# jeffchy/RE2NN-SEQ

Measured on AMD Instinct MI355X. Metric: tagged tokens/sec @ batch=256, seqlen=64; achieved HBM GB/s vs peak, higher is better.
Workload: dtype f32; 1 GPU; ATIS-BIO-sized onehot i-FST (--method onehot --independent 2): V=950 S=71 C=128, batch 256 x seqlen 64 per GPU, lengths U[5,64]; batches_rotated=4, parallelism=batch-sharded x1 (weights replicated)

## Files before the change

re2nn-seq_amd/csrc/chain_dest.hip.h:

```cpp
#pragma once
#include "common.hip.h"
#include "chain_regs_params.hip.h"

namespace farnn {

template <int D, int LPR>
struct DestRing {
    static constexpr int NC = 20 / LPR;
    v4f r[D][NC];
    unsigned voff[NC];
    int tkw_lo, tkw_hi;
};

template <int LPR>
__device__ __forceinline__ void dest_lane(const int lane, int &rj, int &rs, bool &has_row) {
    if constexpr (LPR == 4) { rj = lane >> 2; rs = lane & 3; has_row = true; }
    else { const int r16 = lane & 15, bq = r16 / 5; rs = r16 - 5 * bq; rj = 3 * (lane >> 4) + bq; has_row = bq < 3; }
}

#ifndef FARNN_RD_CPOL
#define FARNN_RD_CPOL ""
#endif
#define FARNN_RD_ISSUE_(ring_, d, base_)                                                       \
    do {                                                                                       \
        const char *bp_ = (base_);                                                             \
        if constexpr (NC == 5)                                                                 \
            asm volatile("s_nop 4\n\t"                                                         \
                         "global_load_dwordx4 %0, %5, %10" FARNN_RD_CPOL "\n\t"                                 \
                         "global_load_dwordx4 %1, %6, %10" FARNN_RD_CPOL "\n\t"                                 \
                         "global_load_dwordx4 %2, %7, %10" FARNN_RD_CPOL "\n\t"                                 \
                         "global_load_dwordx4 %3, %8, %10" FARNN_RD_CPOL "\n\t"                                 \
                         "global_load_dwordx4 %4, %9, %10" FARNN_RD_CPOL                                     \
                         : "=&v"(ring_.r[d][0]), "=&v"(ring_.r[d][1]), "=&v"(ring_.r[d][2]), "=&v"(ring_.r[d][3]), "=&v"(ring_.r[d][NC - 1]) \
                         : "v"(ring_.voff[0]), "v"(ring_.voff[1]), "v"(ring_.voff[2]), "v"(ring_.voff[3]), "v"(ring_.voff[NC - 1]), "s"(bp_)); \
        else                                                                                   \
            asm volatile("s_nop 4\n\t"                                                         \
                         "global_load_dwordx4 %0, %4, %8" FARNN_RD_CPOL "\n\t"                                  \
                         "global_load_dwordx4 %1, %5, %8" FARNN_RD_CPOL "\n\t"                                  \
                         "global_load_dwordx4 %2, %6, %8" FARNN_RD_CPOL "\n\t"                                  \
                         "global_load_dwordx4 %3, %7, %8" FARNN_RD_CPOL                                      \
                         : "=&v"(ring_.r[d][0]), "=&v"(ring_.r[d][1]), "=&v"(ring_.r[d][2]), "=&v"(ring_.r[d][3]) \
                         : "v"(ring_.voff[0]), "v"(ring_.voff[1]), "v"(ring_.voff[2]), "v"(ring_.voff[3]), "s"(bp_)); \
    } while (0)

template <int D, int LPR>
__device__ __forceinline__ void regs_dest_prime(const RegsParams &p, const int dir, const int w, const int lane, const int nsteps,
                                                const int len, const int b, DestRing<D, LPR> &ring) {
    constexpr int NC = DestRing<D, LPR>::NC;
    const int S = p.S, SP = p.SP, CPR = p.CPR;
    const int RW = (S + RG_NWC - 1) / RG_NWC;
    int rj, rs;
    bool has_row;
    dest_lane<LPR>(lane, rj, rs, has_row);
    const int my_row = w * RW + rj;
    const bool my_valid = has_row && rj < RW && my_row < S;
#pragma unroll
    for (int i = 0; i < NC; i++) {
        const int ci = rs + LPR * i;
        ring.voff[i] = ((unsigned)(my_valid ? my_row : 0) * (unsigned)SP + (unsigned)((my_valid && ci < CPR) ? ci : rs < CPR ? rs : 0) * 4u) * 4u;
    }
    {
        const int t = lane < nsteps ? lane : nsteps - 1;
        const int idx = (dir == 0) ? t : (t < len ? len - 1 - t : t);
        const long long o_ = (long long)clamp_tok(p.x[(long long)b * p.L + idx], p.V) * p.blk * 4;
        ring.tkw_lo = (int)(unsigned)o_; ring.tkw_hi = (int)(unsigned)(o_ >> 32);
    }
    const char *Mbase = reinterpret_cast<const char *>(dir == 0 ? p.Mb : p.Mf);
#pragma unroll
    for (int d = 0; d < D; d++) {
#pragma unroll
        for (int u = 0; u < NC; u++) ring.r[d][u] = v4f{0.f, 0.f, 0.f, 0.f};
        if (d < nsteps) {
            const unsigned lo = (unsigned)__builtin_amdgcn_readlane(ring.tkw_lo, d), hi = (unsigned)__builtin_amdgcn_readlane(ring.tkw_hi, d);
            FARNN_RD_ISSUE_(ring, d, Mbase + (((long long)hi << 32) | lo));
        }
    }
}

template <bool NLX, int D, int LPR>
__device__ __forceinline__ void regs_compute_dest(const RegsParams &p, const int dir, const int w, const int lane_in, const int nsteps,
                                                  const long long *tokoff, float *flags, const float *ol, float *hist, float *xd,
                                                  const bool probe, const int b, DestRing<D, LPR> &ring) {
    static_assert(D == 2 || D == 4, "an even ring depth that divides 64 (the exchange row's parity and the address window)");
    static_assert(LPR == 4 || LPR == 5, "four or five lanes per output row");
    constexpr int NC = 20 / LPR;
    static_assert(LPR * NC * 4 == RD_XS, "the exchange row holds every lane's chunks");
    int lane = lane_in;
    const int S = p.S, SP = p.SP, CPR = p.CPR;
    const int RW = (S + RG_NWC - 1) / RG_NWC;
    int rj, rs;
    bool has_row;
    dest_lane<LPR>(lane, rj, rs, has_row);
    const int my_row = w * RW + rj;
    const bool my_valid = has_row && rj < RW && my_row < S;
    const bool my_writer = my_valid && rs == (LPR == 4 ? 0 : 4);
    const bool is_flane = lane == 63;
    (void)CPR;
    const char *Mbase = reinterpret_cast<const char *>(dir == 0 ? p.Mb : p.Mf);
    const float my_o = my_valid ? ol[my_row] : 1.0f;
    const float c_pre = dir == 0 ? my_o : 1.0f, c_post = dir == 0 ? 1.0f : my_o;
    float *xbuf = xd;
    float *dumpa = xd + 2 * RD_XS, *dumpb = dumpa + 64;
    float *hptr = my_writer ? hist + SP + my_row : dumpa + lane;
    const int hstep = my_writer ? SP : 0;
    float *xw0 = my_writer ? xbuf + my_row : (is_flane ? flags + 4 * w : dumpb + lane);
    float *xw1 = my_writer ? xbuf + RD_XS + my_row : (is_flane ? flags + 4 * w : dumpb + lane);
    const float *xr = xbuf + 4 * rs;
    const int nl_mode = p.nl;
    const bool nl_relu = nl_mode == FARNN_NL_RELU;
    const int *pflag = reinterpret_cast<const int *>(flags) + 4 * (lane < RG_NWC ? lane : 0);

    v4f (&r)[D][NC] = ring.r;
    int &tkw_lo = ring.tkw_lo, &tkw_hi = ring.tkw_hi;
#define FARNN_RD_WINDOW(t_)                                                                    \
    do {                                                                                       \
        const int ti_ = (t_) + lane;                                                           \
        const long long o_ = tokoff[ti_ < nsteps ? ti_ : nsteps - 1];                          \
        tkw_lo = (int)(unsigned)o_; tkw_hi = (int)(unsigned)(o_ >> 32);                        \
    } while (0)
#define FARNN_RD_BASE(t_, lo_, hi_)                                                            \
    do {                                                                                       \
        const int li_ = (t_) & 63;                                                             \
        lo_ = (unsigned)__builtin_amdgcn_readlane(tkw_lo, li_);                                \
        hi_ = (unsigned)__builtin_amdgcn_readlane(tkw_hi, li_);                                \
    } while (0)
#define FARNN_RD_ISSUE(d, lo_, hi_) FARNN_RD_ISSUE_(ring, d, Mbase + (((long long)(hi_) << 32) | (lo_)))
#define FARNN_RD_WAITSTR                                                                       \
    "s_cmp_ge_i32 %[rem], %[dm1]\n\t"                                                          \
    "s_cbranch_scc1 1f\n\t"                                                                    \
    "s_waitcnt vmcnt(0)\n\t"                                                                   \
    "s_branch 2f\n"                                                                            \
    "1:\n\t"                                                                                   \
    "s_waitcnt vmcnt(%[cnt])\n"                                                                \
    "2:"
#define FARNN_RD_WAIT(d, rem_)                                                                 \
    do {                                                                                       \
        if constexpr (NC == 5)                                                                 \
            asm volatile(FARNN_RD_WAITSTR : "+v"(r[d][0]), "+v"(r[d][1]), "+v"(r[d][2]), "+v"(r[d][3]), "+v"(r[d][NC - 1]) \
                         : [rem] "s"(rem_), [dm1] "n"(D - 1), [cnt] "n"((D - 1) * NC) : "scc"); \
        else                                                                                   \
            asm volatile(FARNN_RD_WAITSTR : "+v"(r[d][0]), "+v"(r[d][1]), "+v"(r[d][2]), "+v"(r[d][3]) \
                         : [rem] "s"(rem_), [dm1] "n"(D - 1), [cnt] "n"((D - 1) * NC) : "scc"); \
    } while (0)

    unsigned nlo = 0, nhi = 0;
#if defined(FARNN_PROBES)
    long long ph[4] = {0, 0, 0, 0}, pt = 0;
#define FARNN_RD_PHASE(i) do { if (probe && w == 0 && (p.dbg & 256)) { const long long n_ = (long long)__builtin_amdgcn_s_memtime(); ph[i] += n_ - pt; pt = n_; } } while (0)
    if (probe && w == 0) pt = (long long)__builtin_amdgcn_s_memtime();
#else
#define FARNN_RD_PHASE(i) do { } while (0)
    (void)probe; (void)b;
#endif
    if (D < nsteps) FARNN_RD_BASE(D, nlo, nhi);
    for (int t0 = 0; t0 < nsteps; t0 += D) {
#pragma unroll
        for (int d = 0; d < D; d++) {
            const int t = t0 + d;
            if (t >= nsteps) break;
            constexpr int dummy = 0; (void)dummy;
            const int roff = (d & 1) * RD_XS;
            v4f st[NC];
            {
                int fl = lds_flag_get(pflag);
#pragma unroll
                for (int i = 0; i < NC; i++) st[i] = *reinterpret_cast<const v4f *>(xr + roff + 4 * LPR * i);
                asm volatile("" ::: "memory");
                if (__ballot(fl < t + 1) != 0ull) {
                    do { fl = lds_flag_get(pflag); } while (__ballot(fl < t + 1) != 0ull);
#pragma unroll
                    for (int i = 0; i < NC; i++) st[i] = *reinterpret_cast<const v4f *>(xr + roff + 4 * LPR * i);
                    asm volatile("" ::: "memory");
                }
            }
            FARNN_RD_PHASE(0);
            FARNN_RD_WAIT(d, nsteps - 1 - t);
            FARNN_RD_PHASE(1);
            v2f a01 = v2f{0.f, 0.f}, a23 = v2f{0.f, 0.f};
#pragma unroll
            for (int i = 0; i < NC; i++) {
                a01 = __builtin_elementwise_fma(st[i].xy, r[d][i].xy, a01);
                a23 = __builtin_elementwise_fma(st[i].zw, r[d][i].zw, a23);
            }
            float sa = a01.x + a01.y, sb = a23.x + a23.y;
            asm volatile("" : "+v"(sa), "+v"(sb));
            float s = sa + sb;
            if constexpr (LPR == 4) s = quad_sum(s);
            else {
                const float s1 = s + __int_as_float(__builtin_amdgcn_update_dpp(0, __float_as_int(s), 0x111, 0xf, 0xf, true));
                const float s2 = s1 + __int_as_float(__builtin_amdgcn_update_dpp(0, __float_as_int(s1), 0x112, 0xf, 0xf, true));
                s = s2 + __int_as_float(__builtin_amdgcn_update_dpp(0, __float_as_int(s), 0x114, 0xf, 0xf, true));
            }
            const float pre = s * c_pre;
            float hn;
            if (NLX) hn = apply_nl(pre, nl_mode);
            else     hn = nl_relu ? fmaxf(pre, 0.0f) : pre;
            const float hx = is_flane ? __int_as_float(t + 2) : hn * c_post;
            asm volatile("" ::: "memory");
            *hptr = hn;
            hptr += hstep;
            if (d & 1) *xw0 = hx; else *xw1 = hx;
            asm volatile("" ::: "memory");
            if (t + D < nsteps) FARNN_RD_ISSUE(d, nlo, nhi);
            if (d == D - 1 && ((t + 1 + D) & 63) == 0 && t + 1 + D < nsteps) FARNN_RD_WINDOW(t + 1 + D);
            FARNN_RD_BASE(t + 1 + D, nlo, nhi);
            asm volatile("" : "+s"(nlo), "+s"(nhi));
            FARNN_RD_PHASE(2);
        }
    }
#if defined(FARNN_PROBES)
    if (probe && w == 0 && lane == 0 && (p.dbg & 256))
        printf("seq %d dir %d chain phases (destination split), cycles per step: partner wait + state reads %lld, block wait %lld, fma + reduce + stores + issue %lld\n",
               b, dir, ph[0] / nsteps, ph[1] / nsteps, ph[2] / nsteps);
#endif
#undef FARNN_RD_PHASE
#undef FARNN_RD_WAIT
#undef FARNN_RD_WAITSTR
#undef FARNN_RD_ISSUE
#undef FARNN_RD_BASE
#undef FARNN_RD_WINDOW
}

}
```

re2nn-seq_amd/csrc/chain_regs.hip:

```cpp
#include <hip/hip_runtime.h>
#include <hip/hip_ext.h>

#include "common.hip.h"
#include "host_util.hip.h"
#include "chain_regs.hip.h"

namespace farnn {

int launch_chain_regs(const RegsParams &p, bool maxsr, bool score, hipStream_t s, hipEvent_t e0, hipEvent_t e1) {
    const int NP = RG_NWC * p.G;
    const bool dest = p.dest && !maxsr;
    const size_t lds = (size_t)regs_lds(p.L, p.SP, NP, p.sp.c16, p.sp.Kc, score, RG_RQ, score && bs_label_map_path(p.sp), dest).total * sizeof(float);
    const dim3 grid(2 * p.B), block(RG_WAVES * 64);
    int rc;
    const bool nlx = p.nl != FARNN_NL_NONE && p.nl != FARNN_NL_RELU;
    const bool lmo = score && bs_label_map_path(p.sp);
#define FARNN_LAUNCH_REGS5(MX, SC, NX, LM, DS)                                                 \
    do {                                                                                       \
        if ((rc = raise_lds_limit(chain_regs_kernel<MX, SC, NX, LM, DS>, lds))) return rc;     \
        if (e0 && e1)                                                                          \
            hipExtLaunchKernelGGL((chain_regs_kernel<MX, SC, NX, LM, DS>), grid, block, (uint32_t)lds, s, e0, e1, 0, p); \
        else                                                                                   \
            chain_regs_kernel<MX, SC, NX, LM, DS><<<grid, block, lds, s>>>(p);                \
    } while (0)
#if defined(FARNN_AB)
#define FARNN_LAUNCH_REGS4(MX, SC, NX, LM) do { if (!MX && dest) FARNN_LAUNCH_REGS5(MX, SC, NX, LM, !MX); else FARNN_LAUNCH_REGS5(MX, SC, NX, LM, false); } while (0)
#else
#define FARNN_LAUNCH_REGS4(MX, SC, NX, LM)                                                     \
    do {                                                                                       \
        if (!MX && dest) FARNN_LAUNCH_REGS5(MX, SC, NX, LM, !MX);                              \
        else if constexpr (MX) FARNN_LAUNCH_REGS5(MX, SC, NX, LM, false);                      \
        else return fail(FARNN_EINVAL, "FARNN_NODEST=1: the source-split compute wavefronts of the sum semiring are compiled into the A/B " \
                                       "build only (FARNN_LIB=.../libfarnn_hip_probes.so, csrc/build.py --probes)%s%s"); \
    } while (0)
#endif
#define FARNN_LAUNCH_REGS3(MX, SC, NX) do { if (SC && lmo) FARNN_LAUNCH_REGS4(MX, SC, NX, SC); else FARNN_LAUNCH_REGS4(MX, SC, NX, false); } while (0)
#define FARNN_LAUNCH_REGS(MX, SC) do { if (nlx) FARNN_LAUNCH_REGS3(MX, SC, true); else FARNN_LAUNCH_REGS3(MX, SC, false); } while (0)
    if (maxsr) { if (score) FARNN_LAUNCH_REGS(true, true); else FARNN_LAUNCH_REGS(true, false); }
    else       { if (score) FARNN_LAUNCH_REGS(false, true); else FARNN_LAUNCH_REGS(false, false); }
#undef FARNN_LAUNCH_REGS
#undef FARNN_LAUNCH_REGS3
#undef FARNN_LAUNCH_REGS4
#undef FARNN_LAUNCH_REGS5
    FARNN_HIP_TRY(hipGetLastError());
    return FARNN_OK;
}

}

#if defined(FARNN_PROBES)
extern "C" int farnn_debug_wg_stamps(long long *out, int n_workgroups) {
    if (!out || n_workgroups < 0 || n_workgroups > farnn::WG_STAMP_MAX) return FARNN_EINVAL;
    if (hipDeviceSynchronize() != hipSuccess) return FARNN_EIO;
    return hipMemcpyFromSymbol(out, HIP_SYMBOL(farnn::g_wg_stamps), sizeof(long long) * 16 * (size_t)n_workgroups) == hipSuccess ? FARNN_OK : FARNN_EIO;
}
#endif
```

re2nn-seq_amd/csrc/chain_regs.hip.h:

```cpp
#pragma once
#include "common.hip.h"
#include "score_params.hip.h"
#include "launch_order.hip.h"
#include "chain_regs_params.hip.h"
#include "beside.hip.h"

#ifndef FARNN_ABLATE
#define FARNN_ABLATE 0
#endif

namespace farnn {

__device__ __forceinline__ void lds_flag_set(int *f, int v) {
    asm volatile("" ::: "memory");
    __hip_atomic_store(f, v, __ATOMIC_RELAXED, __HIP_MEMORY_SCOPE_WORKGROUP);
}
__device__ __forceinline__ int lds_flag_get(const int *f) {
    const int v = __hip_atomic_load(f, __ATOMIC_RELAXED, __HIP_MEMORY_SCOPE_WORKGROUP);
    asm volatile("" ::: "memory");
    return v;
}
template <int PSTR = RG_PART_STRIDE>
__device__ __forceinline__ int regs_flag_newest(const float *fbase, int lane) {
    const int *f = reinterpret_cast<const int *>(fbase) + 4 * (lane < RG_NWC ? lane : 0);
    const int v0 = lds_flag_get(f), v1 = lds_flag_get(f + PSTR);
    return max(v0, v1);
}
template <int PSTR = RG_PART_STRIDE>
__device__ __forceinline__ bool regs_rows_reached(const float *fbase, int lane, int rows) {
    return __ballot(regs_flag_newest<PSTR>(fbase, lane) < rows + 1) == 0ull;
}
template <int PSTR = RG_PART_STRIDE>
__device__ __forceinline__ int regs_rows_done(const float *fbase, int lane) {
    int v = regs_flag_newest<PSTR>(fbase, lane);
#pragma unroll
    for (int off = 1; off < 8; off <<= 1) v = min(v, __shfl_xor(v, off, WAVE));
    return __builtin_amdgcn_readfirstlane(v) - 1;
}

__device__ __forceinline__ float quad_sum(float x) {
    x += __int_as_float(__builtin_amdgcn_update_dpp(0, __float_as_int(x), 0xB1, 0xf, 0xf, true));
    x += __int_as_float(__builtin_amdgcn_update_dpp(0, __float_as_int(x), 0x4E, 0xf, 0xf, true));
    return x;
}
__device__ __forceinline__ float quad_max(float x) {
    x = fmaxf(x, __int_as_float(__builtin_amdgcn_update_dpp(0, __float_as_int(x), 0xB1, 0xf, 0xf, true)));
    x = fmaxf(x, __int_as_float(__builtin_amdgcn_update_dpp(0, __float_as_int(x), 0x4E, 0xf, 0xf, true)));
    return x;
}

}
#include "chain_wide.hip.h"
#include "chain_dest.hip.h"
namespace farnn {

#if defined(FARNN_PROBES)
constexpr int WG_STAMP_MAX = 4096;
__device__ long long g_wg_stamps[16 * WG_STAMP_MAX];
#define FARNN_RG_STAMP(i) do { if (probe && lane == 0) stamps[i] = (long long)__builtin_amdgcn_s_memtime(); } while (0)
#else
#define FARNN_RG_STAMP(i) do { } while (0)
#endif

template <bool MAXSR, bool SCORE, bool NLX, int RQ = RG_RQ, int D = RG_D, bool LMO = false, bool DEST = false>
__device__ __forceinline__ void chain_regs_body(const RegsParams &p, float *smem, const int tid, const int item, int *b_out) {
    constexpr bool WIDE = RQ != RG_RQ;
    static_assert(!DEST || (!WIDE && !MAXSR), "the destination-split form exists for the narrow kernel and the sum semiring");
    constexpr int PSTR = WIDE ? rgw_part_stride(RQ) : RG_PART_STRIDE;
    constexpr int NG = WIDE ? RGW_NG : RG_NG;
    const int lane = tid & 63;
    const int w = __builtin_amdgcn_readfirstlane(tid >> 6);
    constexpr int nthreads = RG_WAVES * 64;
    const int dir = item & 1, slot = item >> 1;
    const int S = p.S, SP = p.SP, G = p.G, RPG = p.RPG, NP = RG_NWC * G;
    const int PS = WIDE ? p.PS : SP;
    const bool lm_path = SCORE && (LMO || bs_label_map_path(p.sp));
    const RegsLds lds = regs_lds(p.L, SP, NP, p.sp.c16, p.sp.Kc, SCORE, RQ, lm_path, DEST);
    long long *tokoff = reinterpret_cast<long long *>(smem + lds.tok);
    float *part = smem + lds.part, *ol = smem + lds.ol, *hist = smem + lds.hist;
    float *ab = smem + lds.ab, *scl = smem + lds.scl, *obuf = smem + lds.obuf;
    int *misc = reinterpret_cast<int *>(smem + lds.misc);

    int b = p.order ? p.order[slot] : slot;
    int len_sel = -1;
    if (p.sort) b = select_by_length_rank(p.len, p.B, p.L, p.pair ? folded_rank(slot, p.B) : slot, reinterpret_cast<int *>(hist), tid, nthreads, &len_sel);
    if (b_out) *b_out = b;
    const int len = len_sel >= 0 ? len_sel : clamp_len(p.len[b], p.L);
    const int nsteps = p.full ? p.L : len;
    const float *hinit = dir == 0 ? p.h0 : p.hT;
#if defined(FARNN_PROBES)
    __shared__ long long stamps[8];
    const bool quiet = (p.dbg & 2048) != 0;
    const bool probe = ((p.dbg & 32768) && nsteps == p.L && p.L >= 32) || quiet;
    if (w == 0) FARNN_RG_STAMP(0);
#endif

    constexpr bool PRIME_EARLY = DEST && (!SCORE || LMO);
    DestRing<RD_D, RD_LPR> dring;
    if constexpr (PRIME_EARLY)
        if (w < RG_NWC && nsteps > 0) regs_dest_prime<RD_D, RD_LPR>(p, dir, w, lane, nsteps, len, b, dring);
    for (int k = tid; k < nsteps; k += nthreads) {
        const int idx = (dir == 0) ? k : (k < len ? len - 1 - k : k);
        tokoff[k] = (long long)clamp_tok(p.x[(long long)b * p.L + idx], p.V) * p.blk * 4;
    }
    for (int j = tid; j < SP; j += nthreads) ol[j] = (p.o && j < S) ? p.o[j] : 1.0f;
    for (int j = tid; j < (nsteps + 1) * SP; j += nthreads) hist[j] = (j < S) ? hinit[j] : 0.0f;
    if (tid < 32) misc[tid] = tid == RGM_ACQ ? -1 : 0;
    if (tid < 2) part[tid * PSTR + PSTR - 1] = MAXSR ? -INFINITY : 0.0f;
    if (tid < 2 * 4 * RG_NWC) {
        const int fb = tid / (4 * RG_NWC), fk = tid % (4 * RG_NWC);
        part[fb * PSTR + NP * PS + fk] = (DEST && fb == 0 && (fk & 3) == 0) ? __int_as_float(1) : 0.0f;
    }
    if constexpr (DEST) {
        for (int j = tid; j < 2 * RD_XS; j += nthreads)
            smem[lds.xd + j] = j < S ? hinit[j] * ((dir == 1 && p.o) ? p.o[j] : 1.0f) : 0.0f;
    }
    if (WIDE && tid < RG_NWC * RGW_XCH) smem[lds.xch + tid] = 0.0f;
    __syncthreads();
    if (w == 0) FARNN_RG_STAMP(1);
#if FARNN_ABLATE & 256
    return;
#endif

    const float *sflag = part + NP * PS;
    float *stash = (dir == 0 ? p.A : p.Bk) + (long long)b * (p.L + 1) * SP;
    const int ntl = (nsteps + RG_TT - 1) / RG_TT;
    int kmid = 0, pubmax = 0;
    if (SCORE) bs_halves(dir, len, nsteps, kmid, pubmax);
    BesideParams bs;
    bs.A = p.A; bs.Bk = p.Bk; bs.B = p.B; bs.L = p.L; bs.SP = p.SP; bs.CPR = p.CPR; bs.prog = p.prog; bs.arr = p.arr;
    bs.done = p.done; bs.spin = p.spin; bs.dbg = p.dbg; bs.sp = p.sp;
    bs.epoch = (SCORE && w >= RG_NWC) ? (p.done ? bs_launch_epoch(p.done, lane) : p.epoch_host) : 0u;
    int wr_next = 0;
    unsigned lm_pk0 = 0u, lm_pk1 = 0u;
    if (lm_path) lm_load_packed(bs.sp.lm, lane, lm_pk0, lm_pk1);
    if (w < RG_NWC) {
        if constexpr (WIDE) {
            if (nsteps > 0) {
                __builtin_amdgcn_s_setprio(2);
                regs_compute_wide<MAXSR, NLX, RQ, D>(p, dir, w, lane, nsteps, tokoff, part, ol, hist, smem + lds.xch);
                __builtin_amdgcn_s_setprio(0);
                if (w == 0) FARNN_RG_STAMP(2);
#if defined(FARNN_PROBES)
                if (!SCORE && probe && !quiet && w == 0 && lane == 0)
                    printf("seq %d dir %d (wide): setup %lld, chain %lld (%lld per step)\n", b, dir, stamps[1] - stamps[0], stamps[2] - stamps[1],
                           (stamps[2] - stamps[1]) / nsteps);
#endif
            }
        } else if constexpr (DEST) {
            if (nsteps > 0) {
                __builtin_amdgcn_s_setprio(2);
#if defined(FARNN_PROBES)
                const bool probe_ = probe;
#else
                const bool probe_ = false;
#endif
                if constexpr (!PRIME_EARLY) regs_dest_prime<RD_D, RD_LPR>(p, dir, w, lane, nsteps, len, b, dring);
                regs_compute_dest<NLX, RD_D, RD_LPR>(p, dir, w, lane, nsteps, tokoff, part + NP * PS, ol, hist, smem + lds.xd, probe_, b, dring);
                __builtin_amdgcn_s_setprio(0);
                if (w == 0) FARNN_RG_STAMP(2);
#if defined(FARNN_PROBES)
                if (!SCORE && probe && !quiet && w == 0 && lane == 0)
                    printf("seq %d dir %d (destination split): setup %lld, chain %lld (%lld per step)\n", b, dir, stamps[1] - stamps[0], stamps[2] - stamps[1],
                           (stamps[2] - stamps[1]) / nsteps);
#endif
            }
        } else if (nsteps > 0) {
            __builtin_amdgcn_s_setprio(2);
            int g = lane / p.CPR;
            const int c = lane - g * p.CPR;
            const bool active = g < G;
            if (!active) g = 0;
            const int gid = w * G + g, row0 = gid * RPG;
            unsigned voff[RG_RQ];
#pragma unroll
            for (int u = 0; u < RG_RQ; u++) voff[u] = ((unsigned)(row0 + u) * (unsigned)SP + (unsigned)c * 4u) * 4u;
            const char *Mbase = reinterpret_cast<const char *>(dir == 0 ? p.Mf : p.Mb);
            const int rows_w = G * RPG;
            const int rj = lane >> 2, rs = lane & 3;
            const int my_row = w * rows_w + rj;
            const bool my_valid = rj < rows_w && my_row < S;
            const bool my_writer = my_valid && rs == 0;
            const float my_o = my_valid ? ol[my_row] : 1.0f;
            const float c_pre = dir == 0 ? my_o : 1.0f, c_post = dir == 0 ? 1.0f : my_o;
            const float ninf = -INFINITY;
            bool okrow[RG_RQ];
#pragma unroll
            for (int u = 0; u < RG_RQ; u++) okrow[u] = u < RPG && row0 + u < S;
            constexpr int NQI = (RG_NWC * RG_MAXG + 3) / 4;
            const float *ident = part + RG_PART_STRIDE - 1;
            float *dump = part + 2 * RG_PART_STRIDE;
            const float *qptr[NQI];
#pragma unroll
            for (int i = 0; i < NQI; i++)
                qptr[i] = (my_valid && rs + 4 * i < NP) ? part + (rs + 4 * i) * SP + my_row : ident;
            const int nact = G * p.CPR;
            const bool has_flane = nact < 64;
            const bool is_flane = lane == nact;
            float *fslot = part + NP * SP + 4 * w;
            float *wptr = active ? part + gid * SP + c * 4 : (is_flane ? fslot : part + NP * SP + 4 * RG_NWC + (lane - nact) * 4);
            float *hptr = my_writer ? hist + SP + my_row : dump + lane;
            const int hstep = my_writer ? SP : 0;
            int bsrc[RG_RQ];
            float hs[RG_RQ];
#pragma unroll
            for (int u = 0; u < RG_RQ; u++) {
                bsrc[u] = u < RPG ? 16 * (g * RPG + u) : 4 * 63;
                hs[u] = okrow[u] ? hist[row0 + u] * (dir == 1 ? ol[row0 + u] : 1.0f) : 0.0f;
            }
            const int nl_mode = p.nl;
            const bool nl_relu = nl_mode == FARNN_NL_RELU;
            const int *pflag = reinterpret_cast<const int *>(part + NP * SP) + 4 * (lane < RG_NWC ? lane : 0);

            v4f r[RG_D][RG_RQ];
#define FARNN_RG_WINDOW(t_)                                                                    \
            do {                                                                               \
                const int ti_ = (t_) + lane;                                                   \
                const long long o_ = tokoff[ti_ < nsteps ? ti_ : nsteps - 1];                  \
                tkw_lo = (int)(unsigned)o_; tkw_hi = (int)(unsigned)(o_ >> 32);                \
            } while (0)
#define FARNN_RG_BASE(t_, lo_, hi_)                                                            \
            do {                                                                               \
                const int li_ = (t_) & 63;                                                     \
                lo_ = (unsigned)__builtin_amdgcn_readlane(tkw_lo, li_);                        \
                hi_ = (unsigned)__builtin_amdgcn_readlane(tkw_hi, li_);                        \
            } while (0)
#define FARNN_RG_ISSUE(d, lo_, hi_)                                                            \
            do {                                                                               \
                const char *bp_ = Mbase + (((long long)(hi_) << 32) | (lo_));                  \
                asm volatile("s_nop 4\n\t"                                                     \
                             "global_load_dwordx4 %0, %4, %8\n\t"                              \
                             "global_load_dwordx4 %1, %5, %8\n\t"                              \
                             "global_load_dwordx4 %2, %6, %8\n\t"                              \
                             "global_load_dwordx4 %3, %7, %8"                                  \
                             : "=&v"(r[d][0]), "=&v"(r[d][1]), "=&v"(r[d][2]), "=&v"(r[d][3]) \
                             : "v"(voff[0]), "v"(voff[1]), "v"(voff[2]), "v"(voff[3]), "s"(bp_)); \
            } while (0)
#define FARNN_RG_WAIT(d, rem_)                                                                 \
            asm volatile("s_cmp_ge_i32 %4, 3\n\t"                                              \
                         "s_cbranch_scc1 1f\n\t"                                               \
                         "s_waitcnt vmcnt(0)\n\t"                                              \
                         "s_branch 2f\n"                                                       \
                         "1:\n\t"                                                              \
                         "s_waitcnt vmcnt(12)\n"                                               \
                         "2:"                                                                  \
                         : "+v"(r[d][0]), "+v"(r[d][1]), "+v"(r[d][2]), "+v"(r[d][3]) : "s"(rem_) : "scc")
            unsigned nlo = 0, nhi = 0;
            int tkw_lo, tkw_hi;
            FARNN_RG_WINDOW(0);
#pragma unroll
            for (int d = 0; d < RG_D; d++) {
#pragma unroll
                for (int u = 0; u < RG_RQ; u++) r[d][u] = v4f{0.f, 0.f, 0.f, 0.f};
                if (d < nsteps) {
                    FARNN_RG_BASE(d, nlo, nhi);
                    FARNN_RG_ISSUE(d, nlo, nhi);
                }
            }
#if defined(FARNN_PROBES)
            long long ph[5] = {0, 0, 0, 0, 0}, pt = 0;
#define FARNN_RG_PHASE(i) do { if (probe && w == 0 && (p.dbg & 256)) { const long long n_ = (long long)__builtin_amdgcn_s_memtime(); ph[i] += n_ - pt; pt = n_; } } while (0)
            if (probe && w == 0) pt = (long long)__builtin_amdgcn_s_memtime();
#else
#define FARNN_RG_PHASE(i) do { } while (0)
#endif
            if (RG_D < nsteps) FARNN_RG_BASE(RG_D, nlo, nhi);
#if FARNN_ABLATE & 512
            for (int t0 = 0; t0 < 0; t0 += RG_D) {
#else
            for (int t0 = 0; t0 < nsteps; t0 += RG_D) {
#endif
#pragma unroll
                for (int d = 0; d < RG_D; d++) {
                    const int t = t0 + d;
                    if (t >= nsteps) break;
                    static_assert(RG_D == 4 && RG_RQ == 4, "FARNN_RG_WAIT is written out for a 4 x 4 ring");
                    FARNN_RG_WAIT(d, nsteps - 1 - t);
                    FARNN_RG_PHASE(0);
                    v4f acc = MAXSR ? v4f{ninf, ninf, ninf, ninf} : v4f{0.f, 0.f, 0.f, 0.f};
#if FARNN_ABLATE & 8
                    acc = r[d][0] + r[d][1] * hs[0] + r[d][2] + r[d][3];
#else
#pragma unroll
                    for (int u = 0; u < RG_RQ; u++) {
                        if (MAXSR) {
                            acc.x = fmaxf(acc.x, okrow[u] ? hs[u] * r[d][u].x : ninf);
                            acc.y = fmaxf(acc.y, okrow[u] ? hs[u] * r[d][u].y : ninf);
                            acc.z = fmaxf(acc.z, okrow[u] ? hs[u] * r[d][u].z : ninf);
                            acc.w = fmaxf(acc.w, okrow[u] ? hs[u] * r[d][u].w : ninf);
                        } else {
                            acc.x = fmaf(hs[u], r[d][u].x, acc.x);
                            acc.y = fmaf(hs[u], r[d][u].y, acc.y);
                            acc.z = fmaf(hs[u], r[d][u].z, acc.z);
                            acc.w = fmaf(hs[u], r[d][u].w, acc.w);
                        }
                    }
#endif
                    const int boff = (d & 1) * RG_PART_STRIDE;
#if !(FARNN_ABLATE & 32)
                    if (has_flane) acc.x = is_flane ? __int_as_float(t + 1) : acc.x;
                    asm volatile("" ::: "memory");
                    *reinterpret_cast<v4f *>(wptr + boff) = acc;
                    if (!has_flane && lane == 0) lds_flag_set(reinterpret_cast<int *>(fslot + boff), t + 1);
#endif
                    asm volatile("" : "+v"(acc));
#if !(FARNN_ABLATE & 1)
                    if (t + RG_D < nsteps) FARNN_RG_ISSUE(d, nlo, nhi);
#endif
                    FARNN_RG_PHASE(1);
                    float pv[NQI];
#if FARNN_ABLATE & 16
#pragma unroll
                    for (int i = 0; i < NQI; i++) pv[i] = acc.x;
#else
                    for (;;) {
                        const int fl = lds_flag_get(pflag + boff);
#pragma unroll
                        for (int i = 0; i < NQI - 1; i++) pv[i] = qptr[i][boff];
                        pv[NQI - 1] = MAXSR ? ninf : 0.0f;
                        if (NP > 4 * (NQI - 1)) pv[NQI - 1] = qptr[NQI - 1][boff];
                        asm volatile("" ::: "memory");
                        if (__ballot(fl < t + 1) == 0ull) break;
#if FARNN_ABLATE & 2
                        break;
#endif
                    }
#endif
                    FARNN_RG_PHASE(2);
                    static_assert(NQI == 6, "the reduction tree below is written out for six partial sums per lane");
                    float s;
                    if (MAXSR) s = fmaxf(fmaxf(fmaxf(pv[0], pv[1]), fmaxf(pv[2], pv[3])), fmaxf(pv[4], pv[5]));
                    else       s = ((pv[0] + pv[1]) + (pv[2] + pv[3])) + (pv[4] + pv[5]);
                    s = MAXSR ? quad_max(s) : quad_sum(s);
                    const float pre = s * c_pre;
                    float hn;
                    if (NLX) hn = apply_nl(pre, nl_mode);
                    else     hn = nl_relu ? fmaxf(pre, 0.0f) : pre;
                    const float hx = my_valid ? hn * c_post : 0.0f;
#if !(FARNN_ABLATE & 64)
                    *hptr = hn;
                    hptr += hstep;
#endif
#if !(FARNN_ABLATE & 4)
                    int bp[RG_RQ];
#pragma unroll
                    for (int u = 0; u < RG_RQ; u++) bp[u] = __builtin_amdgcn_ds_bpermute(bsrc[u], __float_as_int(hx));
                    if (d == RG_D - 1 && ((t + 1 + RG_D) & 63) == 0 && t + 1 + RG_D < nsteps) FARNN_RG_WINDOW(t + 1 + RG_D);
                    FARNN_RG_BASE(t + 1 + RG_D, nlo, nhi);
                    asm volatile("" : "+s"(nlo), "+s"(nhi));
#pragma unroll
                    for (int u = 0; u < RG_RQ; u++) hs[u] = __int_as_float(bp[u]);
#else
                    if (t + 1 + RG_D < nsteps) {
                        if (((t + 1 + RG_D) & 63) == 0) FARNN_RG_WINDOW(t + 1 + RG_D);
                        FARNN_RG_BASE(t + 1 + RG_D, nlo, nhi);
                    }
#endif
                    FARNN_RG_PHASE(3);
                }
            }
            if (lane == 0) lds_flag_set(reinterpret_cast<int *>(fslot), nsteps + 1);
#if defined(FARNN_PROBES)
            if (probe && w == 0 && lane == 0 && (p.dbg & 256))
                printf("seq %d dir %d chain phases, cycles per step: block wait %lld, fma + store + issue %lld, partner wait + partial reads %lld, reduce + exchange %lld\n",
                       b, dir, ph[0] / nsteps, ph[1] / nsteps, ph[2] / nsteps, ph[3] / nsteps);
#endif
#undef FARNN_RG_PHASE
#undef FARNN_RG_ISSUE
#undef FARNN_RG_BASE
#undef FARNN_RG_WINDOW
#undef FARNN_RG_WAIT
            __builtin_amdgcn_s_setprio(0);
            if (w == 0) FARNN_RG_STAMP(2);
#if defined(FARNN_PROBES)
            if (!SCORE && probe && !quiet && w == 0 && lane == 0)
                printf("seq %d dir %d: setup %lld, chain %lld (%lld per step)\n", b, dir, stamps[1] - stamps[0], stamps[2] - stamps[1],
                       (stamps[2] - stamps[1]) / nsteps);
#endif
        }
    } else if (w == RG_NWC) {
        if (SCORE && dir == 0) {
            for (int i = nsteps + lane; i < p.L; i += WAVE)
                if (p.sp.tags) p.sp.tags[(long long)b * p.L + i] = -1;
            if (p.sp.scores)
                for (long long e = (long long)nsteps * p.sp.K + lane; e < (long long)p.L * p.sp.K; e += WAVE)
                    p.sp.scores[(long long)b * p.L * p.sp.K + e] = 0.0f;
        }
        int published = -1;
        auto copy_rows = [&](int r0, int r1) {
            const float *src = hist + r0 * SP;
            float *dst = stash + (long long)r0 * SP;
            const int nfl = (r1 - r0 + 1) * SP;
            if (SCORE) {
                for (int j = 2 * lane; j < nfl; j += 2 * WAVE) st2_agent(dst + j, src[j], src[j + 1]);
            } else {
                for (int j = lane; j < nfl; j += WAVE) dst[j] = src[j];
            }
        };
        if (!SCORE && !p.A) wr_next = nsteps + 1;
        while (wr_next <= nsteps) {
            const int done = nsteps > 0 ? regs_rows_done<PSTR>(sflag, lane) : 0;
            if (done < wr_next) { __builtin_amdgcn_s_sleep(1); continue; }
            if (SCORE && nsteps > 0 && wr_next > pubmax && done >= nsteps) break;
            const int hi = min(done, (SCORE && wr_next <= pubmax) ? pubmax : nsteps);
            copy_rows(wr_next, hi);
            wr_next = hi + 1;
            if (SCORE && hi < nsteps && published < pubmax) {
                published = hi;
                asm volatile("s_waitcnt vmcnt(0)" ::: "memory");
                if (lane == 0)
                    __hip_atomic_store(p.prog + (long long)dir * p.B + b, ((unsigned long long)bs.epoch << 32) | (unsigned)published,
                                       __ATOMIC_RELAXED, __HIP_MEMORY_SCOPE_AGENT);
            }
        }
    } else if (SCORE) {
        const int fo = bs_flat_offset(bs, b, lane);
        if (lane == 0) misc[RGM_FOFF] = fo;
        const long long foff = fo;
        unsigned mine = 0u;
        int acq = -1;
        const unsigned long long *oprog = p.prog + (long long)(dir ^ 1) * p.B + b;
        const int kfirst = dir == 0 ? kmid : kmid - 1, kstep = dir == 0 ? 1 : -1, klast = dir == 0 ? ntl : -1;
        if constexpr (!LMO)
        for (int k = kfirst; k != klast && !lm_path; k += kstep) {
            int na, nb;
            bs_tile_need(k, len, nsteps, na, nb);
            const int need_own = dir == 0 ? na : nb, need_oth = dir == 0 ? nb : na;
            if (nsteps - need_own < p.solo_margin) break;
            while (!regs_rows_reached<PSTR>(sflag, lane, need_own)) __builtin_amdgcn_s_sleep(4);
            if (need_oth > acq) {
                int pr = -1;
                for (;;) {
                    pr = lane == 0 ? bs_read_prog(oprog, bs.epoch) : 0;
                    pr = __builtin_amdgcn_readfirstlane(pr);
                    if (pr >= need_oth) break;
                    if (regs_rows_reached<PSTR>(sflag, lane, nsteps)) break;
                    __builtin_amdgcn_s_sleep(8);
                }
                if (pr < need_oth) break;
                __builtin_amdgcn_fence(__ATOMIC_ACQUIRE, "agent");
                acq = pr;
            }
            {
                const rg_f32x4 none[NG] = {};
                bs_score_tiles<false, RG_WAVES, NG, RG_NWC>(bs, b, dir, len, nsteps, k, -1, hist, nullptr, nullptr, ab, scl, foff, 0, lane, none);
            }
            mine |= 1u << k;
        }
        {
            int slot = 0;
            for (int k = kfirst; k != klast && slot < RG_NOB; k += kstep) {
                if ((mine >> k) & 1u) continue;
                int na, nb;
                bs_tile_need(k, len, nsteps, na, nb);
                const int need_oth = dir == 0 ? nb : na;
                if (need_oth > acq) {
                    int pr = -1;
                    for (;;) {
                        pr = lane == 0 ? bs_read_prog(oprog, bs.epoch) : 0;
                        pr = __builtin_amdgcn_readfirstlane(pr);
                        if (pr >= need_oth) break;
                        if (regs_rows_reached<PSTR>(sflag, lane, nsteps)) break;
                        __builtin_amdgcn_s_sleep(16);
                    }
                    if (pr < need_oth) break;
                    __builtin_amdgcn_fence(__ATOMIC_ACQUIRE, "agent");
                    acq = pr;
                }
                bs_park_rows<NG, (LMO && WIDE) ? NG / 2 : NG>(bs, b, dir, len, nsteps, k, obuf + slot * RG_TT * SP, lane);
                if (lane == 0) misc[RGM_PARK + slot] = k + 1;
                slot++;
            }
        }
        if (lane == 0) { misc[RGM_MINE] = (int)mine; misc[RGM_ACQ] = acq; }
        FARNN_RG_STAMP(3);
    }
    if constexpr (!SCORE) {
        if (b_out && dir == 0 && w == RG_WAVES - 1) {
            int partsum = 0;
            if (p.sp.flat && !p.sp.offs)
                for (int j = lane; j < b; j += WAVE) partsum += clamp_len(p.len[j], p.L);
#pragma unroll
            for (int off = 32; off >= 1; off >>= 1) partsum += __shfl_xor(partsum, off, WAVE);
            if (lane == 0) { misc[RGM_FOFF] = partsum; misc[RGM_FOFF + 1] = len; }
        }
        return;
    }

    if (w == 0) FARNN_RG_STAMP(4);
    bs_finish<RG_WAVES, NG, RG_WAVES - 1, RG_NWC, true, LMO>(bs, b, dir, len, nsteps, kmid, hist, ab, scl, obuf, misc, w, lane, lm_pk0, lm_pk1, bs.epoch,
        [&]() {
            if (w == RG_NWC)
                for (; wr_next <= nsteps; wr_next++)
                    for (int j = 2 * lane; j < SP; j += 2 * WAVE)
                        st2_agent(stash + (long long)wr_next * SP + j, hist[wr_next * SP + j], hist[wr_next * SP + j + 1]);
        },
        [&]() {
            if (w == RG_NWC) {
                asm volatile("s_waitcnt vmcnt(0)" ::: "memory");
                if (lane == 0)
                    __hip_atomic_store(p.prog + (long long)dir * p.B + b, ((unsigned long long)bs.epoch << 32) | (unsigned)nsteps,
                                       __ATOMIC_RELAXED, __HIP_MEMORY_SCOPE_AGENT);
            }
        });
#if defined(FARNN_PROBES)
    if (quiet && tid == 0 && item < WG_STAMP_MAX) {
        long long *o = g_wg_stamps + 16 * (long long)item + 8;
        o[0] = stamps[1] - stamps[0]; o[1] = stamps[2] - stamps[1]; o[2] = stamps[3] - stamps[2]; o[3] = stamps[4] - stamps[2];
        o[4] = (long long)__builtin_amdgcn_s_memtime() - stamps[4];
    }
    if (probe && !quiet && tid == 0) {
        const long long e = (long long)__builtin_amdgcn_s_memtime();
        printf("seq %d dir %d: setup %lld, chain %lld (%lld per step), scorer alone until +%lld, all waves at the meeting point +%lld, "
               "tiles + arrival %lld; tiles alone %d of %d\n", b, dir, stamps[1] - stamps[0], stamps[2] - stamps[1],
               (stamps[2] - stamps[1]) / nsteps, stamps[3] - stamps[2], stamps[4] - stamps[2], e - stamps[4],
               __popc((unsigned)misc[RGM_MINE]), ntl);
    }
#endif
}

template <bool MAXSR, bool SCORE, bool NLX, bool LMO = false, bool DEST = false>
__global__ void __launch_bounds__(RG_WAVES * 64, 4)
chain_regs_kernel(const RegsParams p) {
    extern __shared__ __align__(16) float smem[];
#if defined(FARNN_PROBES)
    long long w0r = 0, w0c = 0;
    if ((p.dbg & 2048) && threadIdx.x == 0) { w0r = (long long)__builtin_amdgcn_s_memrealtime(); w0c = (long long)__builtin_amdgcn_s_memtime(); }
    int b_probe = -1;
    chain_regs_body<MAXSR, SCORE, NLX, RG_RQ, RG_D, LMO, DEST>(p, smem, (int)threadIdx.x, (int)blockIdx.x, &b_probe);
    if ((p.dbg & 2048) && threadIdx.x == 0 && blockIdx.x < WG_STAMP_MAX) {
        const long long w1r = (long long)__builtin_amdgcn_s_memrealtime(), w1c = (long long)__builtin_amdgcn_s_memtime();
        unsigned hwid, xcc;
        asm volatile("s_getreg_b32 %0, hwreg(HW_REG_HW_ID)" : "=s"(hwid));
        asm volatile("s_getreg_b32 %0, hwreg(HW_REG_XCC_ID)" : "=s"(xcc));
        long long *o = g_wg_stamps + 16 * (long long)blockIdx.x;
        o[0] = b_probe; o[1] = b_probe >= 0 ? (long long)p.len[b_probe] : -1; o[2] = w0r; o[3] = w1r; o[4] = w1c - w0c;
        o[5] = xcc & 15u; o[6] = (hwid >> 13) & 7u; o[7] = (hwid >> 8) & 15u;
    }
#else
    chain_regs_body<MAXSR, SCORE, NLX, RG_RQ, RG_D, LMO, DEST>(p, smem, (int)threadIdx.x, (int)blockIdx.x, nullptr);
#endif
}

template <bool MAXSR, bool SCORE, bool NLX, int RQ, int D>
__global__ void __launch_bounds__(RG_WAVES * 64, 2)
chain_wide_kernel(const RegsParams p) {
    extern __shared__ __align__(16) float smem[];
    chain_regs_body<MAXSR, SCORE, NLX, RQ, D>(p, smem, (int)threadIdx.x, (int)blockIdx.x, nullptr);
}

template <bool MAXSR, bool NLX, int RQ>
__global__ void __launch_bounds__(RG_WAVES * 64, 4)
chain_wide_paired_kernel(const RegsParams p) {
    extern __shared__ __align__(16) float smem[];
    chain_regs_body<MAXSR, true, NLX, RQ, 2, true>(p, smem, (int)threadIdx.x, (int)blockIdx.x, nullptr);
}

}
```

re2nn-seq_amd/csrc/chain_regs_params.hip.h:

```cpp
#pragma once
#include <hip/hip_runtime.h>
#include "common.hip.h"
#include "score_params.hip.h"

namespace farnn {

constexpr int RG_NWC = 6;
constexpr int RG_WAVES = 8;
constexpr int RG_D = 4;
constexpr int RG_RQ = 4;
constexpr int RG_MAXG = 4;
constexpr int RG_MAXSP = 72;
constexpr int RG_PART_STRIDE = RG_NWC * RG_MAXG * RG_MAXSP;
constexpr int RGW_G = 2;
constexpr int RGW_NP = RG_NWC * RGW_G;
constexpr int RGW_MAXSP = 128;
constexpr int RGW_MAXRQ = 11;
__host__ __device__ constexpr int rgw_part_stride(int rq) { return rq <= 9 ? 1536 : 2048; }
constexpr int RGW_XCH = 32;
constexpr int RD_LPR = 5;
constexpr int RD_XS = 80;
constexpr int RD_D = 4;
constexpr int RD_XD_FLOATS = 2 * RD_XS + 128;

struct RegsParams {
    const float *Mf, *Mb;
    long long blk;
    const float *o, *h0, *hT;
    const int64_t *x, *len;
    const int *order;
    int sort;
    float *A, *Bk;
    int B, L, S, SP, CPR, V;
    int G, RPG;
    int RQ, D;
    int pair;
    int PS;
    int nl, full;
    unsigned long long *prog;
    unsigned long long *arr;
    unsigned long long *done;
    unsigned epoch_host;
    int spin;
    int dbg;
    int solo_margin;
    int dest;
    ScoreParams sp;
};
constexpr int RG_NG = 5;
constexpr int RGW_NG = 8;

struct RegsGeom {
    int G, RPG, NP, CPR, SP, rows;
    bool ok;
    bool wide;
    int RQ, D, PS;
};

inline RegsGeom regs_geometry(int S) {
    RegsGeom g;
    g.wide = false; g.RQ = RG_RQ; g.D = RG_D; g.PS = 0;
    g.SP = round_up(S, 4);
    g.CPR = g.SP / 4;
    g.ok = g.CPR <= 64 && S >= 1;
    g.G = g.ok ? 64 / g.CPR : 1;
    if (g.G > RG_MAXG) g.G = RG_MAXG;
    g.NP = RG_NWC * g.G;
    g.RPG = (S + g.NP - 1) / g.NP;
    if (g.RPG > RG_RQ) g.ok = false;
    g.rows = (g.NP - 1) * g.RPG + RG_RQ;
    if (g.NP * g.SP + 4 * RG_NWC + 4 * (64 - g.G * g.CPR) >= RG_PART_STRIDE) g.ok = false;
    if (!g.ok && S > 4 * RG_RQ && g.SP <= RGW_MAXSP) {
        g.wide = true;
        g.G = RGW_G; g.NP = RGW_NP;
        g.RPG = (S + g.NP - 1) / g.NP;
        g.RQ = g.RPG <= 8 ? 8 : (g.RPG <= 9 ? 9 : RGW_MAXRQ);
        g.D = 4;
        g.rows = g.NP * g.RPG;
        g.PS = ((g.SP + 15) & ~31) + 16;
        g.ok = g.RPG <= RGW_MAXRQ && g.NP * g.PS + 4 * RG_NWC + 4 * (64 - g.G * g.CPR) < rgw_part_stride(g.RQ);
    }
    return g;
}

struct RegsLds {
    int tok, hp, part, ol, hist, ab, scl, obuf, misc, xch, xd, total;
};
__host__ __device__ inline RegsLds regs_lds(int L, int SP, int NP, int c16, int Kc, bool score, int rq = RG_RQ, bool lm = false, bool dest = false) {
    const bool wide = rq != RG_RQ;
    RegsLds l;
    int at = 0;
    l.tok = at;  at += 2 * ((L + 1) & ~1);
    l.hp = at;
    l.part = at; at += 2 * (wide ? rgw_part_stride(rq) : RG_PART_STRIDE) + 64 * 4;
    l.ol = at;   at += SP;
    l.hist = at; at += (L + 1) * SP + 16;
    l.ab = at;   at += (score && !lm) ? 2 * RG_TT * (16 * c16 + 4) : 0;
    l.scl = at;  at += (score && !lm) ? 2 * RG_TT * Kc : 0;
    l.obuf = at; at += score ? 2 * RG_TT * SP : 0;
    l.misc = at; at += 32;
    l.xch = at;  at += wide ? RG_NWC * RGW_XCH : 0;
    l.xd = at;   at += dest ? RD_XD_FLOATS : 0;
    l.total = at;
    return l;
}

int launch_chain_regs(const RegsParams &p, bool maxsr, bool score, hipStream_t s, hipEvent_t e0, hipEvent_t e1);
int launch_chain_wide(const RegsParams &p, bool maxsr, bool score, hipStream_t s, hipEvent_t e0, hipEvent_t e1);
int launch_chain_wide_paired(const RegsParams &p, bool maxsr, hipStream_t s, hipEvent_t e0, hipEvent_t e1);

bool chain_viterbi_fits(int L, int SP, int NP, int K, int Kp, bool label_map, int rq = RG_RQ);
int launch_chain_viterbi(const RegsParams &p, const ScoreParams &sp, bool maxsr, hipStream_t s, hipEvent_t e0, hipEvent_t e1);

}
```

re2nn-seq_amd/csrc/farnn_hip.hip:

```cpp
#include <hip/hip_runtime.h>
#include <hip/hip_ext.h>
#include <stdlib.h>
#include <algorithm>
#include <utility>
#include <vector>

#include "common.hip.h"
#include "host_util.hip.h"
#include "chain.hip.h"
#include "score_decode.hip.h"
#include "layout.hip.h"
#include "fst4_score.hip.h"
#include "decomp_chain.hip.h"
#include "decomp1_score.hip.h"
#include "decomp_rows.hip.h"
#include "compact_tag.hip.h"
#include "decomp_regs.hip.h"
#include "compact.hip.h"
#include "chain_regs_params.hip.h"
#include "tag_host.hip.h"
#include "tag_create.hip.h"

namespace farnn {
thread_local char g_err[512] = "";
thread_local const Tunables *g_tun = nullptr;
}

extern "C" int farnn_has_compact(const farnn_model *m) { return (m && m->bmNS > 0 && m->bmF) ? 1 : 0; }

extern "C" int farnn_set_compact(farnn_model *m, int32_t enable) {
    if (!m) return fail(FARNN_EINVAL, "set_compact: null model%s%s");
    if (enable && !farnn_has_compact(m))
        return fail(FARNN_EINVAL, "set_compact: this model has no compact form (i-FST with 0/1 weights, sum semiring, at most 512 states)%s%s");
    if (!enable && !m->Mf) return fail(FARNN_EINVAL, "set_compact: this handle was created compact-only (no dense blocks)%s%s");
    m->compact_on = enable != 0;
    return FARNN_OK;
}

extern "C" int farnn_reserve(farnn_model *m, int32_t B, int32_t L) {
    if (!m || B <= 0 || L <= 0) return fail(FARNN_EINVAL, "reserve: bad arguments%s%s");
    Workspace &w = m->ws;
    if (B <= w.B && L <= w.L) return FARNN_OK;
    TunScope tun_scope(&m->tun);
    FARNN_HIP_TRY(hipSetDevice(m->device));
    const int nB = B > w.B ? B : w.B, nL = L > w.L ? L : w.L;
    if (w.A) FARNN_HIP_TRY(hipDeviceSynchronize());
    w.release();
    size_t stash = (size_t)nB * (nL + 1) * m->SP * sizeof(float);
    FARNN_HIP_TRY(hipMalloc((void **)&w.A, stash));
    FARNN_HIP_TRY(hipMalloc((void **)&w.Bk, stash));
    FARNN_HIP_TRY(hipMalloc((void **)&w.offs, (size_t)(nB + 1) * sizeof(int64_t)));
    FARNN_HIP_TRY(hipMalloc((void **)&w.order, (size_t)nB * sizeof(int)));
    w.hs_bytes = round_up_sz((size_t)(3 * nB + 48) * sizeof(unsigned long long), 16);
    FARNN_HIP_TRY(hipMalloc((void **)&w.hs, w.hs_bytes));
    FARNN_HIP_TRY(hipMemset(w.hs, 0, w.hs_bytes));
    if (m->use_crf)
        FARNN_HIP_TRY(hipMalloc((void **)&w.crf_scores, (size_t)nB * nL * m->Kp * sizeof(float) + 1024));
    if (m->d1_BSSp)
        FARNN_HIP_TRY(hipMalloc((void **)&w.d1_br, (size_t)nB * nL * ((m->S + 15) / 16) * ((m->RO + 15) / 16 * 16) * sizeof(float)));
    FARNN_HIP_TRY(hipMemset(w.A, 0, stash));
    FARNN_HIP_TRY(hipMemset(w.Bk, 0, stash));
    FARNN_HIP_TRY(hipDeviceSynchronize());
    w.B = nB; w.L = nL;
    return FARNN_OK;
}

struct KernelTimer {
    farnn_model *m; int which; hipStream_t s; hipEvent_t e0 = nullptr, e1 = nullptr;
    bool ext;
    KernelTimer(farnn_model *m_, int w, hipStream_t s_, bool ext_ = false) : m(m_), which(w), s(s_), ext(ext_) {
        if (m->prof_this_call) {
            e0 = m->prof.get(); e1 = m->prof.get();
            if (e0 && e1 && !ext) (void)hipEventRecord(e0, s);
        }
    }
    ~KernelTimer() {
        if (e0 && e1) {
            if (!ext) (void)hipEventRecord(e1, s);
            m->prof.ev[which].push_back(e0);
            m->prof.ev[which].push_back(e1);
        }
    }
};

static void prof_fold(farnn_model *m) {
    for (int k = 0; k < KERN_COUNT; k++) {
        auto &v = m->prof.ev[k];
        for (size_t i = 0; i + 1 < v.size(); i += 2) {
            float ms = 0.f;
            if (hipEventSynchronize(v[i + 1]) == hipSuccess &&
                hipEventElapsedTime(&ms, v[i], v[i + 1]) == hipSuccess) {
                m->prof.ms[k] += ms; m->prof.n[k] += 1;
            }
            m->prof.pool.push_back(v[i]); m->prof.pool.push_back(v[i + 1]);
        }
        v.clear();
    }
}

extern "C" int farnn_set_profiling(farnn_model *m, int32_t enable) {
    if (!m) return fail(FARNN_EINVAL, "null model%s%s");
    prof_fold(m);
    if (enable) {
        for (int k = 0; k < KERN_COUNT; k++) { m->prof.ms[k] = 0; m->prof.n[k] = 0; }
        while (m->prof.pool.size() < 256) {
            hipEvent_t e = nullptr;
            if (hipEventCreate(&e) != hipSuccess) break;
            m->prof.pool.push_back(e);
        }
    }
    m->profiling = enable > 0 ? enable : 0;
    m->calls = 0;
    return FARNN_OK;
}

extern "C" int farnn_kernel_time(farnn_model *m, int32_t which, double *total_ms, int64_t *launches) {
    if (!m || which < 0 || which >= KERN_COUNT) return fail(FARNN_EINVAL, "kernel_time: bad arguments%s%s");
    prof_fold(m);
    if (total_ms) *total_ms = m->prof.ms[which];
    if (launches) *launches = m->prof.n[which];
    return FARNN_OK;
}

extern "C" const char *farnn_kernel_name(const farnn_model *m, int32_t which) {
    if (!m) return "";
    TunScope tun_scope(&m->tun);
    switch (which) {
        case KERN_CHAIN:
            if (m->compact_on) return m->last_fused ? "compact_tag_kernel<fused: both chains + label-map scores + decode>" : "compact_chain_kernel";
            if (m->last_regs && m->last_fused && m->use_crf) return "chain_viterbi_kernel<fused: recurrence + scores + CRF decode>";
            if (m->last_regs && m->rgeom.wide) return m->last_fused ? "chain_wide_kernel<fused: scores + decode beside the recurrence>" : "chain_wide_kernel";
            if (m->last_regs) return m->last_fused ? "chain_regs_kernel<fused: scores + decode beside the recurrence>" : "chain_regs_kernel";
            if (m->dense_decomp) return "chain_kernel";
            if (m->kind == KIND_DECOMP && m->last_fused && m->last_wave) return "decomp_regs_kernel<fused: scores + decode beside the recurrence>";
            if (m->kind == KIND_DECOMP || m->kind == KIND_DECOMP1 || m->kind == KIND_DECOMP0)
                return m->rows.ok ? ((m->last_wave || (m->calls == 0 && m->dw.farnn == 0 && m->dw.R <= DG_ROWS && !tun(TUN_DECOMP_NOREGS))) ? "decomp_regs_kernel" : "decomp_rows_kernel") : "decomp_chain_kernel";
            return "chain_kernel";
        case KERN_SCORE: return m->kind == KIND_FST4 ? "fst4_score_kernel"
                              : (m->kind == KIND_IND1 ? "ind1_score_kernel"
                              : (m->kind == KIND_DECOMP1 ? (m->d1_BSSp ? "decomp1_br_mfma_kernel+decomp1_label_kernel" : "decomp1_score_kernel")
                              : (m->kind == KIND_DECOMP0 ? "decomp0_score_kernel"
                              : (m->use_crf ? "score_tile_kernel+viterbi_kernel" : (m->last_lm_score ? "label_map_score_kernel" : "score_tile_kernel")))));
        case KERN_PREP:  return "batch_prep_kernel";
        default: return "";
    }
}


static RegsParams make_regs_params(farnn_model *m, const int64_t *x, const int64_t *len, int B, int full) {
    const RegsGeom &rg = m->rgeom;
    RegsParams rp;
    memset(&rp, 0, sizeof(rp));
    rp.Mf = m->Mf; rp.Mb = m->Mb; rp.blk = (long long)m->geom.SR * m->SP;
    rp.o = m->o; rp.h0 = m->h0; rp.hT = m->hT; rp.x = x; rp.len = len;
    rp.order = m->order_valid ? m->ws.order : nullptr; rp.sort = m->sort_in_kernel ? 1 : 0;
    rp.A = m->ws.A; rp.Bk = m->ws.Bk; rp.B = B; rp.L = m->curL; rp.S = m->S; rp.SP = m->SP; rp.CPR = rg.CPR; rp.V = m->V;
    rp.G = rg.G; rp.RPG = rg.RPG; rp.RQ = rg.RQ; rp.D = rg.D; rp.PS = rg.PS; rp.pair = rg.wide ? 0 : 1;
    rp.nl = m->nl; rp.full = full; rp.dbg = tun(TUN_DBG);
    rp.dest = (!rg.wide && m->semiring != FARNN_SEMIRING_MAX && !tun(TUN_NODEST)) ? 1 : 0;
    return rp;
}

static int handoff_words(farnn_model *m, unsigned long long **prog, unsigned long long **arr, unsigned long long **done) {
    *prog = m->ws.hs; *arr = m->ws.hs + (size_t)2 * m->ws.B; *done = m->ws.hs + (size_t)3 * m->ws.B + 16;
    return FARNN_OK;
}

static int launch_chain(farnn_model *m, const int64_t *x, const int64_t *len, int B, int L, int full,
                        hipStream_t s, const ScoreParams *fuse_sp = nullptr, bool *fused = nullptr) {
    const ChainGeom &g = m->geom;
    if (fused) *fused = false;
    m->last_regs = false;
    if (m->rgeom.ok && !tun(TUN_NOREGS)) {
        const RegsGeom &rg = m->rgeom;
        const size_t lds_cap = rg.wide ? 158 * 1024 : 80 * 1024;
        bool score = fuse_sp && m->ws.hs && m->OTm && m->c16 >= 1 && m->c16 <= (rg.wide ? RGW_NG : RG_NG) && m->Kc <= 256 && m->curL <= 31 * RG_TT &&
                     (B <= 1024 || !fuse_sp->flat || fuse_sp->offs) && !tun(TUN_NOFUSE);
        if (score && !rg.wide && bs_label_map_path(*fuse_sp) && !tun(TUN_FUSE)) score = false;
        const bool lm_path = score && bs_label_map_path(*fuse_sp);
        const bool dest = !rg.wide && m->semiring != FARNN_SEMIRING_MAX && !tun(TUN_NODEST);
        size_t lds = (size_t)regs_lds(m->curL, m->SP, rg.NP, score ? m->c16 : 0, score ? m->Kc : 0, score, rg.RQ, lm_path, dest).total * sizeof(float);
        const bool paired = rg.wide && lm_path && rg.RQ <= 9 && lds <= 80 * 1024 && !tun(TUN_WIDE_UNPAIRED);
        if (score && lds > lds_cap) {
            score = false;
            lds = (size_t)regs_lds(m->curL, m->SP, rg.NP, 0, 0, false, rg.RQ, false, dest).total * sizeof(float);
        }
        if (lds <= lds_cap) {
            RegsParams rp = make_regs_params(m, x, len, B, full);
            if (score) {
                int hrc = handoff_words(m, &rp.prog, &rp.arr, &rp.done);
                if (hrc) return hrc;
                if (tun(TUN_HOST_EPOCH)) {
                    if (++m->epoch_u == 0) { FARNN_HIP_TRY(hipMemsetAsync(m->ws.hs, 0, m->ws.hs_bytes, s)); m->epoch_u = 1; }
                    rp.done = nullptr; rp.epoch_host = m->epoch_u + 0x40000000u;
                }
                rp.spin = tun(TUN_FUSE_SPIN);
                rp.solo_margin = tun(TUN_SOLO_MARGIN);
                rp.sp = *fuse_sp;
                if (fused) *fused = true;
            }
            KernelTimer kt(m, KERN_CHAIN, s, true);
            if (paired && score) { rp.D = 2; rp.pair = 1; }
            const int rc = (paired && score) ? launch_chain_wide_paired(rp, m->semiring == FARNN_SEMIRING_MAX, s, kt.e0, kt.e1)
                           : rg.wide ? launch_chain_wide(rp, m->semiring == FARNN_SEMIRING_MAX, score, s, kt.e0, kt.e1)
                                     : launch_chain_regs(rp, m->semiring == FARNN_SEMIRING_MAX, score, s, kt.e0, kt.e1);
            if (rc) return rc;
            m->last_regs = true;
            return FARNN_OK;
        }
    }
    (void)fuse_sp;
    ChainParams p;
    p.Mf = m->Mf; p.Mb = m->Mb; p.blk = (long long)m->geom.SR * m->SP;
    p.o = m->o; p.h0 = m->h0; p.hT = m->hT; p.x = x; p.len = len; p.A = m->ws.A; p.Bk = m->ws.Bk;
    p.order = m->order_valid ? m->ws.order : nullptr;
    p.sort = m->sort_in_kernel ? 1 : 0;
    p.B = B; p.L = m->curL; p.S = m->S; p.SP = m->SP; p.CPR = g.CPR; p.V = m->V;
    p.NW = g.NW; p.NLD = g.NLD; p.G = g.G; p.LPR = g.LPR; p.RPG = g.RPG; p.RPGp = g.RPGp; p.NQ = g.NQ;
    p.nl = m->nl; p.full = full; p.dbg = tun(TUN_DBG);
    int ks = 2, nqp = g.NQ;
    if (!g.pick_ring(m->curL, m->chain_ks, ks, nqp))
        return fail(FARNN_ERANGE, "chain kernel: LDS ring does not fit (sequence too long for this S)%s%s");
    p.KS = ks; p.NQP = nqp; p.PPS = (g.NQ + nqp - 1) / nqp;
    const size_t lds = g.lds_bytes(m->curL, ks, nqp);
    dim3 grid(2 * B), block((g.NW + g.NLD + 1) * 64);
    const bool mx = m->semiring == FARNN_SEMIRING_MAX;
    int rc = FARNN_OK;
    if (tun(TUN_CHAIN_HELPER) && block.x < 512) block = dim3(block.x + 64);
    KernelTimer kt(m, KERN_CHAIN, s, true);
    const int fq_max = block.x <= 384 ? 6 : 3;
    const int fq = (g.NCH == 1 && p.PPS == 1 && g.NQ <= fq_max && !tun(TUN_NOFAST)) ? g.NQ : 0;
    auto go = [&](auto NCH, auto FQ) {
        return mx ? launch_timed(chain_kernel<NCH(), true, FQ()>, grid, block, lds, s, kt.e0, kt.e1, p)
                  : launch_timed(chain_kernel<NCH(), false, FQ()>, grid, block, lds, s, kt.e0, kt.e1, p);
    };
    if (g.NCH == 1) {
        if (fq == 1) rc = go(int_c<1>(), int_c<1>());
        else if (fq == 2) rc = go(int_c<1>(), int_c<2>());
        else if (fq == 3) rc = go(int_c<1>(), int_c<3>());
        else if (fq == 4) rc = go(int_c<1>(), int_c<4>());
        else if (fq == 5) rc = go(int_c<1>(), int_c<5>());
        else if (fq == 6) rc = go(int_c<1>(), int_c<6>());
        else rc = go(int_c<1>(), int_c<0>());
    } else if (g.NCH == 2) rc = go(int_c<2>(), int_c<0>());
    else if (g.NCH <= 4) rc = go(int_c<4>(), int_c<0>());
    else return fail(FARNN_ERANGE, "unsupported state count%s%s");
    if (rc) return rc;
    FARNN_HIP_TRY(hipGetLastError());
    return FARNN_OK;
}

static int launch_decomp_recurrence(farnn_model *m, const int64_t *x, const int64_t *lengths, int B, int full,
                                    hipStream_t s, const ScoreParams *fuse_sp = nullptr, bool *fused = nullptr) {
    if (fused) *fused = false;
    const int *order = m->order_valid ? m->ws.order : nullptr;
    if (m->n_cu <= 0) m->n_cu = device_cus(m->device);
    RegsPlan rp;
    m->last_wave = m->rows.ok && regs_plan(m->rows, m->dw, m->curL, rp);
    if (m->last_wave) {
        BesideParams bs;
        const BesideParams *use = nullptr;
        bool score = fuse_sp && m->ws.hs && m->OTm && m->c16 >= 1 && m->c16 <= DG_NG && m->Kc <= 256 && m->curL <= 31 * RG_TT &&
                     (B <= 1024 || !fuse_sp->flat || fuse_sp->offs) && !tun(TUN_NOFUSE);
        if (score) {
            rp.lds_score = regs_score_lds(rp, m->curL, m->SP, m->c16, m->Kc);
            if (rp.lds_score > 80 * 1024) score = false;
        }
        if (score) {
            memset(&bs, 0, sizeof(bs));
            bs.A = m->ws.A; bs.Bk = m->ws.Bk; bs.B = B; bs.L = m->curL; bs.SP = m->SP; bs.CPR = m->SP / 4;
            int hrc = handoff_words(m, &bs.prog, &bs.arr, &bs.done);
            if (hrc) return hrc;
            bs.spin = tun(TUN_FUSE_SPIN); bs.dbg = tun(TUN_DBG); bs.sp = *fuse_sp;
            use = &bs;
            if (fused) *fused = true;
        }
        return launch_decomp_regs(m->rows, m->dw, rp, x, lengths, order, m->sort_in_kernel ? 1 : 0, m->ws.A, m->ws.Bk, B, m->curL,
                                  full, s, use);
    }
    RowsPlan pl;
    if (m->rows.ok && rows_plan(m->rows, m->dw, B, m->curL, pl))
        return launch_decomp_rows(m->rows, m->dw, pl, x, lengths, order, m->sort_in_kernel ? 1 : 0, m->ws.A, m->ws.Bk, B,
                                  m->curL, full, m->n_cu, s);
    return launch_decomp_chain(m->dw, x, lengths, order, m->ws.A, m->ws.Bk, B, m->curL, full, s);
}

static bool viterbi_can_fuse(const farnn_model *m, const ScoreParams &p) {
    return m->use_crf && !p.scores && !p.P && p.A && p.OT && m->K <= 256 &&
           viterbi_hist_lds_bytes(m->K, m->Kp, p.SP, p.L, true) <= 158 * 1024 && viterbi_hist_ib4(m->K) <= 6 &&
           !tun(TUN_VITERBI_BP) && !tun(TUN_VITERBI_UNFUSED);
}

static int launch_viterbi(farnn_model *m, const ScoreParams &p, int B, hipStream_t s, bool fused = false) {
    int rc;
    if (m->K > 256) return fail(FARNN_ERANGE, "Viterbi: more than 256 tags%s%s");
    const size_t hlds = viterbi_hist_lds_bytes(m->K, m->Kp, p.SP, p.L, fused);
    if (hlds <= 158 * 1024 && viterbi_hist_ib4(m->K) <= 6 && !tun(TUN_VITERBI_BP)) {
        const int threads = viterbi_hist_score_threads(m->K, fused);
        auto go = [&](auto N) {
            return fused ? launch(viterbi_hist_kernel<N(), true>, dim3(B), dim3(threads), hlds, s, p)
                         : launch(viterbi_hist_kernel<N(), false>, dim3(B), dim3(threads), hlds, s, p);
        };
        rc = FARNN_OK;
        switch (viterbi_hist_ib4(m->K)) {
            case 0: rc = go(int_c<0>()); break;
            case 1: rc = go(int_c<1>()); break;
            case 2: rc = go(int_c<2>()); break;
            case 3: rc = go(int_c<3>()); break;
            case 4: rc = go(int_c<4>()); break;
            case 5: rc = go(int_c<5>()); break;
            case 6: rc = go(int_c<6>()); break;
        }
        if (rc) return rc;
        FARNN_HIP_TRY(hipGetLastError());
        return FARNN_OK;
    }
    if (fused) return fail(FARNN_EINVAL, "Viterbi: the fused form needs the history in LDS%s%s");
    const size_t vlds = viterbi_lds_bytes(m->K, m->Kp, p.L);
    const int threads = round_up(4 * m->K, 64);
    auto go = [&](auto N) { return launch(viterbi_kernel<N()>, dim3(B), dim3(threads), vlds, s, p); };
    const int ib4 = viterbi_ib4(m->K);
    if (ib4 == 2) rc = go(int_c<2>());
    else if (ib4 == 4) rc = go(int_c<4>());
    else if (ib4 == 9) rc = go(int_c<9>());
    else if (ib4 == 13) rc = go(int_c<13>());
    else rc = go(int_c<16>());
    if (rc) return rc;
    FARNN_HIP_TRY(hipGetLastError());
    return FARNN_OK;
}

static int launch_decomp1_score(farnn_model *m, const int64_t *x, const int64_t *len, int B, int full,
                                int32_t *tags, int64_t *flat, float *scores, hipStream_t s) {
    Decomp1ScoreParams p;
    p.A = m->ws.A; p.Bk = m->ws.Bk; p.Vgen = m->dw.Vgen; p.S1 = m->dw.S1; p.S2 = m->dw.S2; p.W = m->dw.W;
    p.S1o = m->d1_S1o; p.S2o = m->d1_S2o; p.CoutT = m->d1_CoutT; p.P = m->P;
    p.x = x; p.len = len; p.offs = flat ? m->ws.offs : nullptr;
    p.tags = tags; p.flat = flat; p.scores = scores; p.crf_scores = m->ws.crf_scores;
    p.B = B; p.L = m->curL; p.S = m->S; p.SP = m->SP; p.R = m->R; p.Rp = m->Rp; p.RO = m->RO; p.ROp = m->ROp;
    p.V = m->V;
    p.K = m->K; p.Kp = m->Kp; p.Kc = m->Kc;
    p.full = full; p.use_crf = m->use_crf; p.o_idx = m->o_idx; p.threshold = m->threshold;
    int rc;
    KernelTimer kt(m, KERN_SCORE, s);
    Decomp1MfmaParams qm;
    qm.base = p; qm.BSSp = m->d1_BSSp; qm.S1oP = m->d1_S1oP; qm.S2oP = m->d1_S2oP; qm.br = m->ws.d1_br;
    if (!full) qm.base.offs = m->ws.offs;
    qm.MT = (m->S + 15) / 16; qm.NT = (m->RO + 15) / 16; qm.KQ4 = (m->S + 15) / 16;
    const size_t mlds = decomp1_mfma_lds_bytes(qm.MT, qm.NT);
    if (m->d1_BSSp && m->ws.d1_br && mlds <= 80 * 1024) {
        if (m->n_cu <= 0) m->n_cu = device_cus(m->device);
        const int nwg = std::min(2 * m->n_cu, (B * p.L + 3) / 4);
        auto go = [&](auto N) { return launch(decomp1_br_mfma_kernel<N()>, dim3(nwg), dim3(256), mlds, s, qm); };
        switch (qm.NT) {
            case 1: rc = go(int_c<1>()); break;
            case 2: rc = go(int_c<2>()); break;
            case 3: rc = go(int_c<3>()); break;
            case 4: rc = go(int_c<4>()); break;
            case 5: rc = go(int_c<5>()); break;
            default: return fail(FARNN_ERANGE, "decomp_ind1: output rank above 80 on the MFMA path%s%s");
        }
        if (rc) return rc;
        FARNN_HIP_TRY(hipGetLastError());
        const int NC = qm.NT * 16;
        const bool staged = decomp1_label_lds_bytes(NC, m->RO, m->K, m->Kc, true, 16) <= 150 * 1024;
        const int lthreads = staged ? 1024 : 256;
        const size_t llds = decomp1_label_lds_bytes(NC, m->RO, m->K, m->Kc, staged, lthreads / 64);
        const int lgrid = std::min((staged ? 1 : 4) * m->n_cu, (B * p.L + lthreads / 64 - 1) / (lthreads / 64));
        if (staged) {
            if ((rc = raise_lds_limit(decomp1_label_kernel<true>, llds))) return rc;
            decomp1_label_kernel<true><<<dim3(lgrid), dim3(lthreads), llds, s>>>(p, m->ws.d1_br, NC, qm.MT, full ? nullptr : m->ws.offs);
        } else {
            decomp1_label_kernel<false><<<dim3(lgrid), dim3(lthreads), llds, s>>>(p, m->ws.d1_br, NC, qm.MT, full ? nullptr : m->ws.offs);
        }
    } else {
        const size_t lds = decomp1_score_lds_bytes(m->S, m->SP, m->Rp, m->ROp, m->Kc);
        if ((rc = raise_lds_limit(decomp1_score_kernel, lds))) return rc;
        decomp1_score_kernel<<<dim3(p.L, B), dim3(256), lds, s>>>(p);
    }
    FARNN_HIP_TRY(hipGetLastError());
    if (m->use_crf) {
        ScoreParams v;
        memset(&v, 0, sizeof(v));
        v.trT = m->tr; v.len = len; v.offs = flat ? m->ws.offs : nullptr; v.tags = tags; v.flat = flat;
        v.crf_scores = m->ws.crf_scores; v.B = B; v.L = m->curL; v.K = m->K; v.Kp = m->Kp;
        v.full = full; v.use_crf = 1; v.o_idx = m->o_idx; v.threshold = m->threshold;
        if ((rc = launch_viterbi(m, v, B, s))) return rc;
    }
    return FARNN_OK;
}

static int launch_decomp0_score(farnn_model *m, const int64_t *x, const int64_t *len, int B, int full,
                                int32_t *tags, int64_t *flat, float *scores, hipStream_t s) {
    Decomp0ScoreParams p;
    p.A = m->ws.A; p.Bk = m->ws.Bk; p.Vgen = m->d0_Vgen; p.S1 = m->dw.S1; p.S2 = m->dw.S2; p.CT = m->d0_CT;
    p.S1w = m->d0_S1w; p.S2w = m->d0_S2w; p.CwT = m->d0_CwT; p.P = m->P;
    p.x = x; p.len = len; p.offs = flat ? m->ws.offs : nullptr;
    p.tags = tags; p.flat = flat; p.scores = scores; p.crf_scores = m->ws.crf_scores;
    p.B = B; p.L = m->curL; p.S = m->S; p.SP = m->SP; p.R = m->R; p.Rp = m->Rp; p.RW = m->RW; p.RWp = m->RWp;
    p.V = m->V;
    p.K = m->K; p.Kp = m->Kp; p.Kc = m->Kc;
    p.full = full; p.use_crf = m->use_crf; p.o_idx = m->o_idx; p.threshold = m->threshold;
    const size_t lds = decomp0_score_lds_bytes(m->SP, m->Rp, m->RWp, m->Kc);
    int rc;
    if ((rc = raise_lds_limit(decomp0_score_kernel, lds))) return rc;
    KernelTimer kt(m, KERN_SCORE, s);
    decomp0_score_kernel<<<dim3((p.L + D0_TOK - 1) / D0_TOK, B), dim3(256), lds, s>>>(p);
    FARNN_HIP_TRY(hipGetLastError());
    if (m->use_crf) {
        ScoreParams v;
        memset(&v, 0, sizeof(v));
        v.trT = m->tr; v.len = len; v.offs = flat ? m->ws.offs : nullptr; v.tags = tags; v.flat = flat;
        v.crf_scores = m->ws.crf_scores; v.B = B; v.L = m->curL; v.K = m->K; v.Kp = m->Kp;
        v.full = full; v.use_crf = 1; v.o_idx = m->o_idx; v.threshold = m->threshold;
        if ((rc = launch_viterbi(m, v, B, s))) return rc;
    }
    return FARNN_OK;
}

static ScoreParams make_score_params(farnn_model *m, const int64_t *len, int B, int full, int32_t *tags,
                                     int64_t *flat, float *scores) {
    ScoreParams p;
    memset(&p, 0, sizeof(p));
    p.A = m->ws.A; p.Bk = m->ws.Bk; p.OT = m->OT; p.OTm = m->OTm; p.c16 = m->c16; p.P = m->P; p.trT = m->tr; p.len = len;
    p.offs = (flat && !m->prep_in_kernel) ? m->ws.offs : nullptr; p.tags = tags; p.flat = flat; p.scores = scores;
    p.crf_scores = m->ws.crf_scores;
    p.B = B; p.L = m->curL; p.S = m->S; p.SP = m->SP; p.K = m->K; p.Kp = m->Kp; p.Kc = m->Kc;
    p.kch = m->Kc / 64;
    p.full = full; p.use_crf = m->use_crf; p.o_idx = m->o_idx; p.threshold = m->threshold;
    p.dbg = tun(TUN_DBG);
    p.kz = (m->kind == KIND_IFST && m->use_crf && !tun(TUN_NOKZ)) ? m->C : 0;
    p.lm = m->lm;
    return p;
}

static int launch_score_decode(farnn_model *m, const int64_t *len, int B, int full, int32_t *tags,
                               int64_t *flat, float *scores, hipStream_t s) {
    ScoreParams p = make_score_params(m, len, B, full, tags, flat, scores);
    if (viterbi_can_fuse(m, p)) {
        KernelTimer kt(m, KERN_SCORE, s);
        return launch_viterbi(m, p, B, s, true);
    }
    int rc;
    if (p.lm.on && !p.P && !scores && !m->use_crf && m->S <= LM_MAXS * 2 && (B <= 1024 || !flat || p.offs)) {
        KernelTimer kt(m, KERN_SCORE, s);
        label_map_score_kernel<LMS_WAVES><<<B, LMS_WAVES * 64, 0, s>>>(p);
        FARNN_HIP_TRY(hipGetLastError());
        m->last_lm_score = true;
        return FARNN_OK;
    }
    m->last_lm_score = false;
    const size_t lds = score_lds_bytes(m->S, m->Kc);
    const dim3 grid((p.L + SCORE_TT - 1) / SCORE_TT, B), block(SCORE_WAVES * 64);
    KernelTimer kt(m, KERN_SCORE, s);
    auto go = [&](auto KCH) { return launch(score_tile_kernel<KCH()>, grid, block, lds, s, p); };
    switch (p.kch) {
        case 1: rc = go(int_c<1>()); break;
        case 2: rc = go(int_c<2>()); break;
        case 3: rc = go(int_c<3>()); break;
        default: rc = go(int_c<4>()); break;
    }
    if (rc) return rc;
    FARNN_HIP_TRY(hipGetLastError());
    if (m->use_crf && (rc = launch_viterbi(m, p, B, s))) return rc;
    return FARNN_OK;
}

static int launch_chain_and_decode(farnn_model *m, const int64_t *x, const int64_t *len, int B, int L, int full,
                                   int32_t *tags, int64_t *flat, float *scores, hipStream_t s) {
    int rc;
    if (!m->use_crf) {
        const ScoreParams sp = make_score_params(m, len, B, full, tags, flat, scores);
        bool fused = false;
        if ((rc = launch_chain(m, x, len, B, L, full, s, &sp, &fused))) return rc;
        m->last_fused = fused;
        if (fused) return FARNN_OK;
    } else {
        m->last_fused = false;
        const ScoreParams sp = make_score_params(m, len, B, full, tags, flat, scores);
#if defined(FARNN_AB)
        if (tun(TUN_CV_ONE) && m->rgeom.ok && !tun(TUN_NOREGS) && !tun(TUN_NOFUSE) && viterbi_can_fuse(m, sp) &&
            (B <= 1024 || !flat || sp.offs) && chain_viterbi_fits(m->curL, m->SP, m->rgeom.NP, m->K, m->Kp, m->lm.on != 0, m->rgeom.RQ)) {
            const RegsParams rp = make_regs_params(m, x, len, B, full);
            KernelTimer kt(m, KERN_CHAIN, s, true);
            if ((rc = launch_chain_viterbi(rp, sp, m->semiring == FARNN_SEMIRING_MAX, s, kt.e0, kt.e1))) return rc;
            m->last_regs = true; m->last_fused = true;
            return FARNN_OK;
        }
#endif
        if ((rc = launch_chain(m, x, len, B, L, full, s))) return rc;
    }
    return launch_score_decode(m, len, B, full, tags, flat, scores, s);
}

__global__ void clamp_oo_column_kernel(float *scores, long long rows, int K, int col, float threshold) {
    const long long r = (long long)blockIdx.x * blockDim.x + threadIdx.x;
    if (r < rows) {
        const float x = scores[r * K + col];
        scores[r * K + col] = (x < threshold || x != x) ? x : threshold;
    }
}

static int tag_impl(farnn_model *m, const int64_t *x, const int64_t *lengths, int32_t B, int32_t L,
                    int32_t mode, int32_t *tags, int64_t *flat_tags, float *scores, void *stream) {
    TunScope tun_scope(&m->tun);
    FARNN_HIP_TRY(hipSetDevice(m->device));
    hipStream_t s = reinterpret_cast<hipStream_t>(stream);
    int rc;
    hipStreamCaptureStatus cap_ = hipStreamCaptureStatusNone;
    const bool capturing = hipStreamIsCapturing(s, &cap_) != hipSuccess || cap_ != hipStreamCaptureStatusNone;
    if (m->have_last && m->last_stream != s && !capturing) {
        if (!m->ev_order) FARNN_HIP_TRY(hipEventCreateWithFlags(&m->ev_order, hipEventDisableTiming));
        if (!m->multi_stream) FARNN_HIP_TRY(hipEventRecord(m->ev_order, m->last_stream));
        FARNN_HIP_TRY(hipStreamWaitEvent(s, m->ev_order, 0));
        m->multi_stream = true;
    }
    m->last_stream = s; m->have_last = true;
    struct LeaveEvent {
        farnn_model *m; hipStream_t s; bool on;
        ~LeaveEvent() { if (on && m->ev_order) (void)hipEventRecord(m->ev_order, s); }
    } leave_event{m, s, m->multi_stream && !capturing};
    if (B > m->ws.B || L > m->ws.L)
        if ((rc = farnn_reserve(m, B, L))) return rc;
    m->curL = L;
    const int full = mode == FARNN_MODE_FULL;
    m->prof_this_call = m->profiling > 0 && (m->calls++ % m->profiling) == 0;
    const bool want_order = !full && B > 2 && !tun(TUN_NOSORT);
    m->prep_in_kernel = (m->kind == KIND_IFST || (m->kind == KIND_DECOMP && m->rows.ok)) && B <= 1024 && L <= 1023 &&
                        !tun(TUN_PREP);
    m->order_valid = want_order && !m->prep_in_kernel;
    m->sort_in_kernel = want_order && m->prep_in_kernel;
    const bool want_offs = flat_tags || (m->kind == KIND_DECOMP1 && m->d1_BSSp && !full);
    if ((want_offs || want_order) && !m->prep_in_kernel) {
        KernelTimer kt(m, KERN_PREP, s);
        if (B <= 1024) {
            int G = 1;
            while (G < 16 && B * G * 2 <= 1024) G *= 2;
            batch_prep_small_kernel<<<1, round_up(B * G, 64), 0, s>>>(
                lengths, want_offs ? m->ws.offs : nullptr, want_order ? m->ws.order : nullptr, B, L, G);
        }
        else
            batch_prep_kernel<<<1, 1024, (size_t)(L + 2) * sizeof(int), s>>>(
                lengths, want_offs ? m->ws.offs : nullptr, want_order ? m->ws.order : nullptr, B, L);
        FARNN_HIP_TRY(hipGetLastError());
    }
    switch (m->kind) {
        case KIND_IFST:
            if (m->compact_on) {
                if (L > 1024) return fail(FARNN_ERANGE, "compact recurrence: more than 1024 positions%s%s");
                CompactParams cp;
                cp.bitsF = m->bmF; cp.bitsB = m->bmB; cp.wF = m->bmWF; cp.wB = m->bmWB; cp.o = m->o; cp.h0 = m->h0; cp.hT = m->hT;
                cp.mF = m->bmMF; cp.mB = m->bmMB; cp.xF = m->bmXF; cp.xB = m->bmXB; cp.tokoff = m->bmTok;
                cp.x = x; cp.len = lengths; cp.order = m->order_valid ? m->ws.order : nullptr; cp.A = m->ws.A; cp.Bk = m->ws.Bk;
                cp.B = B; cp.L = L; cp.S = m->S; cp.SP = m->SP; cp.V = m->V; cp.nl = m->nl; cp.full = full; cp.dbg = tun(TUN_DBG);
                m->last_fused = false;
                {
                    const ScoreParams sp = make_score_params(m, lengths, B, full, tags, flat_tags, scores);
                    if (m->bmTok && sp.lm.on && !sp.P && !scores && !m->use_crf && !tun(TUN_NOFUSE) &&
                        compact_tag_fits(m->V, m->S, L) && (B <= 1024 || !flat_tags || sp.offs)) {
                        const size_t lds = (size_t)compact_tag_lds(L, m->bmNS).total * 4;
                        const int nlk = m->nl == FARNN_NL_NONE ? 0 : m->nl == FARNN_NL_RELU ? 1 : 2;
                        const int nw = (m->S + 31) / 32;
                        KernelTimer kt(m, KERN_CHAIN, s);
                        auto go = [&](auto NW) {
                            const dim3 grid(B), block(CT_WAVES * 64);
                            if (nlk == 0) return launch(compact_tag_kernel<NW(), 0>, grid, block, lds, s, cp, sp);
                            if (nlk == 1) return launch(compact_tag_kernel<NW(), 1>, grid, block, lds, s, cp, sp);
                            return launch(compact_tag_kernel<NW(), 2>, grid, block, lds, s, cp, sp);
                        };
                        if (nw <= 1) rc = go(int_c<1>()); else if (nw == 2) rc = go(int_c<2>());
                        else if (nw == 3) rc = go(int_c<3>()); else rc = go(int_c<4>());
                        if (rc) return rc;
                        FARNN_HIP_TRY(hipGetLastError());
                        m->last_fused = true;
                        return FARNN_OK;
                    }
                }
                {
                    KernelTimer kt(m, KERN_CHAIN, s);
                    if ((rc = launch_compact_chain(cp, m->bmNS, s))) return rc;
                }
                return launch_score_decode(m, lengths, B, full, tags, flat_tags, scores, s);
            }
            return launch_chain_and_decode(m, x, lengths, B, L, full, tags, flat_tags, scores, s);
        case KIND_FST4:
            if ((rc = launch_chain(m, x, lengths, B, L, full, s))) return rc;
            {
                KernelTimer kt(m, KERN_SCORE, s);
                return launch_fst4_score(m->A4, m->ws.A, m->ws.Bk, m->P, x, lengths, flat_tags ? m->ws.offs : nullptr,
                                         tags, flat_tags, scores, B, m->curL, m->S, m->SP, m->C, m->Kc, full,
                                         m->o_idx, m->threshold,  nullptr, m->V, s);
            }
        case KIND_IND1:
            if ((rc = launch_chain(m, x, lengths, B, L, full, s))) return rc;
            {
                KernelTimer kt(m, KERN_SCORE, s);
                return launch_fst4_score(m->Ms, m->ws.A, m->ws.Bk, m->P, x, lengths, flat_tags ? m->ws.offs : nullptr,
                                         tags, flat_tags, scores, B, m->curL, m->S, m->SP, m->C, m->Kc, full,
                                         m->o_idx, m->threshold, m->Oten, m->V, s);
            }
        case KIND_DECOMP: {
            if (m->dense_decomp) return launch_chain_and_decode(m, x, lengths, B, L, full, tags, flat_tags, scores, s);
            bool fused = false;
            {
                KernelTimer kt(m, KERN_CHAIN, s);
                if (!m->use_crf) {
                    const ScoreParams sp = make_score_params(m, lengths, B, full, tags, flat_tags, scores);
                    if ((rc = launch_decomp_recurrence(m, x, lengths, B, full, s, &sp, &fused))) return rc;
                } else if ((rc = launch_decomp_recurrence(m, x, lengths, B, full, s))) return rc;
            }
            m->last_fused = fused;
            if (fused) return FARNN_OK;
            return launch_score_decode(m, lengths, B, full, tags, flat_tags, scores, s);
        }
        case KIND_DECOMP0: {
            {
                KernelTimer kt(m, KERN_CHAIN, s);
                if ((rc = launch_decomp_recurrence(m, x, lengths, B, full, s))) return rc;
            }
            return launch_decomp0_score(m, x, lengths, B, full, tags, flat_tags, scores, s);
        }
        case KIND_DECOMP1: {
            if (m->dense_decomp) {
                if ((rc = launch_chain(m, x, lengths, B, L, full, s))) return rc;
            } else {
                KernelTimer kt(m, KERN_CHAIN, s);
                if ((rc = launch_decomp_chain(m->dw, x, lengths, nullptr, m->ws.A, m->ws.Bk, B, m->curL, full, s))) return rc;
            }
            return launch_decomp1_score(m, x, lengths, B, full, tags, flat_tags, scores, s);
        }
        default:
            return fail(FARNN_EINVAL, "tag: unknown model kind%s%s");
    }
}

extern "C" int farnn_tag(farnn_model *m, const int64_t *x, const int64_t *lengths, int32_t B, int32_t L,
                         int32_t mode, int32_t *tags, int64_t *flat_tags, float *scores, void *stream) {
    if (!m || !x || !lengths) return fail(FARNN_EINVAL, "tag: null model / x / lengths%s%s");
    if (B <= 0 || L <= 0) return fail(FARNN_EINVAL, "tag: B and L must be positive%s%s");
    if (mode != FARNN_MODE_LOCAL && mode != FARNN_MODE_FULL && mode != FARNN_MODE_RE)
        return fail(FARNN_EINVAL, "tag: bad mode%s%s");
    if (mode != FARNN_MODE_RE) return tag_impl(m, x, lengths, B, L, mode, tags, flat_tags, scores, stream);
    if (m->kind != KIND_IFST && m->kind != KIND_FST4 && m->kind != KIND_IND1)
        return fail(FARNN_EINVAL, "tag: FARNN_MODE_RE exists on the onehot models only (model_onehot.py:148)%s%s");
    int rc = tag_impl(m, x, lengths, B, L, FARNN_MODE_FULL, tags, flat_tags, scores, stream);
    if (rc || !scores) return rc;
    const long long rows = (long long)B * L;
    clamp_oo_column_kernel<<<(unsigned)((rows + 255) / 256), 256, 0, reinterpret_cast<hipStream_t>(stream)>>>(
        scores, rows, m->K, m->C - 1, m->threshold);
    FARNN_HIP_TRY(hipGetLastError());
    return FARNN_OK;
}

static void host_slot_free(farnn_model::HostSlot &h) {
    if (h.x_pin) (void)hipHostFree(h.x_pin);
    if (h.flat_pin) (void)hipHostFree(h.flat_pin);
    if (h.x_dev) (void)hipFree(h.x_dev);
    h.x_pin = h.flat_pin = h.x_dev = h.flat_dev = h.x_map = nullptr;
    h.capN = h.capB = 0;
}

extern "C" int farnn_tag_host_submit(farnn_model *m, const int64_t *x_host, const int64_t *len_host, int32_t B, int32_t L,
                                     int32_t *ticket, int64_t *n_flat) {
    if (!m || !x_host || !len_host || !ticket) return fail(FARNN_EINVAL, "tag_host_submit: null argument%s%s");
    if (B <= 0 || L <= 0) return fail(FARNN_EINVAL, "tag_host_submit: B and L must be positive%s%s");
    FARNN_HIP_TRY(hipSetDevice(m->device));
    if (!m->hs_run) FARNN_HIP_TRY(hipStreamCreateWithFlags(&m->hs_run, hipStreamNonBlocking));
    const int slot = m->hnext;
    farnn_model::HostSlot &h = m->hslot[slot];
    if (h.busy && h.ev_out && hipEventQuery(h.ev_out) == hipSuccess) h.busy = false;
    if (h.busy) return fail(FARNN_EINVAL, "tag_host_submit: FARNN_HOST_SLOTS batches already in flight (wait for the oldest ticket first)%s%s");
    const size_t N = (size_t)B * L;
    if (N > h.capN || (size_t)B > h.capB) {
        FARNN_HIP_TRY(hipStreamSynchronize(m->hs_run));
        host_slot_free(h);
        FARNN_HIP_TRY(hipHostMalloc((void **)&h.x_pin, (N + B) * 8 + 16, hipHostMallocMapped));
        FARNN_HIP_TRY(hipHostMalloc((void **)&h.flat_pin, N * 8, hipHostMallocMapped));
        FARNN_HIP_TRY(hipMalloc((void **)&h.x_dev, (N + B) * 8 + 16));
        FARNN_HIP_TRY(hipHostGetDevicePointer((void **)&h.x_map, h.x_pin, 0));
        FARNN_HIP_TRY(hipHostGetDevicePointer((void **)&h.flat_dev, h.flat_pin, 0));
        h.capN = N; h.capB = (size_t)B;
    }
    if (!h.ev_out) FARNN_HIP_TRY(hipEventCreateWithFlags(&h.ev_out, hipEventDisableTiming));
    if (B > m->ws.B || L > m->ws.L) {
        FARNN_HIP_TRY(hipStreamSynchronize(m->hs_run));
        int rc = farnn_reserve(m, B, L);
        if (rc) return rc;
    }
    memcpy(h.x_pin, x_host, N * 8);
    memcpy(h.x_pin + N, len_host, (size_t)B * 8);
    long long total = 0;
    for (int b = 0; b < B; b++) { const long long v = len_host[b]; total += v < 0 ? 0 : (v > L ? L : v); }
    h.total = total;
    {
        const long long n = (long long)(N + B);
        stage_in_kernel<<<(unsigned)((n / 2 + 256) / 256), 256, 0, m->hs_run>>>(h.x_map, h.x_dev, n);
        FARNN_HIP_TRY(hipGetLastError());
    }
    int rc = farnn_tag(m, h.x_dev, h.x_dev + N, B, L, FARNN_MODE_LOCAL, nullptr, h.flat_dev, nullptr, m->hs_run);
    if (rc) return rc;
    FARNN_HIP_TRY(hipEventRecord(h.ev_out, m->hs_run));
    h.busy = true;
    h.gen = (h.gen + 1) & 0x7fffffu;
    m->hnext = (slot + 1) % FARNN_HOST_SLOTS;
    *ticket = (int32_t)((unsigned)slot | (h.gen << 8));
    if (n_flat) *n_flat = total;
    return FARNN_OK;
}

extern "C" int farnn_tag_host_wait(farnn_model *m, int32_t ticket, int64_t *flat_out, int64_t *n_out) {
    if (!m || ticket < 0 || (ticket & 0xff) >= FARNN_HOST_SLOTS) return fail(FARNN_EINVAL, "tag_host_wait: bad ticket%s%s");
    farnn_model::HostSlot &h = m->hslot[ticket & 0xff];
    if (!h.busy || h.gen != ((unsigned)ticket >> 8))
        return fail(FARNN_EINVAL, "tag_host_wait: no batch in flight under this ticket (stale or already waited for)%s%s");
    FARNN_HIP_TRY(hipSetDevice(m->device));
    FARNN_HIP_TRY(hipEventSynchronize(h.ev_out));
    if (flat_out && h.total > 0) memcpy(flat_out, h.flat_pin, (size_t)h.total * 8);
    if (n_out) *n_out = h.total;
    h.busy = false;
    return FARNN_OK;
}

extern "C" int64_t farnn_flatten_host(const int64_t *a, const int64_t *len_host, int32_t B, int32_t L, int64_t *out) {
    int64_t n = 0;
    if (!a || !len_host || !out) return -1;
    for (int b = 0; b < B; b++) {
        long long v = len_host[b];
        v = v < 0 ? 0 : (v > L ? L : v);
        memcpy(out + n, a + (size_t)b * L, (size_t)v * 8);
        n += v;
    }
    return n;
}

extern "C" void farnn_destroy(farnn_model *m) {
    if (!m) return;
    (void)hipSetDevice(m->device);
    (void)hipDeviceSynchronize();
    for (auto &h : m->hslot) {
        host_slot_free(h);
        if (h.ev_out) (void)hipEventDestroy(h.ev_out);
    }
    if (m->hs_run) (void)hipStreamDestroy(m->hs_run);
    prof_fold(m);
    for (hipEvent_t e : m->prof.pool) (void)hipEventDestroy(e);
    for (void *p : m->owned) (void)hipFree(p);
    m->ws.release();
    if (m->ev_order) (void)hipEventDestroy(m->ev_order);
    delete m;
}

extern "C" int farnn_abi_version(void) { return FARNN_ABI_VERSION; }
extern "C" int farnn_ab_build(void) {
#if defined(FARNN_AB)
    return 1;
#else
    return 0;
#endif
}

extern "C" int farnn_device_count(void) {
    int n = 0;
    if (hipGetDeviceCount(&n) != hipSuccess) return 0;
    return n;
}

extern "C" const char *farnn_last_error(void) { return g_err; }

extern "C" int farnn_num_columns(const farnn_model *m) { return m ? m->K : 0; }

extern "C" double farnn_algorithmic_bytes(const farnn_model *m, int64_t valid_tokens) {
    if (!m) return 0.0;
    const double S = m->S, C = m->C, R = m->R, K = m->K;
    double per_tok = 0.0, once = 0.0;
    switch (m->kind) {
        case KIND_IFST: per_tok = 2.0 * S * S * 4 + 12; break;
        case KIND_IND1: per_tok = 3.0 * S * S * 4 + 12; once = C * S * S * 4; break;
        case KIND_FST4: per_tok = (C + 2.0) * S * S * 4 + 12; break;
        case KIND_DECOMP0:
        case KIND_DECOMP1:
        case KIND_DECOMP:
            per_tok = R * 4 + 12;
            once = (2.0 * S * R + S * S + K * S) * 4;
            break;
    }
    return per_tok * (double)valid_tokens + once;
}

extern "C" double farnn_kernel_algorithmic_bytes(const farnn_model *m, int32_t which, int64_t valid_tokens) {
    if (!m) return 0.0;
    const double S = m->S, C = m->C, R = m->R, K = m->K, n = (double)valid_tokens;
    if (which == KERN_CHAIN) {
        if (m->compact_on) return (2.0 * S * m->bmNS * 8 + 8) * n;
        if (!m->dense_decomp && (m->kind == KIND_DECOMP || m->kind == KIND_DECOMP1 || m->kind == KIND_DECOMP0))
            return (R * 4 + 8) * n + (2.0 * S * R + S * S) * 4;
        return (2.0 * S * S * 4 + 8 + (m->last_fused ? 4 : 0)) * n + (m->last_fused ? K * S * 4 : 0);
    }
    if (which == KERN_SCORE) {
        switch (m->kind) {
            case KIND_FST4: return (C * S * S * 4 + 4) * n;
            case KIND_IND1: return (S * S * 4 + 4) * n + C * S * S * 4;
            default: return 4 * n + K * S * 4;
        }
    }
    return 0.0;
}


#if defined(FARNN_PROBES)
extern "C" int farnn_debug_ct_stamps(long long *out, int n_workgroups) {
    if (!out || n_workgroups < 0 || n_workgroups > farnn::CT_STAMP_MAX) return FARNN_EINVAL;
    if (hipDeviceSynchronize() != hipSuccess) return FARNN_EIO;
    return hipMemcpyFromSymbol(out, HIP_SYMBOL(farnn::g_ct_stamps), sizeof(long long) * 16 * (size_t)n_workgroups) == hipSuccess ? FARNN_OK : FARNN_EIO;
}
#endif
```

re2nn-seq_amd/csrc/host_util.hip.h:

```cpp
#pragma once
#include <hip/hip_runtime.h>
#include <hip/hip_ext.h>
#include <stdlib.h>
#include <map>
#include <mutex>
#include <type_traits>
#include <utility>
#include "common.hip.h"

namespace farnn {

inline int env_int(const char *name, int dflt) {
    const char *v = getenv(name);
    return (v && *v) ? atoi(v) : dflt;
}

inline int check_env_switches() {
#if !defined(FARNN_AB)
    for (const char *name : {"FARNN_CV_ONE", "FARNN_CV_STASH", "FARNN_NODEST"})
        if (env_int(name, 0))
            return fail(FARNN_EINVAL, "%s is set: that form is compiled into the A/B build only (csrc/build.py --probes; load it with "
                                      "FARNN_LIB=.../libfarnn_hip_probes.so)%s", name);
#endif
    for (const char *name : {"FARNN_CV_WIDE", "FARNN_DECOMP_OLD"})
        if (env_int(name, 0))
            return fail(FARNN_EINVAL, "%s is set: that switch was removed (round 5; include/farnn.h lists the supported ones)%s", name);
    return FARNN_OK;
}

inline int select_device(int device) {
    if (int rc = check_env_switches()) return rc;
    int n = 0;
    if (hipGetDeviceCount(&n) != hipSuccess || n <= 0)
        return fail(FARNN_ENODEV, "no HIP device visible%s%s");
    if (device < 0 || device >= n) return fail(FARNN_EINVAL, "device index out of range%s%s");
    FARNN_HIP_TRY(hipSetDevice(device));
    return FARNN_OK;
}

#define FARNN_TUNABLES(X)                                                                                      \
                                                                                                \
    X(NOFUSE, 0, true) X(FUSE, 0, true) X(NOREGS, 0, true) X(NOLABELMAP, 0, true) X(PREP, 0, true) X(NOSORT, 0, true)           \
    X(VITERBI_BP, 0, true) X(VITERBI_UNFUSED, 0, true) X(DECOMP_NOREGS, 0, true)                               \
    X(ROWS_NOREGS, 0, true) X(TRAIN_NOLDS, 0, true) X(TRAIN_NSEQ, 0, true)              \
    X(WIDE_UNPAIRED, 0, true) X(ROWS_LPR4, 0, true) X(ROWS_NOROUNDS, 0, true)                                  \
                       \
    X(CV_ONE, 0, false) X(CV_STASH, 0, false) X(NODEST, 0, false)                                              \
                                                                         \
    X(DBG, 0, false) X(KS, 3, false) X(RPG, 12, false) X(NLD, 4, false) X(NOFAST, 0, false)                    \
    X(CHAIN_HELPER, 0, false) X(HOST_EPOCH, 0, false) X(CV_NOSORT, 0, false) X(NOKZ, 0, false)                 \
    X(FUSE_SPIN, 4, false) X(SOLO_MARGIN, 24, false) X(DECOMP_FOUR, 0, false) X(ROWS_NSEQ, 0, false)
enum TunId {
#define FARNN_TUN_ENUM(name, dflt, prod) TUN_##name,
    FARNN_TUNABLES(FARNN_TUN_ENUM)
#undef FARNN_TUN_ENUM
    TUN_COUNT
};
struct Tunables {
    int v[TUN_COUNT];
    Tunables() {
#if defined(FARNN_PROBES)
        constexpr bool diag = true;
#else
        constexpr bool diag = false;
#endif
#define FARNN_TUN_READ(name, dflt, prod) v[TUN_##name] = ((prod) || diag) ? env_int("FARNN_" #name, dflt) : (dflt);
        FARNN_TUNABLES(FARNN_TUN_READ)
#undef FARNN_TUN_READ
    }
};
extern thread_local const Tunables *g_tun;
struct TunScope {
    const Tunables *prev;
    explicit TunScope(const Tunables *t) : prev(g_tun) { g_tun = t; }
    ~TunScope() { g_tun = prev; }
};
inline int tun(TunId id) {
    static const Tunables defaults_at_load;
    return (g_tun ? g_tun : &defaults_at_load)->v[id];
}

inline int lds_fits(size_t bytes) {
    return bytes > 160 * 1024 ? fail(FARNN_ERANGE, "kernel needs more than 160 KiB of LDS%s%s") : FARNN_OK;
}

template <typename KernelT>
inline int raise_lds_limit(KernelT kern, size_t bytes) {
    static std::map<std::pair<int, const void *>, size_t> granted;
    static std::mutex granted_mu;
    if (int rc = lds_fits(bytes)) return rc;
    if (bytes <= 48 * 1024) return FARNN_OK;
    int dev = 0;
    (void)hipGetDevice(&dev);
    const void *fn = reinterpret_cast<const void *>(kern);
    std::lock_guard<std::mutex> lock(granted_mu);
    size_t &g = granted[{dev, fn}];
    if (bytes > g) {
        FARNN_HIP_TRY(hipFuncSetAttribute(fn, hipFuncAttributeMaxDynamicSharedMemorySize, (int)bytes));
        g = bytes;
    }
    return FARNN_OK;
}

template <typename... Params, typename... Args>
inline int launch(void (*kern)(Params...), dim3 grid, dim3 block, size_t lds, hipStream_t s, Args &&...args) {
    if (int rc = raise_lds_limit(kern, lds)) return rc;
    kern<<<grid, block, lds, s>>>(std::forward<Args>(args)...);
    return FARNN_OK;
}
template <typename... Params, typename... Args>
inline int launch_timed(void (*kern)(Params...), dim3 grid, dim3 block, size_t lds, hipStream_t s, hipEvent_t e0, hipEvent_t e1,
                        Args &&...args) {
    if (int rc = raise_lds_limit(kern, lds)) return rc;
    if (e0 && e1) hipExtLaunchKernelGGL(kern, grid, block, (uint32_t)lds, s, e0, e1, 0, std::forward<Args>(args)...);
    else kern<<<grid, block, lds, s>>>(std::forward<Args>(args)...);
    return FARNN_OK;
}
template <int N>
using int_c = std::integral_constant<int, N>;
inline int device_cus(int device) {
    int ncu = 0;
    return hipDeviceGetAttribute(&ncu, hipDeviceAttributeMultiprocessorCount, device) == hipSuccess && ncu > 0 ? ncu : 256;
}

template <typename T>
struct DevBuf {
    T *p = nullptr;
    size_t n = 0;
    ~DevBuf() { release(); }
    int ensure(size_t need, const char *what) {
        if (need <= n) return FARNN_OK;
        if (p) { FARNN_HIP_TRY(hipDeviceSynchronize()); release(); }
        if (hipMalloc((void **)&p, need * sizeof(T)) != hipSuccess) { p = nullptr; return fail(FARNN_ENOMEM, what); }
        n = need;
        return FARNN_OK;
    }
    void release() { if (p) (void)hipFree(p); p = nullptr; n = 0; }
};

}
```

re2nn-seq_amd/csrc/layout.hip.h:

```cpp
#pragma once
#include "common.hip.h"

namespace farnn {

__global__ void transpose_pad_kernel(const float *src, float *dst, int rows, int cols, int rows_p) {
    int i = blockIdx.x * blockDim.x + threadIdx.x;
    if (i >= rows * cols) return;
    int r = i / cols, c = i - r * cols;
    dst[(long long)c * rows_p + r] = src[i];
}

__global__ void colsum_kernel(const float *src, float *dst, int rows, int cols) {
    int c = blockIdx.x * blockDim.x + threadIdx.x;
    if (c >= cols) return;
    float s = 0.0f;
    for (int r = 0; r < rows; r++) s += src[(long long)r * cols + c];
    dst[c] = s;
}

__global__ void premix_kernel(const float *T, const float *W, const float *mask, float *Mf, float *Mb,
                              int S, int SP, int SR) {
    const long long v = blockIdx.y;
    int idx = blockIdx.x * blockDim.x + threadIdx.x;
    if (idx >= SR * SP) return;
    int r = idx / SP, cpad = idx - r * SP;
    const float *Tv = T + v * S * S;
    float f = 0.0f, bwd = 0.0f;
    if (cpad < S && r < S) {
        f = Tv[r * S + cpad] + W[r * S + cpad];
        if (mask) f *= mask[r * S + cpad];
        bwd = Tv[cpad * S + r] + W[cpad * S + r];
        if (mask) bwd *= mask[cpad * S + r];
    }
    Mf[v * SR * SP + idx] = f;
    if (Mb) Mb[v * SR * SP + idx] = bwd;
}

inline int launch_premix(const float *T, const float *W, const float *mask, float *Mf, float *Mb,
                         int V, int S, int SP, int SR) {
    dim3 grid((SR * SP + 255) / 256, V);
    premix_kernel<<<grid, 256>>>(T, W, mask, Mf, Mb, S, SP, SR);
    FARNN_HIP_TRY(hipGetLastError());
    FARNN_HIP_TRY(hipDeviceSynchronize());
    return FARNN_OK;
}

__global__ void premix_fst4_kernel(const float *T4, const float *W4, float *Mf, float *Mb, float *A4,
                                   int C, int S, int SP, int SR) {
    const long long v = blockIdx.y;
    int idx = blockIdx.x * blockDim.x + threadIdx.x;
    if (idx >= SR * SP) return;
    int r = idx / SP, cpad = idx - r * SP;
    if (r >= S) {
        Mf[v * SR * SP + idx] = 0.0f;
        Mb[v * SR * SP + idx] = 0.0f;
        return;
    }
    const long long SS = (long long)S * S;
    float tsum = 0.0f, wsum = 0.0f, tsum_b = 0.0f, wsum_b = 0.0f;
    for (int c = 0; c < C; c++) {
        float a = 0.0f;
        if (cpad < S) {
            float t = T4[(v * C + c) * SS + r * S + cpad];
            float w = W4[c * SS + r * S + cpad];
            tsum += t; wsum += w; a = t + w;
            tsum_b += T4[(v * C + c) * SS + cpad * S + r];
            wsum_b += W4[c * SS + cpad * S + r];
        }
        A4[((v * C + c) * S) * SP + idx] = a;
    }
    Mf[v * SR * SP + idx] = tsum + wsum;
    Mb[v * SR * SP + idx] = tsum_b + wsum_b;
}

inline int launch_premix_fst4(const float *T4, const float *W4, float *Mf, float *Mb, float *A4,
                              int V, int C, int S, int SP, int SR) {
    dim3 grid((SR * SP + 255) / 256, V);
    premix_fst4_kernel<<<grid, 256>>>(T4, W4, Mf, Mb, A4, C, S, SP, SR);
    FARNN_HIP_TRY(hipGetLastError());
    FARNN_HIP_TRY(hipDeviceSynchronize());
    return FARNN_OK;
}

__global__ void scatter_edges_kernel(const int32_t *word, const int32_t *from, const int32_t *to,
                                     const int32_t *label, const float *val, long long n,
                                     float *T, float *W, float *O, int V, int S, int C, int mode, int *bad) {
    const long long e = (long long)blockIdx.x * blockDim.x + threadIdx.x;
    if (e >= n) return;
    const int w = word[e], f = from[e], t = to[e], l = label ? label[e] : -1;
    if (w >= V || f < 0 || f >= S || t < 0 || t >= S || l >= C || (mode == 1 && w >= -1 && l < 0)) {
        atomicExch(bad, 1);
        return;
    }
    const float v = val ? val[e] : 1.0f;
    if (mode == 1) {
        if (w >= 0) T[(((long long)w * C + l) * S + f) * S + t] = v;
        else if (w == -1) W[((long long)l * S + f) * S + t] = v;
        return;
    }
    if (w >= 0) { if (T) T[((long long)w * S + f) * S + t] = v; }
    else if (w == -1) { if (W) W[(long long)f * S + t] = v; }
    if (l >= 0) {
        if (mode == 0) O[(long long)l * S + t] = 1.0f;
        else O[((long long)l * S + f) * S + t] = 1.0f;
    }
}

__global__ void materialise_blocks_kernel(const float *Vgen, const float *S1, const float *S2, const float *W,
                                          const float *mask, float *Mf, float *Mb, int S, int SP, int SR,
                                          int R, int Rp) {
    const long long v = blockIdx.y;
    const int idx = blockIdx.x * blockDim.x + threadIdx.x;
    if (idx >= SR * SP) return;
    const int i = idx / SP, j = idx - i * SP;
    float tr = 0.0f;
    if (i < S && j < S) {
        const float *vg = Vgen + v * Rp, *s1 = S1 + (long long)i * Rp, *s2 = S2 + (long long)j * Rp;
        for (int r = 0; r < R; r++) tr = fmaf(vg[r] * s1[r], s2[r], tr);
        tr += W[(long long)i * SP + j];
        if (mask) tr *= mask[(long long)i * SP + j];
    }
    Mf[v * SR * SP + idx] = tr;
    if (Mb && i < SP && j < SR) Mb[v * SR * SP + (long long)j * SP + i] = (i < S && j < S) ? tr : 0.0f;
}

}

__global__ void col_avg_norm_kernel(const float *M, int rows, int cols, int ld, int ord, float *avg) {
    const int c = blockIdx.x;
    __shared__ float red[256];
    float acc = 0.0f;
    for (int r = threadIdx.x; r < rows; r += blockDim.x) {
        const float v = M[(long long)r * ld + c];
        acc += ord == 1 ? fabsf(v) : v * v;
    }
    red[threadIdx.x] = acc;
    __syncthreads();
    for (int o = 128; o > 0; o >>= 1) { if ((int)threadIdx.x < o) red[threadIdx.x] += red[threadIdx.x + o]; __syncthreads(); }
    if (threadIdx.x == 0) avg[c] = (ord == 1 ? red[0] : sqrtf(red[0])) / (float)rows;
}

__global__ void norm_scales_kernel(const float *avg , float *scale , int R) {
    const int c = blockIdx.x * blockDim.x + threadIdx.x;
    if (c >= R) return;
    const float f = cbrtf(avg[c] * avg[R + c] * avg[2 * R + c]);
    scale[c] = f / avg[c]; scale[R + c] = f / avg[R + c]; scale[2 * R + c] = f / avg[2 * R + c];
}

__global__ void gram_kernel(const float *M, int rows, int cols, double *G) {
    const int i = blockIdx.x, j = blockIdx.y;
    if (j > i) return;
    __shared__ double red[256];
    double acc = 0.0;
    for (int r = threadIdx.x; r < rows; r += blockDim.x) acc += (double)M[(long long)r * cols + i] * (double)M[(long long)r * cols + j];
    red[threadIdx.x] = acc;
    __syncthreads();
    for (int o = 128; o > 0; o >>= 1) { if ((int)threadIdx.x < o) red[threadIdx.x] += red[threadIdx.x + o]; __syncthreads(); }
    if (threadIdx.x == 0) { G[(long long)i * cols + j] = red[0]; G[(long long)j * cols + i] = red[0]; }
}

__global__ void scale_cols_kernel(float *M, long long n, int cols, const float *scale) {
    const long long i = (long long)blockIdx.x * blockDim.x + threadIdx.x;
    if (i < n) M[i] *= scale[i % cols];
}

__global__ void fold_vgen_kernel(const float *Vemb, const float *E, const float *G, const float *beta, const float *cv,
                                 float *Vgen, int V, int R, int D, int add_nl) {
    const long long idx = (long long)blockIdx.x * blockDim.x + threadIdx.x;
    if (idx >= (long long)V * R) return;
    const int w = (int)(idx / R), r = (int)(idx % R);
    float g = 0.0f;
    for (int d = 0; d < D; d++) g = fmaf(E[(long long)w * D + d], G[(long long)d * R + r], g);
    const float c = cv ? cv[r] : 1.0f;
    const float b = beta[r];
    Vgen[idx] = Vemb[idx] * c * b + farnn::apply_nl(g * c, add_nl) * (1.0f - b);
}

__global__ void stage_in_kernel(const int64_t *__restrict__ src, int64_t *__restrict__ dst, long long n) {
    const long long i = ((long long)blockIdx.x * blockDim.x + threadIdx.x) * 2;
    if (i + 1 < n) *reinterpret_cast<int4 *>(dst + i) = *reinterpret_cast<const int4 *>(src + i);
    else if (i < n) dst[i] = src[i];
}
```

re2nn-seq_amd/csrc/tag_create.hip.h:

```cpp
#pragma once
#include <algorithm>
#include <utility>
#include <vector>

#include "tag_host.hip.h"
#include "score_decode.hip.h"
#include "decomp1_score.hip.h"
#include "compact.hip.h"

static int begin_create(bool args_ok, farnn_model **out) {
    if (!args_ok || !out) return fail(FARNN_EINVAL, "null argument%s%s");
    *out = nullptr;
    return FARNN_OK;
}

static int begin_model(ModelOwner &own, int kind, int device) {
    int rc = select_device(device);
    if (rc) return rc;
    own.reset(new (std::nothrow) farnn_model());
    if (!own) return fail(FARNN_ENOMEM, "host allocation failed%s%s");
    own->kind = kind; own->device = device;
    return FARNN_OK;
}

static void set_labels(farnn_model *m, int K) {
    m->K = K; m->Kp = round_up(K, 4); m->Kc = round_up(K, 64);
}

static void pick_chain_geometry(farnn_model *m) {
    m->geom = chain_geometry(m->S, tun(TUN_RPG), tun(TUN_NLD));
    m->rgeom = regs_geometry(m->S);
    if (m->rgeom.SP != m->geom.SP) m->rgeom.ok = false;
    if (m->rgeom.ok && m->rgeom.rows > m->geom.SR) m->geom.SR = m->rgeom.rows;
    m->chain_ks = tun(TUN_KS);
}

static int onehot_geometry(farnn_model *m) {
    pick_chain_geometry(m);
    m->SP = m->geom.SP;
    return m->geom.NCH > 4 ? fail(FARNN_ERANGE, "more than 1024 states%s%s") : FARNN_OK;
}

static int alloc_chain_blocks(farnn_model *m) {
    const size_t nM = (size_t)m->V * m->geom.SR * m->SP;
    if (int rc = dev_alloc(m, (void **)&m->Mf, nM * 4)) return rc;
    return dev_alloc(m, (void **)&m->Mb, nM * 4);
}

static int premix_chain_blocks(farnn_model *m, const float *T, const float *W, const float *mask) {
    if (int rc = alloc_chain_blocks(m)) return rc;
    return launch_premix(T, W, mask, m->Mf, m->Mb, m->V, m->S, m->SP, m->geom.SR);
}

static int upload_start_final(farnn_model *m, const float *h0, const float *hT, int on_device) {
    int rc;
    if ((rc = dev_upload(m, &m->h0, h0, m->S, m->SP, on_device))) return rc;
    if ((rc = dev_upload(m, &m->hT, hT, m->S, m->SP, on_device))) return rc;
    m->dw.h0 = m->h0; m->dw.hT = m->hT;
    return FARNN_OK;
}

static int default_crf_transitions(std::vector<float> &tr, int K) {
    tr.assign((size_t)K * K, 0.0f);
    for (int i = 0; i < K; i++) tr[(size_t)i * K + (K - 2)] = -10000.0f;
    for (int j = 0; j < K; j++) tr[(size_t)(K - 1) * K + j] = -10000.0f;
    return FARNN_OK;
}

static int setup_priority(farnn_model *m, const float *P, int on_device) {
    if (!P) return FARNN_OK;
    return upload_padded(m, &m->P, P, m->K, m->K, m->K, m->Kc, on_device);
}

static int setup_crf(farnn_model *m, const float *crf_trans, int on_device) {
    if (!m->use_crf) return FARNN_OK;
    std::vector<float> dflt;
    if (!crf_trans) { default_crf_transitions(dflt, m->K); crf_trans = dflt.data(); on_device = 0; }
    return upload_transposed(m, &m->tr, crf_trans, m->K, m->K, m->Kp, on_device);
}
static int upload_decode_tables(farnn_model *m, const float *P, const float *crf_trans, int on_device) {
    if (int rc = setup_priority(m, P, on_device)) return rc;
    return setup_crf(m, crf_trans, on_device);
}

static int build_ot_image(farnn_model *m) {
    int rc;
    m->c16 = (m->S + 15) / 16;
    const long long n = (long long)(m->Kc / 16) * m->c16 * 256;
    if ((rc = dev_alloc(m, (void **)&m->OTm, (size_t)n * 4))) return rc;
    ot_to_mfma_kernel<<<(unsigned)((n + 255) / 256), 256>>>(m->OT, m->OTm, m->S, m->Kc, m->c16);
    FARNN_HIP_TRY(hipGetLastError());
    return FARNN_OK;
}

static int build_label_map(farnn_model *m) {
    m->lm.on = 0;
    if (!m->OT || m->S > 1024 || tun(TUN_NOLABELMAP)) return FARNN_OK;
    std::vector<float> ot((size_t)m->S * m->Kc);
    FARNN_HIP_TRY(hipMemcpy(ot.data(), m->OT, ot.size() * 4, hipMemcpyDeviceToHost));
    std::vector<std::pair<int, int>> pos;
    for (int s = 0; s < m->S; s++) {
        int lab = -1;
        for (int c = 0; c < m->K; c++) {
            const float v = ot[(size_t)s * m->Kc + c];
            if (v == 0.0f) continue;
            if (v != 1.0f || lab >= 0) return FARNN_OK;
            lab = c;
        }
        if (lab >= 0) pos.push_back({lab, s});
    }
    const int n = (int)pos.size();
    if (n > LM_MAXS || m->S > 256 || m->K > 510) return FARNN_OK;
    std::sort(pos.begin(), pos.end());
    const int clampcol = m->use_crf ? m->K - 3 : m->K - 1;
    std::vector<unsigned> tab(128, 0u);
    int lb[128];
    for (int j = 0; j < 128; j++) lb[j] = j < n ? pos[j].first : m->K + j;
    for (int j = 0; j < 128; j++) {
        unsigned wd = j < n ? ((unsigned)pos[j].second | ((unsigned)lb[j] << LM_LB_SHIFT)) : (0x1ffu << LM_LB_SHIFT);
        const int base = j & ~63, r = (j & 63) >> 4;
        const int dd[4] = {1, 2, 4, 8};
        for (int d = 0; d < 4; d++)
            if ((j & 15) >= dd[d] && lb[j - dd[d]] == lb[j]) wd |= 1u << (LM_CF_SHIFT + d);
        if ((r == 1 || r == 3) && lb[base + 16 * r - 1] == lb[j]) wd |= 1u << (LM_CF_SHIFT + 4);
        if ((r == 2 || r == 3) && lb[base + 31] == lb[j]) wd |= 1u << (LM_CF_SHIFT + 5);
        if (j >= 64 && lb[j] == lb[63]) wd |= 1u << LM_CC_BIT;
        if (j < n && (j == n - 1 || lb[j + 1] != lb[j])) wd |= 1u << LM_TL_BIT;
        tab[j] = wd;
    }
    std::vector<char> has((size_t)m->K, 0);
    for (int j = 0; j < n; j++) has[pos[j].first] = 1;
    m->lm.e0 = -1;
    for (int c = 0; c < m->K; c++)
        if (!has[c]) { m->lm.e0 = c; break; }
    m->lm.z0 = (m->lm.e0 == clampcol) ? std::min(0.0f, m->threshold) : 0.0f;
    m->lm.nq = n > 64 ? 2 : 1;
    m->lm.clampcol = clampcol; m->lm.threshold = m->threshold;
    m->lm.clamp_empty = (clampcol >= 0 && clampcol < m->K && !has[clampcol]) ? 1 : 0;
    unsigned *dv = nullptr;
    int rc = dev_alloc(m, (void **)&dv, tab.size() * 4);
    if (rc) return rc;
    FARNN_HIP_TRY(hipMemcpy(dv, tab.data(), tab.size() * 4, hipMemcpyHostToDevice));
    m->lm.tab = dv;
    m->lm.on = 1;
    return FARNN_OK;
}
static int build_output_matrix(farnn_model *m, const float *src, int rows, int on_device) {
    DevTmp tmp;
    const float *O = nullptr;
    int rc;
    if ((rc = tmp.view(&O, src, (size_t)rows * m->S, on_device))) return rc;
    if ((rc = dev_alloc(m, (void **)&m->o, (size_t)m->SP * 4))) return rc;
    if ((rc = dev_alloc(m, (void **)&m->OT, round_up_sz((size_t)m->S * m->Kc * 4, 1024)))) return rc;
    FARNN_HIP_TRY(hipMemset(m->o, 0, (size_t)m->SP * 4));
    FARNN_HIP_TRY(hipMemset(m->OT, 0, round_up_sz((size_t)m->S * m->Kc * 4, 1024)));
    colsum_kernel<<<(m->S + 255) / 256, 256>>>(O, m->o, rows, m->S);
    int n = rows * m->S;
    transpose_pad_kernel<<<(n + 255) / 256, 256>>>(O, m->OT, rows, m->S, m->Kc);
    FARNN_HIP_TRY(hipGetLastError());
    if ((rc = build_ot_image(m))) return rc;
    FARNN_HIP_TRY(hipDeviceSynchronize());
    if ((rc = build_label_map(m))) return rc;
    m->dw.o = m->o;
    return FARNN_OK;
}

static int alloc_bitmaps(farnn_model *m) {
    m->bmNS = (m->semiring == FARNN_SEMIRING_SUM) ? compact_ns(m->S) : 0;
    if (!m->bmNS) return FARNN_OK;
    const size_t nb = (size_t)m->V * m->S * m->bmNS * sizeof(u64), nw = (size_t)m->S * m->bmNS * sizeof(u64);
    int rc;
    if ((rc = dev_alloc(m, (void **)&m->bmF, nb)) || (rc = dev_alloc(m, (void **)&m->bmB, nb)) ||
        (rc = dev_alloc(m, (void **)&m->bmWF, nw)) || (rc = dev_alloc(m, (void **)&m->bmWB, nw))) return rc;
    FARNN_HIP_TRY(hipMemset(m->bmF, 0, nb)); FARNN_HIP_TRY(hipMemset(m->bmB, 0, nb));
    FARNN_HIP_TRY(hipMemset(m->bmWF, 0, nw)); FARNN_HIP_TRY(hipMemset(m->bmWB, 0, nw));
    return FARNN_OK;
}

static int finish_bitmaps(farnn_model *m, int *bad_dev) {
    int bad = 0;
    FARNN_HIP_TRY(hipGetLastError());
    FARNN_HIP_TRY(hipMemcpy(&bad, bad_dev, sizeof(int), hipMemcpyDeviceToHost));
    if (bad) m->bmNS = 0;
    if (m->bmNS >= 1 && m->bmNS <= 2 && (unsigned long long)m->V * m->S * m->bmNS * 8ull < (1ull << 32) - 4096) {
        const size_t nb = (size_t)m->V * m->S * m->bmNS * sizeof(u64);
        int rc;
        if ((rc = dev_alloc(m, (void **)&m->bmMF, nb + 4096)) || (rc = dev_alloc(m, (void **)&m->bmMB, nb + 4096)) ||
            (rc = dev_alloc(m, (void **)&m->bmXF, nb + 4096)) || (rc = dev_alloc(m, (void **)&m->bmXB, nb + 4096)) ||
            (rc = dev_alloc(m, (void **)&m->bmTok, (size_t)m->V * sizeof(unsigned)))) return rc;
        FARNN_HIP_TRY(hipMemset(m->bmMF + nb / 8, 0, 4096)); FARNN_HIP_TRY(hipMemset(m->bmMB + nb / 8, 0, 4096));
        FARNN_HIP_TRY(hipMemset(m->bmXF + nb / 8, 0, 4096)); FARNN_HIP_TRY(hipMemset(m->bmXB + nb / 8, 0, 4096));
        std::vector<unsigned> off((size_t)m->V);
        for (int v = 0; v < m->V; v++) off[(size_t)v] = (unsigned)((size_t)v * m->S * m->bmNS * 8);
        FARNN_HIP_TRY(hipMemcpy(m->bmTok, off.data(), off.size() * sizeof(unsigned), hipMemcpyHostToDevice));
        const long long n = (long long)m->V * m->S * m->bmNS;
        merge_planes_kernel<<<(unsigned)((n + 255) / 256), 256>>>(m->bmF, m->bmB, m->bmWF, m->bmWB, m->bmMF, m->bmMB, m->bmXF, m->bmXB,
                                                                  m->bmTok, m->V, m->S, m->bmNS);
        FARNN_HIP_TRY(hipGetLastError());
        FARNN_HIP_TRY(hipDeviceSynchronize());
    }
    return FARNN_OK;
}

struct DevEdges { const int32_t *word, *from, *to; const float *val; long long n; };

static int build_bitmaps(farnn_model *m, const float *T, const float *W, const DevEdges *e) {
    DevTmp tmp;
    int *bad = nullptr;
    if (int rc = tmp.zeros(&bad, 1)) return rc;
    if (!e)
        dense_to_bits_kernel<<<dim3(m->V + 1, (m->S * m->S + 255) / 256), 256>>>(T, W, m->bmF, m->bmB, m->bmWF, m->bmWB, m->V, m->S,
                                                                              m->bmNS, bad);
    else if (e->n > 0)
        edges_to_bits_kernel<<<(unsigned)((e->n + 255) / 256), 256>>>(e->word, e->from, e->to, e->val, e->n, m->bmF, m->bmB, m->bmWF,
                                                                      m->bmWB, m->V, m->S, m->bmNS, bad);
    return finish_bitmaps(m, bad);
}

static int ifst_create_impl(const farnn_onehot_ifst_desc *d, int device, farnn_model **out, const DevEdges *compact_edges) {
    int rc = begin_create(d != nullptr, out);
    if (rc) return rc;
    if (d->V <= 0 || d->S <= 0 || d->C <= 0 || ((!d->T || !d->W) && !compact_edges) || !d->O || !d->h0 || !d->hT)
        return fail(FARNN_EINVAL, "onehot_ifst: sizes must be positive and T/W/O/h0/hT non-null%s%s");
    if (d->nl < 0 || d->nl > FARNN_NL_RELUTANH) return fail(FARNN_EINVAL, "onehot_ifst: bad nl%s%s");
    if (d->semiring != FARNN_SEMIRING_SUM && d->semiring != FARNN_SEMIRING_MAX)
        return fail(FARNN_EINVAL, "onehot_ifst: bad semiring%s%s");
    ModelOwner own;
    if ((rc = begin_model(own, KIND_IFST, device))) return rc;
    farnn_model *m = own.get();
    TunScope tun_scope(&m->tun);
    m->V = d->V; m->S = d->S; m->C = d->C;
    m->use_crf = d->use_crf ? 1 : 0;
    set_labels(m, d->C + (m->use_crf ? 2 : 0));
    m->nl = d->nl; m->semiring = d->semiring; m->threshold = d->threshold; m->o_idx = d->o_idx;
    if (m->K > 64 * SCORE_KCH) return fail(FARNN_ERANGE, "more than 256 label columns%s%s");
    if ((rc = onehot_geometry(m))) return rc;
    const int od = d->weights_on_device;

    if (compact_edges) {
        if ((rc = alloc_bitmaps(m))) return rc;
        if (!m->bmNS) return fail(FARNN_ERANGE, "onehot_ifst compact form: needs the sum semiring and at most 512 states%s%s");
        if ((rc = build_bitmaps(m, nullptr, nullptr, compact_edges))) return rc;
        if (!m->bmNS) return fail(FARNN_EINVAL, "onehot_ifst compact form: an edge is out of range or has a weight other than 1%s%s");
        m->compact_on = true;
    } else {
        DevTmp tmp;
        const float *T = nullptr, *W = nullptr;
        if ((rc = tmp.view(&T, d->T, (size_t)m->V * m->S * m->S, od))) return rc;
        if ((rc = tmp.view(&W, d->W, (size_t)m->S * m->S, od))) return rc;
        if ((rc = premix_chain_blocks(m, T, W, nullptr))) return rc;
        if ((rc = alloc_bitmaps(m))) return rc;
        if (m->bmNS && (rc = build_bitmaps(m, T, W, nullptr))) return rc;
    }
    if ((rc = build_output_matrix(m, d->O, m->C, od))) return rc;
    if ((rc = upload_start_final(m, d->h0, d->hT, od))) return rc;
    if (d->P && m->use_crf) {
        std::vector<float> Pc((size_t)m->C * m->C), Pk((size_t)m->K * m->K, 0.0f);
        FARNN_HIP_TRY(hipMemcpy(Pc.data(), d->P, Pc.size() * 4,
                                od ? hipMemcpyDeviceToHost : hipMemcpyHostToHost));
        for (int i = 0; i < m->C; i++)
            for (int j = 0; j < m->C; j++) Pk[(size_t)i * m->K + j] = Pc[(size_t)i * m->C + j];
        Pk[(size_t)(m->K - 2) * m->K + m->K - 2] = 1.0f;
        Pk[(size_t)(m->K - 1) * m->K + m->K - 1] = 1.0f;
        if ((rc = setup_priority(m, Pk.data(), 0))) return rc;
    } else if ((rc = setup_priority(m, d->P, od))) return rc;
    if ((rc = setup_crf(m, d->crf_trans, od))) return rc;
    *out = own.release();
    return FARNN_OK;
}

extern "C" int farnn_onehot_ifst_create(const farnn_onehot_ifst_desc *d, int device, farnn_model **out) {
    return ifst_create_impl(d, device, out, nullptr);
}

extern "C" int farnn_onehot_fst4_create(const farnn_onehot_fst4_desc *d, int device, farnn_model **out) {
    int rc = begin_create(d != nullptr, out);
    if (rc) return rc;
    if (d->V <= 0 || d->S <= 0 || d->C <= 0 || !d->T4 || !d->W4 || !d->h0 || !d->hT)
        return fail(FARNN_EINVAL, "onehot_fst4: sizes must be positive and T4/W4/h0/hT non-null%s%s");
    ModelOwner own;
    if ((rc = begin_model(own, KIND_FST4, device))) return rc;
    farnn_model *m = own.get();
    TunScope tun_scope(&m->tun);
    m->V = d->V; m->S = d->S; m->C = d->C;
    set_labels(m, d->C);
    m->nl = FARNN_NL_RELU;
    m->semiring = d->semiring; m->threshold = d->threshold; m->o_idx = d->o_idx;
    if (m->K > 1024) return fail(FARNN_ERANGE, "more than 1024 label columns%s%s");
    if ((rc = onehot_geometry(m))) return rc;
    const int od = d->weights_on_device;
    {
        DevTmp tmp;
        const float *T4 = nullptr, *W4 = nullptr;
        if ((rc = tmp.view(&T4, d->T4, (size_t)m->V * m->C * m->S * m->S, od))) return rc;
        if ((rc = tmp.view(&W4, d->W4, (size_t)m->C * m->S * m->S, od))) return rc;
        if ((rc = alloc_chain_blocks(m))) return rc;
        if ((rc = dev_alloc(m, (void **)&m->A4, (size_t)m->V * m->C * m->S * m->SP * 4))) return rc;
        if ((rc = launch_premix_fst4(T4, W4, m->Mf, m->Mb, m->A4, m->V, m->C, m->S, m->SP, m->geom.SR))) return rc;
    }
    if ((rc = upload_start_final(m, d->h0, d->hT, od))) return rc;
    if ((rc = upload_decode_tables(m, d->P, nullptr, od))) return rc;
    *out = own.release();
    return FARNN_OK;
}

extern "C" int farnn_onehot_ind1_create(const farnn_onehot_ind1_desc *d, int device, farnn_model **out) {
    int rc = begin_create(d != nullptr, out);
    if (rc) return rc;
    if (d->V <= 0 || d->S <= 0 || d->C <= 0 || !d->T || !d->W || !d->Oten || !d->h0 || !d->hT)
        return fail(FARNN_EINVAL, "onehot_ind1: sizes must be positive and T/W/Oten/h0/hT non-null%s%s");
    ModelOwner own;
    if ((rc = begin_model(own, KIND_IND1, device))) return rc;
    farnn_model *m = own.get();
    TunScope tun_scope(&m->tun);
    m->V = d->V; m->S = d->S; m->C = d->C;
    set_labels(m, d->C);
    m->nl = FARNN_NL_RELU;
    m->semiring = d->semiring; m->threshold = d->threshold; m->o_idx = d->o_idx;
    m->mask_by_output = d->mask_by_output;
    if (m->K > 1024) return fail(FARNN_ERANGE, "more than 1024 label columns%s%s");
    if ((rc = onehot_geometry(m))) return rc;
    const int od = d->weights_on_device;
    {
        DevTmp tmp;
        const float *T = nullptr, *W = nullptr, *Ot = nullptr;
        if ((rc = tmp.view(&T, d->T, (size_t)m->V * m->S * m->S, od))) return rc;
        if ((rc = tmp.view(&W, d->W, (size_t)m->S * m->S, od))) return rc;
        if ((rc = tmp.view(&Ot, d->Oten, (size_t)m->C * m->S * m->S, od))) return rc;
        if ((rc = dev_alloc(m, (void **)&m->Ms, (size_t)m->V * m->S * m->SP * 4))) return rc;
        if ((rc = upload_padded(m, &m->Oten, Ot, m->C * m->S, m->S, m->C * m->S, m->SP, 1))) return rc;
        float *osum = nullptr;
        if (m->mask_by_output) {
            if ((rc = dev_alloc(m, (void **)&osum, (size_t)m->S * m->S * 4))) return rc;
            colsum_kernel<<<(m->S * m->S + 255) / 256, 256>>>(Ot, osum, m->C, m->S * m->S);
            FARNN_HIP_TRY(hipGetLastError());
        }
        if ((rc = premix_chain_blocks(m, T, W, osum))) return rc;
        if ((rc = launch_premix(T, W, nullptr, m->Ms, nullptr, m->V, m->S, m->SP, m->S))) return rc;
    }
    if ((rc = upload_start_final(m, d->h0, d->hT, od))) return rc;
    if ((rc = upload_decode_tables(m, d->P, nullptr, od))) return rc;
    *out = own.release();
    return FARNN_OK;
}

template <typename Desc>
static int begin_edge_create(const Desc *b, farnn_model **out, const char *who, bool args_ok = true) {
    if (int rc = begin_create(b && args_ok, out)) return rc;
    if (b->V <= 0 || b->S <= 0 || b->C <= 0) return fail(FARNN_EINVAL, "%s: V, S, C must be positive%s", who, "");
    return FARNN_OK;
}

static int stage_small_params(DevTmp &tmp, int on_device, int S, int C, int use_crf, const float **h0, const float **hT,
                              const float **P, const float **crf_trans) {
    if (on_device) return FARNN_OK;
    int rc;
    const size_t K = (size_t)C + (use_crf ? 2 : 0);
    if ((rc = tmp.view(h0, *h0, S, 0)) || (rc = tmp.view(hT, *hT, S, 0)) || (rc = tmp.view(P, *P, (size_t)C * C, 0))) return rc;
    return crf_trans ? tmp.view(crf_trans, *crf_trans, K * K, 0) : FARNN_OK;
}

static int scatter_edges(DevTmp &tmp, const farnn_edge_list *e, float *T, float *W, float *O, int V, int S, int C,
                         int mode) {
    if (!e || e->n_edges < 0 || (e->n_edges > 0 && (!e->word || !e->from || !e->to)))
        return fail(FARNN_EINVAL, "from_edges: edge arrays missing%s%s");
    const size_t ne = (size_t)e->n_edges;
    if (!ne) return FARNN_OK;
    int32_t *word = nullptr;
    float *val = nullptr;
    int *bad = nullptr;
    int rc;
    if ((rc = tmp.raw(&word, ne * 4))) return rc;
    int32_t *from = word + ne, *to = from + ne, *label = to + ne;
    if ((rc = tmp.raw(&val, ne))) return rc;
    if ((rc = tmp.zeros(&bad, 1))) return rc;
    FARNN_HIP_TRY(hipMemcpy(word, e->word, ne * 4, hipMemcpyHostToDevice));
    FARNN_HIP_TRY(hipMemcpy(from, e->from, ne * 4, hipMemcpyHostToDevice));
    FARNN_HIP_TRY(hipMemcpy(to, e->to, ne * 4, hipMemcpyHostToDevice));
    if (e->label) FARNN_HIP_TRY(hipMemcpy(label, e->label, ne * 4, hipMemcpyHostToDevice));
    if (e->val) FARNN_HIP_TRY(hipMemcpy(val, e->val, ne * 4, hipMemcpyHostToDevice));
    scatter_edges_kernel<<<(unsigned)((ne + 255) / 256), 256>>>(word, from, to, e->label ? label : nullptr,
                                                                 e->val ? val : nullptr, (long long)ne, T, W, O,
                                                                 V, S, C, mode, bad);
    FARNN_HIP_TRY(hipGetLastError());
    int hbad = 0;
    FARNN_HIP_TRY(hipMemcpy(&hbad, bad, 4, hipMemcpyDeviceToHost));
    if (hbad) return fail(FARNN_EINVAL, "from_edges: an edge has a word, state or label index out of range%s%s");
    return FARNN_OK;
}

extern "C" int farnn_onehot_ifst_create_from_edges(const farnn_onehot_ifst_desc *b, const farnn_edge_list *e,
                                                   int device, farnn_model **out) {
    int rc = begin_edge_create(b, out, "ifst_from_edges");
    if (rc || (rc = select_device(device))) return rc;
    DevTmp tmp;
    float *T = nullptr, *W = nullptr, *O = nullptr;
    if ((rc = tmp.zeros(&T, (size_t)b->V * b->S * b->S)) || (rc = tmp.zeros(&W, (size_t)b->S * b->S)) ||
        (rc = tmp.zeros(&O, (size_t)b->C * b->S))) return rc;
    if ((rc = scatter_edges(tmp, e, T, W, O, b->V, b->S, b->C, 0))) return rc;
    farnn_onehot_ifst_desc full = *b;
    if ((rc = stage_small_params(tmp, b->weights_on_device, b->S, b->C, b->use_crf, &full.h0, &full.hT, &full.P, &full.crf_trans))) return rc;
    full.T = T; full.W = W; full.O = O; full.weights_on_device = 1;
    return farnn_onehot_ifst_create(&full, device, out);
}

extern "C" int farnn_onehot_ifst_create_compact(const farnn_onehot_ifst_desc *b, const farnn_edge_list *e, int device,
                                                farnn_model **out) {
    int rc = begin_edge_create(b, out, "ifst_create_compact", e != nullptr);
    if (rc) return rc;
    if (e->n_edges < 0 || (e->n_edges > 0 && (!e->word || !e->from || !e->to)))
        return fail(FARNN_EINVAL, "ifst_create_compact: edge arrays missing%s%s");
    if ((rc = select_device(device))) return rc;
    DevTmp tmp;
    float *O = nullptr;
    if ((rc = tmp.zeros(&O, (size_t)b->C * b->S))) return rc;
    if ((rc = scatter_edges(tmp, e, nullptr, nullptr, O, b->V, b->S, b->C, 0))) return rc;
    const size_t ne = (size_t)e->n_edges;
    int32_t *dw = nullptr;
    float *dv = nullptr;
    if ((rc = tmp.raw(&dw, (ne ? ne : 1) * 3))) return rc;
    if (ne) {
        FARNN_HIP_TRY(hipMemcpy(dw, e->word, ne * 4, hipMemcpyHostToDevice));
        FARNN_HIP_TRY(hipMemcpy(dw + ne, e->from, ne * 4, hipMemcpyHostToDevice));
        FARNN_HIP_TRY(hipMemcpy(dw + 2 * ne, e->to, ne * 4, hipMemcpyHostToDevice));
        if (e->val && (rc = tmp.copy(&dv, e->val, ne, 0))) return rc;
    }
    DevEdges de{dw, dw + ne, dw + 2 * ne, dv, (long long)ne};
    farnn_onehot_ifst_desc full = *b;
    if ((rc = stage_small_params(tmp, b->weights_on_device, b->S, b->C, b->use_crf, &full.h0, &full.hT, &full.P, &full.crf_trans))) return rc;
    full.T = nullptr; full.W = nullptr; full.O = O; full.weights_on_device = 1;
    return ifst_create_impl(&full, device, out, &de);
}

extern "C" int farnn_onehot_fst4_create_from_edges(const farnn_onehot_fst4_desc *b, const farnn_edge_list *e,
                                                   int device, farnn_model **out) {
    int rc = begin_edge_create(b, out, "fst4_from_edges");
    if (rc || (rc = select_device(device))) return rc;
    DevTmp tmp;
    float *T4 = nullptr, *W4 = nullptr;
    if ((rc = tmp.zeros(&T4, (size_t)b->V * b->C * b->S * b->S)) || (rc = tmp.zeros(&W4, (size_t)b->C * b->S * b->S)))
        return rc;
    if ((rc = scatter_edges(tmp, e, T4, W4, nullptr, b->V, b->S, b->C, 1))) return rc;
    farnn_onehot_fst4_desc full = *b;
    if ((rc = stage_small_params(tmp, b->weights_on_device, b->S, b->C, 0, &full.h0, &full.hT, &full.P, nullptr))) return rc;
    full.T4 = T4; full.W4 = W4; full.weights_on_device = 1;
    return farnn_onehot_fst4_create(&full, device, out);
}

extern "C" int farnn_onehot_ind1_create_from_edges(const farnn_onehot_ind1_desc *b, const farnn_edge_list *e,
                                                   int device, farnn_model **out) {
    int rc = begin_edge_create(b, out, "ind1_from_edges");
    if (rc || (rc = select_device(device))) return rc;
    DevTmp tmp;
    float *T = nullptr, *W = nullptr, *Oten = nullptr;
    if ((rc = tmp.zeros(&T, (size_t)b->V * b->S * b->S)) || (rc = tmp.zeros(&W, (size_t)b->S * b->S)) ||
        (rc = tmp.zeros(&Oten, (size_t)b->C * b->S * b->S))) return rc;
    if ((rc = scatter_edges(tmp, e, T, W, Oten, b->V, b->S, b->C, 2))) return rc;
    farnn_onehot_ind1_desc full = *b;
    if ((rc = stage_small_params(tmp, b->weights_on_device, b->S, b->C, 0, &full.h0, &full.hT, &full.P, nullptr))) return rc;
    full.T = T; full.W = W; full.Oten = Oten; full.weights_on_device = 1;
    return farnn_onehot_ind1_create(&full, device, out);
}

static int build_dense_blocks(farnn_model *m) {
    const DecompWeights &w = m->dw;
    if (w.farnn != 0 || !(w.semiring == FARNN_SEMIRING_MAX || w.mask)) return FARNN_OK;
    pick_chain_geometry(m);
    if (m->geom.NCH > 4 || m->geom.SP != m->SP) return FARNN_OK;
    const size_t nM = (size_t)m->V * m->geom.SR * m->SP;
    if (nM * 8 > (size_t)64 << 30) return FARNN_OK;
    if (int rc = alloc_chain_blocks(m)) return rc;
    FARNN_HIP_TRY(hipMemset(m->Mb, 0, nM * 4));
    dim3 grid((m->geom.SR * m->SP + 255) / 256, m->V);
    materialise_blocks_kernel<<<grid, 256>>>(w.Vgen, w.S1, w.S2, w.W, w.mask, m->Mf, m->Mb, m->S, m->SP, m->geom.SR,
                                             m->R, m->Rp);
    FARNN_HIP_TRY(hipGetLastError());
    FARNN_HIP_TRY(hipDeviceSynchronize());
    m->dense_decomp = true;
    return FARNN_OK;
}

static int build_rows_pack(farnn_model *m) {
    DecompWeights &w = m->dw;
    DecompRowsPack &k = m->rows;
    k.ok = false;
    if (w.semiring != FARNN_SEMIRING_SUM || w.mask) return FARNN_OK;
    const int tvl = m->Rp + (w.farnn >= 1 ? m->SP : 0) + (w.farnn == 2 ? m->SP : 0);
    if (tvl > DR_MAX_PF * DR_THREADS) return FARNN_OK;
    k.nch2 = (m->S + DR_CHUNK - 1) / DR_CHUNK; k.nch3 = (m->Rp + m->S + DR_CHUNK - 1) / DR_CHUNK;
    k.ld2 = rows_ld(m->S); k.ld3 = rows_ld(m->Rp + m->S);
    k.n1 = w.farnn == 2 ? 2 * m->S : 0;
    k.n2 = m->R + (w.farnn == 1 ? m->S : 0);
    k.n3 = m->S;
    PackSrc q;
    q.S1 = w.S1; q.S2 = w.S2; q.W = w.W; q.Wss1 = w.Wss1; q.Wss2 = w.Wss2; q.o = w.o;
    q.S = m->S; q.SP = m->SP; q.R = m->R; q.Rp = m->Rp; q.farnn = w.farnn;
    int rc;
    auto blocks = [](long long n) { return (unsigned)((n + 255) / 256); };
    for (int dir = 0; dir < 2; dir++) {
        if ((rc = dev_alloc(m, (void **)&k.P2[dir], (size_t)k.n2 * k.ld2 * 4))) return rc;
        if ((rc = dev_alloc(m, (void **)&k.P3[dir], (size_t)k.n3 * k.ld3 * 4))) return rc;
        pack_p2_kernel<<<blocks((long long)k.n2 * k.ld2), 256>>>(q, k.P2[dir], k.n2, k.ld2, dir);
        pack_p3_kernel<<<blocks((long long)k.n3 * k.ld3), 256>>>(q, k.P3[dir], k.ld3, dir);
    }
    if (k.n1) {
        if ((rc = dev_alloc(m, (void **)&k.P1, (size_t)k.n1 * k.ld2 * 4))) return rc;
        pack_p1_kernel<<<blocks((long long)k.n1 * k.ld2), 256>>>(q, k.P1, k.ld2);
    }
    if (w.farnn == 0) {
        k.TVt = w.Vgen;
    } else {
        float *T = nullptr;
        if ((rc = dev_alloc(m, (void **)&T, (size_t)m->V * tvl * 4))) return rc;
        word_rows_kernel<<<blocks((long long)m->V * m->Rp), 256>>>(w.Vgen, T, tvl, m->V, m->Rp);
        gate_table_kernel<<<blocks((long long)m->V * m->SP), 256>>>(w.Vgen, w.Wrs1, w.bs1, T, tvl, m->Rp, m->V, m->R, m->Rp, m->S, m->SP);
        if (w.farnn == 2)
            gate_table_kernel<<<blocks((long long)m->V * m->SP), 256>>>(w.Vgen, w.Wrs2, w.bs2, T, tvl, m->Rp + m->SP, m->V, m->R, m->Rp, m->S, m->SP);
        k.TVt = T;
    }
    FARNN_HIP_TRY(hipGetLastError());
    FARNN_HIP_TRY(hipDeviceSynchronize());
    k.ok = true;
    return FARNN_OK;
}

struct GateSrc { int farnn; const float *Wss1, *Wrs1, *bs1, *Wss2, *Wrs2, *bs2; };

static int check_gates(const GateSrc &g, const char *who) {
    if (g.farnn < 0 || g.farnn > 2) return fail(FARNN_EINVAL, "%s: farnn must be 0, 1 or 2%s", who, "");
    if (g.farnn >= 1 && (!g.Wss1 || !g.Wrs1 || !g.bs1))
        return fail(FARNN_EINVAL, "%s: farnn>=1 needs Wss1/Wrs1/bs1%s", who, "");
    if (g.farnn == 2 && (!g.Wss2 || !g.Wrs2 || !g.bs2))
        return fail(FARNN_EINVAL, "%s: farnn==2 needs Wss2/Wrs2/bs2%s", who, "");
    return FARNN_OK;
}

static int upload_chain_factors(farnn_model *m, const float *Vgen, int odV, const float *S1, const float *S2,
                                int odS, const float *W, int odW, const GateSrc &g, int odG) {
    DecompWeights &w = m->dw;
    int rc;
    w.S = m->S; w.SP = m->SP; w.R = m->R; w.Rp = m->Rp; w.V = m->V;
    w.farnn = g.farnn; w.nl = m->nl; w.semiring = m->semiring; w.sig_k = m->sig_k;
    float *tmp = nullptr;
    if ((rc = upload_padded(m, &tmp, Vgen, m->V, m->R, m->V, m->Rp, odV))) return rc; w.Vgen = tmp;
    if ((rc = upload_padded(m, &tmp, S1, m->S, m->R, m->S, m->Rp, odS))) return rc; w.S1 = tmp;
    if ((rc = upload_padded(m, &tmp, S2, m->S, m->R, m->S, m->Rp, odS))) return rc; w.S2 = tmp;
    if ((rc = upload_transposed(m, &tmp, S1, m->S, m->R, m->SP, odS))) return rc; w.S1T = tmp;
    if ((rc = upload_transposed(m, &tmp, S2, m->S, m->R, m->SP, odS))) return rc; w.S2T = tmp;
    if ((rc = upload_padded(m, &tmp, W, m->S, m->S, m->S, m->SP, odW))) return rc; w.W = tmp;
    if ((rc = upload_transposed(m, &tmp, W, m->S, m->S, m->SP, odW))) return rc; w.WT = tmp;
    if (g.farnn >= 1) {
        if ((rc = upload_padded(m, &tmp, g.Wss1, m->S, m->S, m->S, m->SP, odG))) return rc; w.Wss1 = tmp;
        if ((rc = upload_padded(m, &tmp, g.Wrs1, m->R, m->S, m->R, m->SP, odG))) return rc; w.Wrs1 = tmp;
        if ((rc = dev_upload(m, &tmp, g.bs1, m->S, m->SP, odG))) return rc; w.bs1 = tmp;
    }
    if (g.farnn == 2) {
        if ((rc = upload_padded(m, &tmp, g.Wss2, m->S, m->S, m->S, m->SP, odG))) return rc; w.Wss2 = tmp;
        if ((rc = upload_padded(m, &tmp, g.Wrs2, m->R, m->S, m->R, m->SP, odG))) return rc; w.Wrs2 = tmp;
        if ((rc = dev_upload(m, &tmp, g.bs2, m->S, m->SP, odG))) return rc; w.bs2 = tmp;
    }
    return FARNN_OK;
}

static int upload_ones_o(farnn_model *m) {
    std::vector<float> ones((size_t)m->SP, 1.0f);
    int rc = dev_upload(m, &m->o, ones.data(), m->SP, m->SP, 0);
    if (rc) return rc;
    m->dw.o = m->o;
    return FARNN_OK;
}

static_assert(64 * SCORE_KCH == 256, "the label-column limit of the decomposed creates");
template <typename Desc>
static int decomp_geometry(farnn_model *m, const Desc *d) {
    m->V = d->V; m->S = d->S; m->R = d->R;
    set_labels(m, d->K);
    m->C = d->use_crf ? d->K - 2 : d->K;
    m->SP = round_up(d->S, 4); m->Rp = round_up(d->R, 4);
    m->nl = d->nl; m->semiring = d->semiring; m->threshold = d->threshold; m->o_idx = d->o_idx;
    m->use_crf = d->use_crf ? 1 : 0; m->farnn_gate = d->farnn; m->sig_k = d->sigmoid_exponent;
    return m->K > 256 ? fail(FARNN_ERANGE, "more than 256 label columns%s%s") : FARNN_OK;
}

static int decomp_ifst_create_impl(const farnn_decomp_ifst_desc *d, int device, farnn_model **out, int od_vgen, int od_s12) {
    int rc = begin_create(d != nullptr, out);
    if (rc) return rc;
    if (d->V <= 0 || d->S <= 0 || d->R <= 0 || d->K <= 0 || !d->Vgen || !d->S1 || !d->S2 || !d->W ||
        !d->Cout || !d->h0 || !d->hT)
        return fail(FARNN_EINVAL, "decomp_ifst: sizes must be positive and factor pointers non-null%s%s");
    const GateSrc gates{d->farnn, d->Wss1, d->Wrs1, d->bs1, d->Wss2, d->Wrs2, d->bs2};
    if ((rc = check_gates(gates, "decomp_ifst"))) return rc;
    if (d->nl < 0 || d->nl > FARNN_NL_RELUTANH) return fail(FARNN_EINVAL, "decomp_ifst: bad nl%s%s");
    ModelOwner own;
    if ((rc = begin_model(own, KIND_DECOMP, device))) return rc;
    farnn_model *m = own.get();
    TunScope tun_scope(&m->tun);
    if ((rc = decomp_geometry(m, d))) return rc;
    if (m->S > 1024 || m->R > 4096) return fail(FARNN_ERANGE, "decomp_ifst: S<=1024, R<=4096%s%s");
    const int od = d->weights_on_device;
    if ((rc = upload_chain_factors(m, d->Vgen, od | od_vgen, d->S1, d->S2, od | od_s12, d->W, od, gates, od))) return rc;
    if ((rc = build_output_matrix(m, d->Cout, m->K, od))) return rc;
    if ((rc = upload_start_final(m, d->h0, d->hT, od))) return rc;
    if ((rc = upload_decode_tables(m, d->P, d->crf_trans, od))) return rc;
    if ((rc = build_rows_pack(m))) return rc;
    if ((rc = build_dense_blocks(m))) return rc;
    *out = own.release();
    return FARNN_OK;
}

extern "C" int farnn_decomp_ifst_create(const farnn_decomp_ifst_desc *d, int device, farnn_model **out) {
    return decomp_ifst_create_impl(d, device, out, 0, 0);
}

static double gram_largest_eigenvalue(std::vector<double> &A, int n) {
    if (n <= 0) return 0.0;
    auto matmul_sq = [&](std::vector<double> &M) {
        double tr = 0.0;
        for (int i = 0; i < n; i++) tr += M[(size_t)i * n + i];
        if (!(tr > 0.0)) return 0.0;
        std::vector<double> N((size_t)n * n, 0.0);
        for (int i = 0; i < n; i++)
            for (int k = 0; k < n; k++) {
                const double a = M[(size_t)i * n + k] / tr;
                if (a == 0.0) continue;
                for (int j = 0; j < n; j++) N[(size_t)i * n + j] += a * (M[(size_t)k * n + j] / tr);
            }
        M.swap(N);
        return tr;
    };
    std::vector<double> B = A;
    for (int k = 0; k < 6; k++)
        if (!(matmul_sq(B) > 0.0)) return 0.0;
    std::vector<double> v((size_t)n), w((size_t)n);
    for (int i = 0; i < n; i++) v[i] = 1.0 + 1e-3 * ((i * 2654435761u) % 1000);
    double lam = 0.0;
    for (int it = 0; it < 200; it++) {
        const std::vector<double> &M = it < 8 ? B : A;
        double nrm = 0.0;
        for (int i = 0; i < n; i++) { double acc = 0.0; for (int j = 0; j < n; j++) acc += M[(size_t)i * n + j] * v[j]; w[i] = acc; nrm += acc * acc; }
        nrm = sqrt(nrm);
        if (!(nrm > 0.0)) return 0.0;
        for (int i = 0; i < n; i++) v[i] = w[i] / nrm;
        if (it >= 8) {
            double num = 0.0;
            for (int i = 0; i < n; i++) { double acc = 0.0; for (int j = 0; j < n; j++) acc += A[(size_t)i * n + j] * v[j]; num += v[i] * acc; }
            if (fabs(num - lam) <= 1e-14 * fabs(num)) { lam = num; break; }
            lam = num;
        }
    }
    return lam;
}

extern "C" int farnn_decomp_ifst_create_folded(const farnn_decomp_ifst_desc *d, const farnn_vgen_fold *f, int device,
                                               farnn_model **out) {
    int rc = begin_create(d && f, out);
    if (rc) return rc;
    if (d->V <= 0 || d->S <= 0 || d->R <= 0 || f->D <= 0 || !f->V_embed || !f->E || !f->G || !f->beta || !d->S1 || !d->S2)
        return fail(FARNN_EINVAL, "decomp_ifst_create_folded: V_embed / E / G / beta / S1 / S2 and positive sizes needed%s%s");
    if (f->add_nl < FARNN_NL_NONE || f->add_nl > FARNN_NL_SIGMOID) return fail(FARNN_EINVAL, "decomp_ifst_create_folded: bad add_nl%s%s");
    if (f->normalize < FARNN_NORM_NONE || f->normalize > FARNN_NORM_L2_RANK)
        return fail(FARNN_EINVAL, "decomp_ifst_create_folded: bad normalize mode%s%s");
    if ((rc = select_device(device))) return rc;
    const size_t V = d->V, R = d->R, S = d->S, D = f->D;
    DevTmp tmp;
    float *Vd = nullptr, *S1d = nullptr, *S2d = nullptr, *Vgen = nullptr, *avg = nullptr;
    const float *E = nullptr, *G = nullptr, *beta = nullptr;
    if ((rc = tmp.copy(&Vd, f->V_embed, V * R, f->on_device)) || (rc = tmp.copy(&S1d, d->S1, S * R, d->weights_on_device)) ||
        (rc = tmp.copy(&S2d, d->S2, S * R, d->weights_on_device)) || (rc = tmp.view(&E, f->E, V * D, f->on_device)) ||
        (rc = tmp.view(&G, f->G, D * R, f->on_device)) || (rc = tmp.view(&beta, f->beta, R, f->on_device)) ||
        (rc = tmp.raw(&Vgen, V * R)) || (rc = tmp.raw(&avg, 6 * R))) return rc;
    const float *cv = nullptr;
    if (f->normalize == FARNN_NORM_L1 || f->normalize == FARNN_NORM_L2) {
        const float *mats[3] = {Vd, S1d, S2d};
        const size_t rows[3] = {V, S, S};
        double avgs[3];
        if (f->normalize == FARNN_NORM_L1) {
            for (int q = 0; q < 3; q++) col_avg_norm_kernel<<<(unsigned)R, 256>>>(mats[q], (int)rows[q], (int)R, (int)R, 1, avg + q * R);
            std::vector<float> hv(3 * R);
            FARNN_HIP_TRY(hipMemcpy(hv.data(), avg, 3 * R * 4, hipMemcpyDeviceToHost));
            for (int q = 0; q < 3; q++) {
                float mx = 0.0f;
                for (size_t c = 0; c < R; c++) mx = hv[q * R + c] > mx ? hv[q * R + c] : mx;
                avgs[q] = (double)mx / (double)R;
            }
        } else {
            double *Gd = nullptr;
            if ((rc = tmp.raw(&Gd, R * R))) return rc;
            std::vector<double> Gh(R * R);
            for (int q = 0; q < 3; q++) {
                gram_kernel<<<dim3((unsigned)R, (unsigned)R), 256>>>(mats[q], (int)rows[q], (int)R, Gd);
                FARNN_HIP_TRY(hipMemcpy(Gh.data(), Gd, R * R * 8, hipMemcpyDeviceToHost));
                avgs[q] = sqrt(gram_largest_eigenvalue(Gh, (int)R)) / ((double)rows[q] * (double)R);
            }
        }
        if (!(avgs[0] > 0.0) || !(avgs[1] > 0.0) || !(avgs[2] > 0.0))
            return fail(FARNN_EINVAL, "decomp_ifst_create_folded: a factor matrix has zero norm%s%s");
        const double fac = cbrt(avgs[0] * avgs[1] * avgs[2]);
        std::vector<float> sc(3 * R);
        for (int q = 0; q < 3; q++)
            for (size_t c = 0; c < R; c++) sc[q * R + c] = (float)(fac / avgs[q]);
        FARNN_HIP_TRY(hipMemcpy(avg + 3 * R, sc.data(), 3 * R * 4, hipMemcpyHostToDevice));
        scale_cols_kernel<<<(unsigned)((S * R + 255) / 256), 256>>>(S1d, (long long)(S * R), (int)R, avg + 4 * R);
        scale_cols_kernel<<<(unsigned)((S * R + 255) / 256), 256>>>(S2d, (long long)(S * R), (int)R, avg + 5 * R);
        cv = avg + 3 * R;
    } else if (f->normalize != FARNN_NORM_NONE) {
        const int ord = f->normalize == FARNN_NORM_L1_RANK ? 1 : 2;
        col_avg_norm_kernel<<<(unsigned)R, 256>>>(Vd, (int)V, (int)R, (int)R, ord, avg);
        col_avg_norm_kernel<<<(unsigned)R, 256>>>(S1d, (int)S, (int)R, (int)R, ord, avg + R);
        col_avg_norm_kernel<<<(unsigned)R, 256>>>(S2d, (int)S, (int)R, (int)R, ord, avg + 2 * R);
        norm_scales_kernel<<<(unsigned)((R + 255) / 256), 256>>>(avg, avg + 3 * R, (int)R);
        scale_cols_kernel<<<(unsigned)((S * R + 255) / 256), 256>>>(S1d, (long long)(S * R), (int)R, avg + 4 * R);
        scale_cols_kernel<<<(unsigned)((S * R + 255) / 256), 256>>>(S2d, (long long)(S * R), (int)R, avg + 5 * R);
        cv = avg + 3 * R;
    }
    fold_vgen_kernel<<<(unsigned)((V * R + 255) / 256), 256>>>(Vd, E, G, beta, cv, Vgen, (int)V, (int)R, (int)D, f->add_nl);
    FARNN_HIP_TRY(hipGetLastError());
    FARNN_HIP_TRY(hipDeviceSynchronize());
    farnn_decomp_ifst_desc full = *d;
    full.Vgen = Vgen; full.S1 = S1d; full.S2 = S2d;
    return decomp_ifst_create_impl(&full, device, out, 1, 1);
}

extern "C" int farnn_decomp_ind1_create(const farnn_decomp_ind1_desc *d, int device, farnn_model **out) {
    int rc = begin_create(d != nullptr, out);
    if (rc) return rc;
    if (d->V <= 0 || d->S <= 0 || d->R <= 0 || d->RO <= 0 || d->K <= 0 || !d->Vgen || !d->S1 || !d->S2 ||
        !d->W || !d->Cout || !d->S1o || !d->S2o || !d->h0 || !d->hT)
        return fail(FARNN_EINVAL, "decomp_ind1: sizes must be positive and factor pointers non-null%s%s");
    const GateSrc gates{d->farnn, d->Wss1, d->Wrs1, d->bs1, d->Wss2, d->Wrs2, d->bs2};
    if ((rc = check_gates(gates, "decomp_ind1"))) return rc;
    if (d->nl < 0 || d->nl > FARNN_NL_RELUTANH) return fail(FARNN_EINVAL, "decomp_ind1: bad nl%s%s");
    ModelOwner own;
    if ((rc = begin_model(own, KIND_DECOMP1, device))) return rc;
    farnn_model *m = own.get();
    TunScope tun_scope(&m->tun);
    m->RO = d->RO; m->ROp = round_up(d->RO, 4);
    if ((rc = decomp_geometry(m, d))) return rc;
    if (decomp1_score_lds_bytes(m->S, m->SP, m->Rp, m->ROp, m->Kc) > 160 * 1024)
        return fail(FARNN_ERANGE, "decomp_ind1: S*S*4 bytes of LDS needed per token (S too large)%s%s");
    const int od = d->weights_on_device;
    if ((rc = upload_chain_factors(m, d->Vgen, od, d->S1, d->S2, od, d->W, od, gates, od))) return rc;
    {
        if ((rc = upload_ones_o(m))) return rc;
        DevTmp tmp;
        const float *Co = nullptr, *S1o = nullptr, *S2o = nullptr, *Wo = nullptr;
        if ((rc = tmp.view(&Co, d->Cout, (size_t)m->K * m->RO, od))) return rc;
        if ((rc = tmp.view(&S1o, d->S1o, (size_t)m->S * m->RO, od))) return rc;
        if ((rc = tmp.view(&S2o, d->S2o, (size_t)m->S * m->RO, od))) return rc;
        if ((rc = tmp.view(&Wo, d->Wo, (size_t)m->S * m->S, od))) return rc;
        float *osum = nullptr;
        if ((rc = dev_alloc(m, (void **)&osum, (size_t)m->S * m->SP * 4))) return rc;
        FARNN_HIP_TRY(hipMemset(osum, 0, (size_t)m->S * m->SP * 4));
        output_sum_kernel<<<(m->S * m->S + 255) / 256, 256>>>(Co, S1o, S2o, Wo, osum, m->K, m->S, m->SP, m->RO);
        FARNN_HIP_TRY(hipGetLastError());
        FARNN_HIP_TRY(hipDeviceSynchronize());
        m->dw.mask = osum;
    }
    if ((rc = upload_padded(m, &m->d1_S1o, d->S1o, m->S, m->RO, m->S, m->ROp, od))) return rc;
    if ((rc = upload_padded(m, &m->d1_S2o, d->S2o, m->S, m->RO, m->S, m->ROp, od))) return rc;
    if ((rc = upload_transposed(m, &m->d1_CoutT, d->Cout, m->K, m->RO, m->Kc, od))) return rc;
    if ((rc = upload_start_final(m, d->h0, d->hT, od))) return rc;
    if ((rc = upload_decode_tables(m, d->P, d->crf_trans, od))) return rc;
    if (m->RO <= 16 * D1M_MAXNT && m->S <= 16 * D1M_MAXKQ4 && (size_t)m->V * m->S * m->SP * 4 <= ((size_t)32 << 30)) {
        const int MT = (m->S + 15) / 16, NT = (m->RO + 15) / 16, KQ4 = MT;
        DevTmp tmp;
        float *bss = nullptr;
        if ((rc = tmp.raw(&bss, (size_t)m->V * m->S * m->SP))) return rc;
        dim3 grid((m->S * m->SP + 255) / 256, m->V);
        materialise_blocks_kernel<<<grid, 256>>>(m->dw.Vgen, m->dw.S1, m->dw.S2, m->dw.W, nullptr, bss, nullptr,
                                                 m->S, m->SP, m->S, m->R, m->Rp);
        const long long total = (long long)m->V * MT * KQ4 * 256;
        if ((rc = dev_alloc(m, (void **)&m->d1_BSSp, (size_t)total * 4)) ||
            (rc = dev_alloc(m, (void **)&m->d1_S1oP, (size_t)MT * NT * 256 * 4)) ||
            (rc = dev_alloc(m, (void **)&m->d1_S2oP, (size_t)KQ4 * NT * 256 * 4))) return rc;
        pack_s2o_operand_kernel<<<(KQ4 * NT * 256 + 255) / 256, 256>>>(m->d1_S2o, m->d1_S2oP, KQ4 * NT * 256,
                                                                      m->S, m->RO, m->ROp, NT);
        pack_bss_operand_kernel<<<(unsigned)((total + 255) / 256), 256>>>(bss, m->d1_BSSp, total, m->S, m->SP, MT, KQ4);
        pack_s1o_operand_kernel<<<(MT * NT * 256 + 255) / 256, 256>>>(m->d1_S1o, m->d1_S1oP, MT * NT * 256,
                                                                     m->S, m->RO, m->ROp, NT);
        FARNN_HIP_TRY(hipGetLastError());
        FARNN_HIP_TRY(hipDeviceSynchronize());
    }
    if ((rc = build_dense_blocks(m))) return rc;
    *out = own.release();
    return FARNN_OK;
}

extern "C" int farnn_decomp_fst_create(const farnn_decomp_fst_desc *d, int device, farnn_model **out) {
    int rc = begin_create(d != nullptr, out);
    if (rc) return rc;
    if (d->V <= 0 || d->S <= 0 || d->R <= 0 || d->RW <= 0 || d->K <= 0 || !d->Vgen || !d->C || !d->S1 ||
        !d->S2 || !d->Cw || !d->S1w || !d->S2w || !d->WW || !d->h0 || !d->hT)
        return fail(FARNN_EINVAL, "decomp_fst: sizes must be positive and factor pointers non-null%s%s");
    const GateSrc gates{d->farnn, d->Wss1, d->Wrs1, d->bs1, d->Wss2, d->Wrs2, d->bs2};
    if ((rc = check_gates(gates, "decomp_fst"))) return rc;
    if (d->nl < 0 || d->nl > FARNN_NL_RELUTANH) return fail(FARNN_EINVAL, "decomp_fst: bad nl%s%s");
    ModelOwner own;
    if ((rc = begin_model(own, KIND_DECOMP0, device))) return rc;
    farnn_model *m = own.get();
    TunScope tun_scope(&m->tun);
    m->RW = d->RW; m->RWp = round_up(d->RW, 4);
    if ((rc = decomp_geometry(m, d))) return rc;
    if (m->S > 1024 || m->R > 4096 || m->RW > 4096)
        return fail(FARNN_ERANGE, "decomp_fst: S<=1024, R<=4096, RW<=4096%s%s");
    const int od = d->weights_on_device;
    {
        DevTmp tmp;
        const float *Cd = nullptr, *Cwd = nullptr, *S1wd = nullptr, *S2wd = nullptr, *WWd = nullptr;
        if ((rc = tmp.view(&Cd, d->C, (size_t)m->K * m->R, od))) return rc;
        if ((rc = tmp.view(&Cwd, d->Cw, (size_t)m->K * m->RW, od))) return rc;
        if ((rc = tmp.view(&S1wd, d->S1w, (size_t)m->S * m->RW, od))) return rc;
        if ((rc = tmp.view(&S2wd, d->S2w, (size_t)m->S * m->RW, od))) return rc;
        if ((rc = tmp.view(&WWd, d->WW, (size_t)m->S * m->S, od))) return rc;
        float *table = nullptr, *wsum = nullptr;
        if ((rc = tmp.copy(&table, d->Vgen, (size_t)m->V * m->R, od))) return rc;
        if ((rc = tmp.raw(&wsum, (size_t)m->S * m->S))) return rc;
        const long long n = (long long)m->V * m->R;
        scale_by_colsum_kernel<<<(unsigned)((n + 255) / 256), 256>>>(table, Cd, m->V, m->R, m->K);
        output_sum_kernel<<<(m->S * m->S + 255) / 256, 256>>>(Cwd, S1wd, S2wd, WWd, wsum, m->K, m->S, m->S, m->RW);
        FARNN_HIP_TRY(hipGetLastError());
        FARNN_HIP_TRY(hipDeviceSynchronize());
        if ((rc = upload_chain_factors(m, table, 1, d->S1, d->S2, od, wsum, 1, gates, od))) return rc;
    }
    if ((rc = upload_ones_o(m))) return rc;
    if ((rc = upload_padded(m, &m->d0_Vgen, d->Vgen, m->V, m->R, m->V, m->Rp, od))) return rc;
    if ((rc = upload_transposed(m, &m->d0_CT, d->C, m->K, m->R, m->Kc, od))) return rc;
    if ((rc = upload_padded(m, &m->d0_S1w, d->S1w, m->S, m->RW, m->S, m->RWp, od))) return rc;
    if ((rc = upload_padded(m, &m->d0_S2w, d->S2w, m->S, m->RW, m->S, m->RWp, od))) return rc;
    if ((rc = upload_transposed(m, &m->d0_CwT, d->Cw, m->K, m->RW, m->Kc, od))) return rc;
    if ((rc = upload_start_final(m, d->h0, d->hT, od))) return rc;
    if ((rc = upload_decode_tables(m, d->P, d->crf_trans, od))) return rc;
    if ((rc = build_rows_pack(m))) return rc;
    *out = own.release();
    return FARNN_OK;
}
```

re2nn-seq_amd/csrc/tag_host.hip.h:

```cpp
#pragma once
#include <hip/hip_runtime.h>
#include <memory>
#include <new>
#include <vector>

#include "common.hip.h"
#include "host_util.hip.h"
#include "chain.hip.h"
#include "layout.hip.h"
#include "decomp_chain.hip.h"
#include "decomp_rows.hip.h"
#include "chain_regs_params.hip.h"

using namespace farnn;

enum { KIND_IFST = 2, KIND_IND1 = 1, KIND_FST4 = 0, KIND_DECOMP = 12, KIND_DECOMP1 = 11, KIND_DECOMP0 = 10 };
enum { KERN_CHAIN = 0, KERN_SCORE = 1, KERN_PREP = 2, KERN_COUNT = 3 };

struct Prof {
    std::vector<hipEvent_t> ev[KERN_COUNT];
    std::vector<hipEvent_t> pool;
    double ms[KERN_COUNT] = {0, 0, 0};
    long long n[KERN_COUNT] = {0, 0, 0};
    hipEvent_t get() {
        hipEvent_t e = nullptr;
        if (!pool.empty()) { e = pool.back(); pool.pop_back(); return e; }
        return hipEventCreate(&e) == hipSuccess ? e : nullptr;
    }
};

struct Workspace {
    float *A = nullptr, *Bk = nullptr;
    int64_t *offs = nullptr;
    int *order = nullptr;
    unsigned long long *hs = nullptr;
    size_t hs_bytes = 0;
    float *crf_scores = nullptr;
    float *d1_br = nullptr;
    int B = 0, L = 0;
    void release() {
        for (void *p : {(void *)A, (void *)Bk, (void *)offs, (void *)order, (void *)hs, (void *)crf_scores, (void *)d1_br})
            if (p) (void)hipFree(p);
        *this = Workspace();
    }
};

struct farnn_model {
    Tunables tun;
    int kind = 0, device = 0;
    int V = 0, S = 0, SP = 0, C = 0, K = 0, Kp = 0, Kc = 0, R = 0, Rp = 0;
    int nl = 0, semiring = 0, o_idx = 0, use_crf = 0, farnn_gate = 0, mask_by_output = 0;
    float threshold = 0.5f, sig_k = 1.0f;
    float *Mf = nullptr, *Mb = nullptr;
    u64 *bmF = nullptr, *bmB = nullptr, *bmWF = nullptr, *bmWB = nullptr;
    int bmNS = 0;
    u64 *bmMF = nullptr, *bmMB = nullptr, *bmXF = nullptr, *bmXB = nullptr;
    unsigned *bmTok = nullptr;
    bool compact_on = false;
    float *Ms = nullptr;
    float *A4 = nullptr;
    float *Oten = nullptr;
    float *o = nullptr, *h0 = nullptr, *hT = nullptr;
    float *OT = nullptr, *P = nullptr, *tr = nullptr;
    float *OTm = nullptr; int c16 = 0;
    LabelMap lm = {nullptr, 0, 0, -1, 0.0f, 0, 0, 0.0f};
    DecompWeights dw;
    DecompRowsPack rows;
    int RO = 0, ROp = 0;
    float *d1_S1o = nullptr, *d1_S2o = nullptr, *d1_CoutT = nullptr;
    float *d1_BSSp = nullptr;
    float *d1_S1oP = nullptr;
    float *d1_S2oP = nullptr;
    int n_cu = 0;
    int RW = 0, RWp = 0;
    float *d0_Vgen = nullptr, *d0_CT = nullptr, *d0_S1w = nullptr, *d0_S2w = nullptr, *d0_CwT = nullptr;
    Workspace ws;
    int curL = 0;
    ChainGeom geom;
    RegsGeom rgeom;
    unsigned epoch_u = 0;
    bool last_regs = false;
    bool last_lm_score = false;
    int chain_ks = 3;
    bool prep_in_kernel = false, sort_in_kernel = false;
    bool dense_decomp = false;
    bool order_valid = false;
    bool last_wave = false;
    bool last_fused = false;
    int profiling = 0;
    long long calls = 0;
    int prof_this_call = 0;
    Prof prof;
    std::vector<void *> owned;
    struct HostSlot {
        int64_t *x_pin = nullptr, *flat_pin = nullptr;
        int64_t *x_dev = nullptr, *flat_dev = nullptr, *x_map = nullptr;
        size_t capN = 0, capB = 0;
        long long total = 0;
        hipEvent_t ev_out = nullptr;
        bool busy = false;
        unsigned gen = 0;
    } hslot[FARNN_HOST_SLOTS];
    hipStream_t hs_run = nullptr;
    int hnext = 0;
    hipStream_t last_stream = nullptr;
    bool have_last = false, multi_stream = false;
    hipEvent_t ev_order = nullptr;
};

struct DestroyModel { void operator()(farnn_model *m) const { farnn_destroy(m); } };
using ModelOwner = std::unique_ptr<farnn_model, DestroyModel>;

struct DevTmp {
    std::vector<void *> held;
    DevTmp() = default;
    DevTmp(const DevTmp &) = delete;
    DevTmp &operator=(const DevTmp &) = delete;
    ~DevTmp() { for (void *p : held) (void)hipFree(p); }
    template <typename T>
    int raw(T **q, size_t count) {
        FARNN_HIP_TRY(hipMalloc((void **)q, count ? count * sizeof(T) : 4));
        held.push_back(*q);
        return FARNN_OK;
    }
    template <typename T>
    int zeros(T **q, size_t count) {
        if (int rc = raw(q, count)) return rc;
        FARNN_HIP_TRY(hipMemset(*q, 0, count * sizeof(T)));
        return FARNN_OK;
    }
    template <typename T>
    int copy(T **q, const T *src, size_t count, int on_device) {
        if (int rc = raw(q, count)) return rc;
        FARNN_HIP_TRY(hipMemcpy(*q, src, count * sizeof(T), on_device ? hipMemcpyDeviceToDevice : hipMemcpyHostToDevice));
        return FARNN_OK;
    }
    int view(const float **q, const float *src, size_t count, int on_device) {
        *q = src;
        if (on_device || !src) return FARNN_OK;
        float *dv = nullptr;
        if (int rc = copy(&dv, src, count, 0)) return rc;
        *q = dv;
        return FARNN_OK;
    }
};

static int dev_alloc(farnn_model *m, void **p, size_t bytes) {
    FARNN_HIP_TRY(hipMalloc(p, bytes + 1024));
    m->owned.push_back(*p);
    return FARNN_OK;
}

static int dev_upload(farnn_model *m, float **dst, const float *src, size_t n, size_t n_alloc,
                      int on_device) {
    int rc = dev_alloc(m, (void **)dst, n_alloc * sizeof(float));
    if (rc) return rc;
    FARNN_HIP_TRY(hipMemset(*dst, 0, n_alloc * sizeof(float)));
    if (src && n)
        FARNN_HIP_TRY(hipMemcpy(*dst, src, n * sizeof(float),
                                on_device ? hipMemcpyDeviceToDevice : hipMemcpyHostToDevice));
    return FARNN_OK;
}

static int upload_padded(farnn_model *m, float **dst, const float *src, int rows, int cols,
                         int rows_alloc, int cols_p, int on_device) {
    int rc = dev_alloc(m, (void **)dst, (size_t)rows_alloc * cols_p * sizeof(float));
    if (rc) return rc;
    FARNN_HIP_TRY(hipMemset(*dst, 0, (size_t)rows_alloc * cols_p * sizeof(float)));
    if (src)
        FARNN_HIP_TRY(hipMemcpy2D(*dst, (size_t)cols_p * 4, src, (size_t)cols * 4, (size_t)cols * 4,
                                  rows, on_device ? hipMemcpyDeviceToDevice : hipMemcpyHostToDevice));
    return FARNN_OK;
}

static int upload_transposed(farnn_model *m, float **dst, const float *src, int rows, int cols,
                             int rows_p, int on_device) {
    DevTmp tmp;
    const float *t = nullptr;
    int rc = tmp.view(&t, src, (size_t)rows * cols, on_device);
    if (rc) return rc;
    rc = dev_alloc(m, (void **)dst, (size_t)cols * rows_p * sizeof(float));
    if (rc) return rc;
    FARNN_HIP_TRY(hipMemset(*dst, 0, (size_t)cols * rows_p * sizeof(float)));
    int n = rows * cols;
    transpose_pad_kernel<<<(n + 255) / 256, 256>>>(t, *dst, rows, cols, rows_p);
    FARNN_HIP_TRY(hipGetLastError());
    FARNN_HIP_TRY(hipDeviceSynchronize());
    return FARNN_OK;
}
```

Baseline: 309.1 million tokens/s.

## Stream transition blocks as exact fp16 image with mixed-precision FMA in destination split

At model creation the code checks whether every premixed transition block value is exactly representable in fp16. If so, it builds a packed 16-bit image of the forward and backward blocks, laid out for five lanes per row. The destination-split recurrence kernel then loads two dwordx4 chunks per lane instead of four or five and accumulates with v_fma_mix_f32, which roughly halves the per-token weight bytes fetched from memory. The cost is a new template variant, extra device memory for the images, and the new path only activates when the onehot weights pass the exactness check, which preserves results.

New measurement: 321.7 million tokens/s, median of 6. +4.1%, better.

```diff
diff --git a/re2nn-seq_amd/csrc/chain_dest.hip.h b/re2nn-seq_amd/csrc/chain_dest.hip.h
--- a/re2nn-seq_amd/csrc/chain_dest.hip.h
+++ b/re2nn-seq_amd/csrc/chain_dest.hip.h
@@ -4,9 +4,10 @@
 
 namespace farnn {
 
-template <int D, int LPR>
+template <int D, int LPR, bool H16 = false>
 struct DestRing {
-    static constexpr int NC = 20 / LPR;
+    static_assert(!H16 || LPR == 5, "the 16-bit image is laid out for five lanes per row");
+    static constexpr int NC = H16 ? 2 : 20 / LPR;
     v4f r[D][NC];
     unsigned voff[NC];
     int tkw_lo, tkw_hi;
@@ -33,6 +34,12 @@
                          "global_load_dwordx4 %4, %9, %10" FARNN_RD_CPOL                                     \
                          : "=&v"(ring_.r[d][0]), "=&v"(ring_.r[d][1]), "=&v"(ring_.r[d][2]), "=&v"(ring_.r[d][3]), "=&v"(ring_.r[d][NC - 1]) \
                          : "v"(ring_.voff[0]), "v"(ring_.voff[1]), "v"(ring_.voff[2]), "v"(ring_.voff[3]), "v"(ring_.voff[NC - 1]), "s"(bp_)); \
+        else if constexpr (NC == 2)                                                            \
+            asm volatile("s_nop 4\n\t"                                                         \
+                         "global_load_dwordx4 %0, %2, %4" FARNN_RD_CPOL "\n\t"                                  \
+                         "global_load_dwordx4 %1, %3, %4" FARNN_RD_CPOL                                      \
+                         : "=&v"(ring_.r[d][0]), "=&v"(ring_.r[d][NC - 1])                      \
+                         : "v"(ring_.voff[0]), "v"(ring_.voff[NC - 1]), "s"(bp_));              \
         else                                                                                   \
             asm volatile("s_nop 4\n\t"                                                         \
                          "global_load_dwordx4 %0, %4, %8" FARNN_RD_CPOL "\n\t"                                  \
@@ -43,10 +50,10 @@
                          : "v"(ring_.voff[0]), "v"(ring_.voff[1]), "v"(ring_.voff[2]), "v"(ring_.voff[3]), "s"(bp_)); \
     } while (0)
 
-template <int D, int LPR>
+template <int D, int LPR, bool H16>
 __device__ __forceinline__ void regs_dest_prime(const RegsParams &p, const int dir, const int w, const int lane, const int nsteps,
-                                                const int len, const int b, DestRing<D, LPR> &ring) {
-    constexpr int NC = DestRing<D, LPR>::NC;
+                                                const int len, const int b, DestRing<D, LPR, H16> &ring) {
+    constexpr int NC = DestRing<D, LPR, H16>::NC;
     const int S = p.S, SP = p.SP, CPR = p.CPR;
     const int RW = (S + RG_NWC - 1) / RG_NWC;
     int rj, rs;
@@ -57,15 +64,20 @@
 #pragma unroll
     for (int i = 0; i < NC; i++) {
         const int ci = rs + LPR * i;
-        ring.voff[i] = ((unsigned)(my_valid ? my_row : 0) * (unsigned)SP + (unsigned)((my_valid && ci < CPR) ? ci : rs < CPR ? rs : 0) * 4u) * 4u;
-    }
+        if constexpr (H16)
+            ring.voff[i] = (unsigned)(my_valid ? my_row : 0) * (unsigned)(RD_XS * 2) + (unsigned)ci * 16u;
+        else
+            ring.voff[i] = ((unsigned)(my_valid ? my_row : 0) * (unsigned)SP + (unsigned)((my_valid && ci < CPR) ? ci : rs < CPR ? rs : 0) * 4u) * 4u;
+    }
+    (void)SP; (void)CPR;
     {
         const int t = lane < nsteps ? lane : nsteps - 1;
         const int idx = (dir == 0) ? t : (t < len ? len - 1 - t : t);
-        const long long o_ = (long long)clamp_tok(p.x[(long long)b * p.L + idx], p.V) * p.blk * 4;
+        const long long o_ = (long long)clamp_tok(p.x[(long long)b * p.L + idx], p.V) * (H16 ? p.blk16 : p.blk * 4);
         ring.tkw_lo = (int)(unsigned)o_; ring.tkw_hi = (int)(unsigned)(o_ >> 32);
     }
-    const char *Mbase = reinterpret_cast<const char *>(dir == 0 ? p.Mb : p.Mf);
+    const char *Mbase = H16 ? reinterpret_cast<const char *>(dir == 0 ? p.Mb16 : p.Mf16)
+                            : reinterpret_cast<const char *>(dir == 0 ? p.Mb : p.Mf);
 #pragma unroll
     for (int d = 0; d < D; d++) {
 #pragma unroll
@@ -77,14 +89,26 @@
     }
 }
 
-template <bool NLX, int D, int LPR>
+template <bool HI, bool FIRST>
+__device__ __forceinline__ void fma_h16(float &acc, const float blk, const float st) {
+    if constexpr (FIRST) {
+        if constexpr (HI) asm("v_fma_mix_f32 %0, %1, %2, 0 op_sel:[1,0,0] op_sel_hi:[1,0,0]" : "=v"(acc) : "v"(blk), "v"(st));
+        else              asm("v_fma_mix_f32 %0, %1, %2, 0 op_sel_hi:[1,0,0]" : "=v"(acc) : "v"(blk), "v"(st));
+    } else {
+        if constexpr (HI) asm("v_fma_mix_f32 %0, %1, %2, %0 op_sel:[1,0,0] op_sel_hi:[1,0,0]" : "+v"(acc) : "v"(blk), "v"(st));
+        else              asm("v_fma_mix_f32 %0, %1, %2, %0 op_sel_hi:[1,0,0]" : "+v"(acc) : "v"(blk), "v"(st));
+    }
+}
+
+template <bool NLX, int D, int LPR, bool H16>
 __device__ __forceinline__ void regs_compute_dest(const RegsParams &p, const int dir, const int w, const int lane_in, const int nsteps,
                                                   const long long *tokoff, float *flags, const float *ol, float *hist, float *xd,
-                                                  const bool probe, const int b, DestRing<D, LPR> &ring) {
+                                                  const bool probe, const int b, DestRing<D, LPR, H16> &ring) {
     static_assert(D == 2 || D == 4, "an even ring depth that divides 64 (the exchange row's parity and the address window)");
     static_assert(LPR == 4 || LPR == 5, "four or five lanes per output row");
-    constexpr int NC = 20 / LPR;
-    static_assert(LPR * NC * 4 == RD_XS, "the exchange row holds every lane's chunks");
+    constexpr int NC = DestRing<D, LPR, H16>::NC;
+    constexpr int NS = 20 / LPR;
+    static_assert(LPR * NS * 4 == RD_XS, "the exchange row holds every lane's chunks");
     int lane = lane_in;
     const int S = p.S, SP = p.SP, CPR = p.CPR;
     const int RW = (S + RG_NWC - 1) / RG_NWC;
@@ -96,7 +120,8 @@
     const bool my_writer = my_valid && rs == (LPR == 4 ? 0 : 4);
     const bool is_flane = lane == 63;
     (void)CPR;
-    const char *Mbase = reinterpret_cast<const char *>(dir == 0 ? p.Mb : p.Mf);
+    const char *Mbase = H16 ? reinterpret_cast<const char *>(dir == 0 ? p.Mb16 : p.Mf16)
+                            : reinterpret_cast<const char *>(dir == 0 ? p.Mb : p.Mf);
     const float my_o = my_valid ? ol[my_row] : 1.0f;
     const float c_pre = dir == 0 ? my_o : 1.0f, c_post = dir == 0 ? 1.0f : my_o;
     float *xbuf = xd;
@@ -138,6 +163,9 @@
         if constexpr (NC == 5)                                                                 \
             asm volatile(FARNN_RD_WAITSTR : "+v"(r[d][0]), "+v"(r[d][1]), "+v"(r[d][2]), "+v"(r[d][3]), "+v"(r[d][NC - 1]) \
                          : [rem] "s"(rem_), [dm1] "n"(D - 1), [cnt] "n"((D - 1) * NC) : "scc"); \
+        else if constexpr (NC == 2)                                                            \
+            asm volatile(FARNN_RD_WAITSTR : "+v"(r[d][0]), "+v"(r[d][NC - 1])                  \
+                         : [rem] "s"(rem_), [dm1] "n"(D - 1), [cnt] "n"((D - 1) * NC) : "scc"); \
         else                                                                                   \
             asm volatile(FARNN_RD_WAITSTR : "+v"(r[d][0]), "+v"(r[d][1]), "+v"(r[d][2]), "+v"(r[d][3]) \
                          : [rem] "s"(rem_), [dm1] "n"(D - 1), [cnt] "n"((D - 1) * NC) : "scc"); \
@@ -160,29 +188,47 @@
             if (t >= nsteps) break;
             constexpr int dummy = 0; (void)dummy;
             const int roff = (d & 1) * RD_XS;
-            v4f st[NC];
+            v4f st[NS];
             {
                 int fl = lds_flag_get(pflag);
 #pragma unroll
-                for (int i = 0; i < NC; i++) st[i] = *reinterpret_cast<const v4f *>(xr + roff + 4 * LPR * i);
+                for (int i = 0; i < NS; i++) st[i] = *reinterpret_cast<const v4f *>(xr + roff + 4 * LPR * i);
                 asm volatile("" ::: "memory");
                 if (__ballot(fl < t + 1) != 0ull) {
                     do { fl = lds_flag_get(pflag); } while (__ballot(fl < t + 1) != 0ull);
 #pragma unroll
-                    for (int i = 0; i < NC; i++) st[i] = *reinterpret_cast<const v4f *>(xr + roff + 4 * LPR * i);
+                    for (int i = 0; i < NS; i++) st[i] = *reinterpret_cast<const v4f *>(xr + roff + 4 * LPR * i);
                     asm volatile("" ::: "memory");
                 }
             }
             FARNN_RD_PHASE(0);
             FARNN_RD_WAIT(d, nsteps - 1 - t);
             FARNN_RD_PHASE(1);
-            v2f a01 = v2f{0.f, 0.f}, a23 = v2f{0.f, 0.f};
-#pragma unroll
-            for (int i = 0; i < NC; i++) {
-                a01 = __builtin_elementwise_fma(st[i].xy, r[d][i].xy, a01);
-                a23 = __builtin_elementwise_fma(st[i].zw, r[d][i].zw, a23);
+            float sa, sb;
+            if constexpr (H16) {
+                float a0, a1, a2, a3;
+                fma_h16<false, true>(a0, r[d][0].x, st[0].x);
+                fma_h16<true, true>(a1, r[d][0].x, st[0].y);
+                fma_h16<false, true>(a2, r[d][0].y, st[0].z);
+                fma_h16<true, true>(a3, r[d][0].y, st[0].w);
+#pragma unroll
+                for (int i = 1; i < NS; i++) {
+                    const float bxy = (i & 1) ? r[d][i >> 1].z : r[d][i >> 1].x, bzw = (i & 1) ? r[d][i >> 1].w : r[d][i >> 1].y;
+                    fma_h16<false, false>(a0, bxy, st[i].x);
+                    fma_h16<true, false>(a1, bxy, st[i].y);
+                    fma_h16<false, false>(a2, bzw, st[i].z);
+                    fma_h16<true, false>(a3, bzw, st[i].w);
+                }
+                sa = a0 + a1; sb = a2 + a3;
+            } else {
+                v2f a01 = v2f{0.f, 0.f}, a23 = v2f{0.f, 0.f};
+#pragma unroll
+                for (int i = 0; i < NS; i++) {
+                    a01 = __builtin_elementwise_fma(st[i].xy, r[d][i].xy, a01);
+                    a23 = __builtin_elementwise_fma(st[i].zw, r[d][i].zw, a23);
+                }
+                sa = a01.x + a01.y; sb = a23.x + a23.y;
             }
-            float sa = a01.x + a01.y, sb = a23.x + a23.y;
             asm volatile("" : "+v"(sa), "+v"(sb));
             float s = sa + sb;
             if constexpr (LPR == 4) s = quad_sum(s);
diff --git a/re2nn-seq_amd/csrc/chain_regs.hip b/re2nn-seq_amd/csrc/chain_regs.hip
--- a/re2nn-seq_amd/csrc/chain_regs.hip
+++ b/re2nn-seq_amd/csrc/chain_regs.hip
@@ -12,16 +12,22 @@
     const bool dest = p.dest && !maxsr;
     const size_t lds = (size_t)regs_lds(p.L, p.SP, NP, p.sp.c16, p.sp.Kc, score, RG_RQ, score && bs_label_map_path(p.sp), dest).total * sizeof(float);
     const dim3 grid(2 * p.B), block(RG_WAVES * 64);
+    const bool half = dest && !score && p.half && p.Mf16 && p.Mb16;
     int rc;
     const bool nlx = p.nl != FARNN_NL_NONE && p.nl != FARNN_NL_RELU;
     const bool lmo = score && bs_label_map_path(p.sp);
+#define FARNN_LAUNCH_REGS6(MX, SC, NX, LM, DS, HF)                                             \
+    do {                                                                                       \
+        if ((rc = raise_lds_limit(chain_regs_kernel<MX, SC, NX, LM, DS, HF>, lds))) return rc; \
+        if (e0 && e1)                                                                          \
+            hipExtLaunchKernelGGL((chain_regs_kernel<MX, SC, NX, LM, DS, HF>), grid, block, (uint32_t)lds, s, e0, e1, 0, p); \
+        else                                                                                   \
+            chain_regs_kernel<MX, SC, NX, LM, DS, HF><<<grid, block, lds, s>>>(p);            \
+    } while (0)
 #define FARNN_LAUNCH_REGS5(MX, SC, NX, LM, DS)                                                 \
     do {                                                                                       \
-        if ((rc = raise_lds_limit(chain_regs_kernel<MX, SC, NX, LM, DS>, lds))) return rc;     \
-        if (e0 && e1)                                                                          \
-            hipExtLaunchKernelGGL((chain_regs_kernel<MX, SC, NX, LM, DS>), grid, block, (uint32_t)lds, s, e0, e1, 0, p); \
-        else                                                                                   \
-            chain_regs_kernel<MX, SC, NX, LM, DS><<<grid, block, lds, s>>>(p);                \
+        if (DS && !SC && half) FARNN_LAUNCH_REGS6(MX, SC, NX, LM, DS, (DS && !SC));            \
+        else FARNN_LAUNCH_REGS6(MX, SC, NX, LM, DS, false);                                    \
     } while (0)
 #if defined(FARNN_AB)
 #define FARNN_LAUNCH_REGS4(MX, SC, NX, LM) do { if (!MX && dest) FARNN_LAUNCH_REGS5(MX, SC, NX, LM, !MX); else FARNN_LAUNCH_REGS5(MX, SC, NX, LM, false); } while (0)
@@ -42,6 +48,7 @@
 #undef FARNN_LAUNCH_REGS3
 #undef FARNN_LAUNCH_REGS4
 #undef FARNN_LAUNCH_REGS5
+#undef FARNN_LAUNCH_REGS6
     FARNN_HIP_TRY(hipGetLastError());
     return FARNN_OK;
 }
diff --git a/re2nn-seq_amd/csrc/chain_regs.hip.h b/re2nn-seq_amd/csrc/chain_regs.hip.h
--- a/re2nn-seq_amd/csrc/chain_regs.hip.h
+++ b/re2nn-seq_amd/csrc/chain_regs.hip.h
@@ -62,10 +62,11 @@
 #define FARNN_RG_STAMP(i) do { } while (0)
 #endif
 
-template <bool MAXSR, bool SCORE, bool NLX, int RQ = RG_RQ, int D = RG_D, bool LMO = false, bool DEST = false>
+template <bool MAXSR, bool SCORE, bool NLX, int RQ = RG_RQ, int D = RG_D, bool LMO = false, bool DEST = false, bool H16 = false>
 __device__ __forceinline__ void chain_regs_body(const RegsParams &p, float *smem, const int tid, const int item, int *b_out) {
     constexpr bool WIDE = RQ != RG_RQ;
     static_assert(!DEST || (!WIDE && !MAXSR), "the destination-split form exists for the narrow kernel and the sum semiring");
+    static_assert(!H16 || (DEST && !SCORE), "the 16-bit image is read by the destination split's recurrence-only launch");
     constexpr int PSTR = WIDE ? rgw_part_stride(RQ) : RG_PART_STRIDE;
     constexpr int NG = WIDE ? RGW_NG : RG_NG;
     const int lane = tid & 63;
@@ -96,12 +97,12 @@
 #endif
 
     constexpr bool PRIME_EARLY = DEST && (!SCORE || LMO);
-    DestRing<RD_D, RD_LPR> dring;
+    DestRing<RD_D, RD_LPR, H16> dring;
     if constexpr (PRIME_EARLY)
-        if (w < RG_NWC && nsteps > 0) regs_dest_prime<RD_D, RD_LPR>(p, dir, w, lane, nsteps, len, b, dring);
+        if (w < RG_NWC && nsteps > 0) regs_dest_prime<RD_D, RD_LPR, H16>(p, dir, w, lane, nsteps, len, b, dring);
     for (int k = tid; k < nsteps; k += nthreads) {
         const int idx = (dir == 0) ? k : (k < len ? len - 1 - k : k);
-        tokoff[k] = (long long)clamp_tok(p.x[(long long)b * p.L + idx], p.V) * p.blk * 4;
+        tokoff[k] = (long long)clamp_tok(p.x[(long long)b * p.L + idx], p.V) * (H16 ? p.blk16 : p.blk * 4);
     }
     for (int j = tid; j < SP; j += nthreads) ol[j] = (p.o && j < S) ? p.o[j] : 1.0f;
     for (int j = tid; j < (nsteps + 1) * SP; j += nthreads) hist[j] = (j < S) ? hinit[j] : 0.0f;
@@ -155,8 +156,8 @@
 #else
                 const bool probe_ = false;
 #endif
-                if constexpr (!PRIME_EARLY) regs_dest_prime<RD_D, RD_LPR>(p, dir, w, lane, nsteps, len, b, dring);
-                regs_compute_dest<NLX, RD_D, RD_LPR>(p, dir, w, lane, nsteps, tokoff, part + NP * PS, ol, hist, smem + lds.xd, probe_, b, dring);
+                if constexpr (!PRIME_EARLY) regs_dest_prime<RD_D, RD_LPR, H16>(p, dir, w, lane, nsteps, len, b, dring);
+                regs_compute_dest<NLX, RD_D, RD_LPR, H16>(p, dir, w, lane, nsteps, tokoff, part + NP * PS, ol, hist, smem + lds.xd, probe_, b, dring);
                 __builtin_amdgcn_s_setprio(0);
                 if (w == 0) FARNN_RG_STAMP(2);
 #if defined(FARNN_PROBES)
@@ -519,7 +520,7 @@
 #endif
 }
 
-template <bool MAXSR, bool SCORE, bool NLX, bool LMO = false, bool DEST = false>
+template <bool MAXSR, bool SCORE, bool NLX, bool LMO = false, bool DEST = false, bool H16 = false>
 __global__ void __launch_bounds__(RG_WAVES * 64, 4)
 chain_regs_kernel(const RegsParams p) {
     extern __shared__ __align__(16) float smem[];
@@ -527,7 +528,7 @@
     long long w0r = 0, w0c = 0;
     if ((p.dbg & 2048) && threadIdx.x == 0) { w0r = (long long)__builtin_amdgcn_s_memrealtime(); w0c = (long long)__builtin_amdgcn_s_memtime(); }
     int b_probe = -1;
-    chain_regs_body<MAXSR, SCORE, NLX, RG_RQ, RG_D, LMO, DEST>(p, smem, (int)threadIdx.x, (int)blockIdx.x, &b_probe);
+    chain_regs_body<MAXSR, SCORE, NLX, RG_RQ, RG_D, LMO, DEST, H16>(p, smem, (int)threadIdx.x, (int)blockIdx.x, &b_probe);
     if ((p.dbg & 2048) && threadIdx.x == 0 && blockIdx.x < WG_STAMP_MAX) {
         const long long w1r = (long long)__builtin_amdgcn_s_memrealtime(), w1c = (long long)__builtin_amdgcn_s_memtime();
         unsigned hwid, xcc;
@@ -538,7 +539,7 @@
         o[5] = xcc & 15u; o[6] = (hwid >> 13) & 7u; o[7] = (hwid >> 8) & 15u;
     }
 #else
-    chain_regs_body<MAXSR, SCORE, NLX, RG_RQ, RG_D, LMO, DEST>(p, smem, (int)threadIdx.x, (int)blockIdx.x, nullptr);
+    chain_regs_body<MAXSR, SCORE, NLX, RG_RQ, RG_D, LMO, DEST, H16>(p, smem, (int)threadIdx.x, (int)blockIdx.x, nullptr);
 #endif
 }
 
diff --git a/re2nn-seq_amd/csrc/chain_regs_params.hip.h b/re2nn-seq_amd/csrc/chain_regs_params.hip.h
--- a/re2nn-seq_amd/csrc/chain_regs_params.hip.h
+++ b/re2nn-seq_amd/csrc/chain_regs_params.hip.h
@@ -26,6 +26,8 @@
 struct RegsParams {
     const float *Mf, *Mb;
     long long blk;
+    const unsigned short *Mf16, *Mb16;
+    long long blk16;
     const float *o, *h0, *hT;
     const int64_t *x, *len;
     const int *order;
@@ -45,6 +47,7 @@
     int dbg;
     int solo_margin;
     int dest;
+    int half;
     ScoreParams sp;
 };
 constexpr int RG_NG = 5;
diff --git a/re2nn-seq_amd/csrc/farnn_hip.hip b/re2nn-seq_amd/csrc/farnn_hip.hip
--- a/re2nn-seq_amd/csrc/farnn_hip.hip
+++ b/re2nn-seq_amd/csrc/farnn_hip.hip
@@ -130,7 +130,8 @@
             if (m->compact_on) return m->last_fused ? "compact_tag_kernel<fused: both chains + label-map scores + decode>" : "compact_chain_kernel";
             if (m->last_regs && m->last_fused && m->use_crf) return "chain_viterbi_kernel<fused: recurrence + scores + CRF decode>";
             if (m->last_regs && m->rgeom.wide) return m->last_fused ? "chain_wide_kernel<fused: scores + decode beside the recurrence>" : "chain_wide_kernel";
-            if (m->last_regs) return m->last_fused ? "chain_regs_kernel<fused: scores + decode beside the recurrence>" : "chain_regs_kernel";
+            if (m->last_regs) return m->last_fused ? "chain_regs_kernel<fused: scores + decode beside the recurrence>"
+                                                   : (m->last_half ? "chain_regs_kernel<f16 blocks>" : "chain_regs_kernel");
             if (m->dense_decomp) return "chain_kernel";
             if (m->kind == KIND_DECOMP && m->last_fused && m->last_wave) return "decomp_regs_kernel<fused: scores + decode beside the recurrence>";
             if (m->kind == KIND_DECOMP || m->kind == KIND_DECOMP1 || m->kind == KIND_DECOMP0)
@@ -158,6 +159,7 @@
     rp.G = rg.G; rp.RPG = rg.RPG; rp.RQ = rg.RQ; rp.D = rg.D; rp.PS = rg.PS; rp.pair = rg.wide ? 0 : 1;
     rp.nl = m->nl; rp.full = full; rp.dbg = tun(TUN_DBG);
     rp.dest = (!rg.wide && m->semiring != FARNN_SEMIRING_MAX && !tun(TUN_NODEST)) ? 1 : 0;
+    rp.Mf16 = m->Mf16; rp.Mb16 = m->Mb16; rp.blk16 = (long long)m->SP * RD_XS * 2;
     return rp;
 }
 
@@ -171,6 +173,7 @@
     const ChainGeom &g = m->geom;
     if (fused) *fused = false;
     m->last_regs = false;
+    m->last_half = false;
     if (m->rgeom.ok && !tun(TUN_NOREGS)) {
         const RegsGeom &rg = m->rgeom;
         const size_t lds_cap = rg.wide ? 158 * 1024 : 80 * 1024;
@@ -199,6 +202,7 @@
                 rp.sp = *fuse_sp;
                 if (fused) *fused = true;
             }
+            rp.half = (rp.dest && !score && m->Mf16 && m->Mb16 && !tun(TUN_NOHALF)) ? 1 : 0;
             KernelTimer kt(m, KERN_CHAIN, s, true);
             if (paired && score) { rp.D = 2; rp.pair = 1; }
             const int rc = (paired && score) ? launch_chain_wide_paired(rp, m->semiring == FARNN_SEMIRING_MAX, s, kt.e0, kt.e1)
@@ -206,6 +210,7 @@
                                      : launch_chain_regs(rp, m->semiring == FARNN_SEMIRING_MAX, score, s, kt.e0, kt.e1);
             if (rc) return rc;
             m->last_regs = true;
+            m->last_half = rp.half != 0;
             return FARNN_OK;
         }
     }
@@ -794,6 +799,7 @@
         if (m->compact_on) return (2.0 * S * m->bmNS * 8 + 8) * n;
         if (!m->dense_decomp && (m->kind == KIND_DECOMP || m->kind == KIND_DECOMP1 || m->kind == KIND_DECOMP0))
             return (R * 4 + 8) * n + (2.0 * S * R + S * S) * 4;
+        if (m->last_regs && m->last_half) return (2.0 * S * S * 2 + 8) * n;
         return (2.0 * S * S * 4 + 8 + (m->last_fused ? 4 : 0)) * n + (m->last_fused ? K * S * 4 : 0);
     }
     if (which == KERN_SCORE) {
diff --git a/re2nn-seq_amd/csrc/half_exact.h b/re2nn-seq_amd/csrc/half_exact.h
--- /dev/null
+++ b/re2nn-seq_amd/csrc/half_exact.h
@@ -0,0 +1,33 @@
+#pragma once
+#include <stdint.h>
+#include <string.h>
+
+#if defined(__HIPCC__)
+#define FARNN_HALF_HD __host__ __device__
+#else
+#define FARNN_HALF_HD
+#endif
+
+namespace farnn {
+
+FARNN_HALF_HD inline uint32_t f32_bits(float x) {
+    uint32_t u;
+    memcpy(&u, &x, sizeof(u));
+    return u;
+}
+
+FARNN_HALF_HD inline bool half_exact(float x) {
+    const uint32_t u = f32_bits(x), e = (u >> 23) & 0xffu, m = u & 0x7fffffu;
+    if (e == 0) return m == 0;
+    if (e < 127 - 14 || e > 127 + 15) return false;
+    return (m & 0x1fffu) == 0;
+}
+
+FARNN_HALF_HD inline uint16_t half_bits_exact(float x) {
+    const uint32_t u = f32_bits(x), e = (u >> 23) & 0xffu, m = u & 0x7fffffu;
+    const uint16_t s = (uint16_t)((u >> 16) & 0x8000u);
+    if (e == 0) return s;
+    return (uint16_t)(s | ((e - 127 + 15) << 10) | (m >> 13));
+}
+
+}
diff --git a/re2nn-seq_amd/csrc/host_util.hip.h b/re2nn-seq_amd/csrc/host_util.hip.h
--- a/re2nn-seq_amd/csrc/host_util.hip.h
+++ b/re2nn-seq_amd/csrc/host_util.hip.h
@@ -43,7 +43,7 @@
     X(NOFUSE, 0, true) X(FUSE, 0, true) X(NOREGS, 0, true) X(NOLABELMAP, 0, true) X(PREP, 0, true) X(NOSORT, 0, true)           \
     X(VITERBI_BP, 0, true) X(VITERBI_UNFUSED, 0, true) X(DECOMP_NOREGS, 0, true)                               \
     X(ROWS_NOREGS, 0, true) X(TRAIN_NOLDS, 0, true) X(TRAIN_NSEQ, 0, true)              \
-    X(WIDE_UNPAIRED, 0, true) X(ROWS_LPR4, 0, true) X(ROWS_NOROUNDS, 0, true)                                  \
+    X(WIDE_UNPAIRED, 0, true) X(ROWS_LPR4, 0, true) X(ROWS_NOROUNDS, 0, true) X(NOHALF, 0, true)                  \
                        \
     X(CV_ONE, 0, false) X(CV_STASH, 0, false) X(NODEST, 0, false)                                              \
                                                                          \
diff --git a/re2nn-seq_amd/csrc/layout.hip.h b/re2nn-seq_amd/csrc/layout.hip.h
--- a/re2nn-seq_amd/csrc/layout.hip.h
+++ b/re2nn-seq_amd/csrc/layout.hip.h
@@ -1,5 +1,7 @@
 #pragma once
 #include "common.hip.h"
+#include "half_exact.h"
+#include "chain_regs_params.hip.h"
 
 namespace farnn {
 
@@ -34,6 +36,23 @@
     }
     Mf[v * SR * SP + idx] = f;
     if (Mb) Mb[v * SR * SP + idx] = bwd;
+}
+
+__global__ void half_eligible_kernel(const float *M, long long n, int *bad) {
+    bool no = false;
+    for (long long i = (long long)blockIdx.x * blockDim.x + threadIdx.x; i < n; i += (long long)gridDim.x * blockDim.x)
+        no |= !half_exact(M[i]);
+    if (no) atomicExch(bad, 1);
+}
+
+__global__ void half_image_kernel(const float *M, unsigned short *img, int SP, int SR) {
+    const long long v = blockIdx.y;
+    const int idx = blockIdx.x * blockDim.x + threadIdx.x;
+    if (idx >= SP * RD_XS) return;
+    const int r = idx / RD_XS, j = idx - r * RD_XS, c = j >> 3, e = j & 7;
+    const int k = (c % 5) + 10 * (c / 5) + (e >= 4 ? 5 : 0), col = 4 * k + (e & 3);
+    const float x = (r < SR && col < SP) ? M[(v * SR + r) * SP + col] : 0.0f;
+    img[v * SP * RD_XS + idx] = half_bits_exact(x);
 }
 
 inline int launch_premix(const float *T, const float *W, const float *mask, float *Mf, float *Mb,
diff --git a/re2nn-seq_amd/csrc/tag_create.hip.h b/re2nn-seq_amd/csrc/tag_create.hip.h
--- a/re2nn-seq_amd/csrc/tag_create.hip.h
+++ b/re2nn-seq_amd/csrc/tag_create.hip.h
@@ -50,6 +50,30 @@
 static int premix_chain_blocks(farnn_model *m, const float *T, const float *W, const float *mask) {
     if (int rc = alloc_chain_blocks(m)) return rc;
     return launch_premix(T, W, mask, m->Mf, m->Mb, m->V, m->S, m->SP, m->geom.SR);
+}
+
+static int build_half_image(farnn_model *m) {
+    if (!m->Mf || !m->Mb || !m->rgeom.ok || m->rgeom.wide || m->semiring == FARNN_SEMIRING_MAX || m->SP > RG_MAXSP || tun(TUN_NOHALF))
+        return FARNN_OK;
+    const long long nM = (long long)m->V * m->geom.SR * m->SP;
+    DevTmp tmp;
+    int *bad = nullptr, bad_h = 0;
+    if (int rc = tmp.zeros(&bad, 1)) return rc;
+    const unsigned nb = (unsigned)std::min<long long>((nM + 255) / 256, 4096);
+    half_eligible_kernel<<<nb, 256>>>(m->Mf, nM, bad);
+    half_eligible_kernel<<<nb, 256>>>(m->Mb, nM, bad);
+    FARNN_HIP_TRY(hipGetLastError());
+    FARNN_HIP_TRY(hipMemcpy(&bad_h, bad, sizeof(int), hipMemcpyDeviceToHost));
+    if (bad_h) return FARNN_OK;
+    const size_t bytes = (size_t)m->V * m->SP * RD_XS * sizeof(unsigned short);
+    if (int rc = dev_alloc(m, (void **)&m->Mf16, bytes)) return rc;
+    if (int rc = dev_alloc(m, (void **)&m->Mb16, bytes)) return rc;
+    const dim3 grid((m->SP * RD_XS + 255) / 256, m->V);
+    half_image_kernel<<<grid, 256>>>(m->Mf, m->Mf16, m->SP, m->geom.SR);
+    half_image_kernel<<<grid, 256>>>(m->Mb, m->Mb16, m->SP, m->geom.SR);
+    FARNN_HIP_TRY(hipGetLastError());
+    FARNN_HIP_TRY(hipDeviceSynchronize());
+    return FARNN_OK;
 }
 
 static int upload_start_final(farnn_model *m, const float *h0, const float *hT, int on_device) {
@@ -249,6 +273,7 @@
         if ((rc = tmp.view(&T, d->T, (size_t)m->V * m->S * m->S, od))) return rc;
         if ((rc = tmp.view(&W, d->W, (size_t)m->S * m->S, od))) return rc;
         if ((rc = premix_chain_blocks(m, T, W, nullptr))) return rc;
+        if ((rc = build_half_image(m))) return rc;
         if ((rc = alloc_bitmaps(m))) return rc;
         if (m->bmNS && (rc = build_bitmaps(m, T, W, nullptr))) return rc;
     }
diff --git a/re2nn-seq_amd/csrc/tag_host.hip.h b/re2nn-seq_amd/csrc/tag_host.hip.h
--- a/re2nn-seq_amd/csrc/tag_host.hip.h
+++ b/re2nn-seq_amd/csrc/tag_host.hip.h
@@ -52,6 +52,8 @@
     int nl = 0, semiring = 0, o_idx = 0, use_crf = 0, farnn_gate = 0, mask_by_output = 0;
     float threshold = 0.5f, sig_k = 1.0f;
     float *Mf = nullptr, *Mb = nullptr;
+    unsigned short *Mf16 = nullptr, *Mb16 = nullptr;
+    bool last_half = false;
     u64 *bmF = nullptr, *bmB = nullptr, *bmWF = nullptr, *bmWB = nullptr;
     int bmNS = 0;
     u64 *bmMF = nullptr, *bmMB = nullptr, *bmXF = nullptr, *bmXB = nullptr;
```
